# gallilmaimon/DISSC

Measured on AMD Instinct MI355X. Metric: audio-sec/sec (RTF) HiFi-GAN resynth, 10s x32 batch, higher is better.
Workload: dtype f32

## Files before the change

### dissc_amd/_lib.py

```python
import ctypes
import os

import torch

_HERE = os.path.dirname(os.path.abspath(__file__))
_LIB_NAME = "libdissc_hip.so"


def library_path():
    return os.environ.get("DISSC_HIP_LIB") or os.path.join(_HERE, _LIB_NAME)


class DisscError(RuntimeError):
    pass


class DisscTensor(ctypes.Structure):
    _fields_ = [("name", ctypes.c_char_p), ("data", ctypes.c_void_p),
                ("shape", ctypes.c_int64 * 4), ("ndim", ctypes.c_int32)]


MAX_UPS, MAX_RK = 8, 4


class DisscGenConfig(ctypes.Structure):
    _fields_ = [("model_in_dim", ctypes.c_int32), ("upsample_initial_channel", ctypes.c_int32),
                ("num_upsamples", ctypes.c_int32), ("upsample_rates", ctypes.c_int32 * MAX_UPS),
                ("upsample_kernel_sizes", ctypes.c_int32 * MAX_UPS), ("num_kernels", ctypes.c_int32),
                ("resblock_kernel_sizes", ctypes.c_int32 * MAX_RK),
                ("resblock_dilations", (ctypes.c_int32 * 3) * MAX_RK),
                ("num_embeddings", ctypes.c_int32), ("embedding_dim", ctypes.c_int32),
                ("num_speakers", ctypes.c_int32), ("has_f0", ctypes.c_int32), ("has_spkr", ctypes.c_int32)]


class DisscConvLaunch(ctypes.Structure):
    _fields_ = [(n, ctypes.c_int32) for n in ("family", "cfg", "bm", "bn", "rows", "p0", "np", "ntap", "pad_left")]


class DisscBf3Info(ctypes.Structure):
    _fields_ = [(n, ctypes.c_int32) for n in ("bm", "bn", "small_grid", "tile", "cols", "h4", "pad")]


class DisscWino8Plan(ctypes.Structure):
    _fields_ = [(n, ctypes.c_int32) for n in ("mi", "ni", "wps", "r", "ns", "unit", "ot", "cpr", "gx", "gy")]


class DisscWinoPlan(ctypes.Structure):
    _fields_ = [(n, ctypes.c_int32) for n in ("ns", "dilation", "cpr", "rh", "tw", "shv", "unit", "ot", "gx", "gy", "wgs", "lds_bytes")]


def _load():
    path = library_path()
    if not os.path.exists(path):
        raise DisscError(
            f"{path} not found: build the HIP library first "
            "(python -c 'import __graft_entry__ as g; g.build()').  "
            "dissc_amd has no CPU fallback.")
    L = ctypes.CDLL(path)
    vp, i32, i64p = ctypes.c_void_p, ctypes.c_int, ctypes.c_void_p
    L.dissc_last_error.restype = ctypes.c_char_p
    L.dissc_abi_version.restype = i32
    L.dissc_device_count.restype = i32
    L.dissc_device_name.argtypes = [i32, ctypes.c_char_p, ctypes.c_size_t]
    L.dissc_gen_create.argtypes = [ctypes.POINTER(DisscGenConfig), ctypes.POINTER(DisscTensor),
                                   ctypes.c_size_t, ctypes.POINTER(vp)]
    L.dissc_gen_create_ex.argtypes = [ctypes.POINTER(DisscGenConfig), ctypes.POINTER(DisscTensor),
                                      ctypes.c_size_t, i32, ctypes.POINTER(vp)]
    L.dissc_gen_destroy.argtypes = [vp]
    L.dissc_gen_destroy.restype = None
    L.dissc_gen_hop.argtypes = [vp]
    L.dissc_gen_workspace_bytes.argtypes = [vp, i32, i32]
    L.dissc_gen_workspace_bytes.restype = ctypes.c_size_t
    L.dissc_gen_flops.argtypes = [vp, ctypes.c_int64]
    L.dissc_gen_flops.restype = ctypes.c_double
    L.dissc_gen_flops_executed.argtypes = [vp, ctypes.c_int64]
    L.dissc_gen_flops_executed.restype = ctypes.c_double
    L.dissc_gen_forward.argtypes = [vp, i64p, vp, i64p, vp, i32, i32, vp, vp, ctypes.c_size_t, vp]
    L.dissc_conv1d.argtypes = [vp, vp, vp, vp, vp, i32, i32, i32, i32, i32, i32, i32, i32,
                               ctypes.c_float, vp]
    L.dissc_conv_transpose1d.argtypes = [vp, vp, vp, vp, vp, i32, i32, i32, i32, i32, i32, i32, i32,
                                         ctypes.c_float, vp]
    L.dissc_conv1d_prec.argtypes = [vp, vp, vp, vp, vp, i32, i32, i32, i32, i32, i32, i32, i32, ctypes.c_float, i32, vp]
    L.dissc_conv_transpose1d_prec.argtypes = [vp, vp, vp, vp, vp, i32, i32, i32, i32, i32, i32, i32, i32, ctypes.c_float, i32, vp]
    L.dissc_pred_create.argtypes = [i32, ctypes.POINTER(DisscTensor), ctypes.c_size_t, ctypes.POINTER(vp)]
    L.dissc_pred_destroy.argtypes = [vp]
    L.dissc_pred_destroy.restype = None
    L.dissc_pred_workspace_bytes.argtypes = [vp, i32, i32]
    L.dissc_pred_workspace_bytes.restype = ctypes.c_size_t
    L.dissc_len_set_norm.argtypes = [vp, ctypes.c_float, ctypes.c_float]
    L.dissc_len_forward.argtypes = [vp, vp, vp, vp, i32, i32, vp, i32, vp, ctypes.c_size_t, vp]
    L.dissc_pitch_forward.argtypes = [vp, vp, vp, vp, i32, i32, i32, vp, vp, i32, vp, i32, vp,
                                      ctypes.c_size_t, vp]
    L.dissc_dedup.argtypes = [vp, vp, i32, i32, vp, vp, vp, vp]
    L.dissc_len_carryover.argtypes = [vp, vp, i32, i32, vp, vp, vp]
    L.dissc_expand.argtypes = [vp, vp, vp, i32, i32, vp, i32, vp]
    L.dissc_hubert_create.argtypes = [i32, ctypes.POINTER(DisscTensor), ctypes.c_size_t, vp, i32,
                                      ctypes.POINTER(vp)]
    L.dissc_hubert_create_ex.argtypes = [i32, ctypes.POINTER(DisscTensor), ctypes.c_size_t, vp, i32, i32,
                                         ctypes.POINTER(vp)]
    L.dissc_hubert_precision.argtypes = [vp]
    L.dissc_hubert_destroy.argtypes = [vp]
    L.dissc_hubert_destroy.restype = None
    L.dissc_hubert_frames.argtypes = [i32]
    L.dissc_hubert_workspace_bytes.argtypes = [vp, i32, i32]
    L.dissc_hubert_workspace_bytes.restype = ctypes.c_size_t
    L.dissc_hubert_forward.argtypes = [vp, vp, vp, i32, i32, vp, vp, vp, ctypes.c_size_t, vp]
    L.dissc_kmeans_assign.argtypes = [vp, vp, vp, i32, i32, i32, vp, vp]
    L.dissc_mfma_peak.argtypes = [i32, ctypes.POINTER(ctypes.c_float)]
    L.dissc_erf_check.argtypes = [vp, vp, i32, vp]
    L.dissc_attention.argtypes = [vp, vp, i32, i32, i32, i32, vp, vp]
    L.dissc_layernorm_cf.argtypes = [vp, vp, vp, vp, i32, i32, i32, ctypes.c_float, vp, vp]
    L.dissc_set_option.argtypes = [ctypes.c_char_p, i32]
    L.dissc_get_option.argtypes = [ctypes.c_char_p, ctypes.POINTER(ctypes.c_int)]
    L.dissc_conv_bench.argtypes = [i32] * 9 + [ctypes.POINTER(ctypes.c_float)]
    L.dissc_conv1d_s2.argtypes = [vp, vp, vp, vp, vp] + [i32] * 9 + [vp]
    L.dissc_conv1d_s2_prec.argtypes = [vp, vp, vp, vp, vp] + [i32] * 9 + [vp]
    L.dissc_linear_prec.argtypes = [vp, vp, vp, vp, vp, vp] + [i32] * 7 + [vp]
    L.dissc_conv_s2_bench.argtypes = [i32] * 5 + [ctypes.POINTER(ctypes.c_float)]
    L.dissc_pair_bench.argtypes = [i32] * 8 + [ctypes.POINTER(ctypes.c_float)]
    L.dissc_pair_info.argtypes = [i32] * 3 + [ctypes.POINTER(ctypes.c_int)] * 2
    L.dissc_conv_info.argtypes = [i32] * 7 + [ctypes.POINTER(DisscConvLaunch), i32, ctypes.POINTER(ctypes.c_int)]
    L.dissc_wino8_info.argtypes = [i32] * 6 + [ctypes.POINTER(DisscWino8Plan)]
    L.dissc_wino_info.argtypes = [i32] * 5 + [ctypes.POINTER(DisscWinoPlan)]
    L.dissc_resblock1d_bf3.argtypes = [vp, vp, vp, vp, vp, i32, i32, i32, vp, i32, i32, ctypes.c_float, i32, ctypes.c_float, i32, i32, vp]
    L.dissc_bf3_info.argtypes = [i32] * 6 + [vp, i32, i32, ctypes.POINTER(DisscBf3Info)]
    L.dissc_respair1d.argtypes = [vp] * 8 + [i32] * 6 + [ctypes.c_float, i32, ctypes.c_float, i32, vp]
    L.dissc_wav_postprocess.argtypes = [vp, vp, i32, i32, vp]
    L.dissc_pitch_stats.argtypes = [vp, vp, i32, vp, vp, vp, vp]
    i64 = ctypes.c_longlong
    L.dissc_pack_rows.argtypes = [vp, i64, vp, vp, i32, i32, vp, vp]
    L.dissc_comm_unique_id.argtypes = [ctypes.c_char_p]
    L.dissc_comm_create.argtypes = [ctypes.c_char_p, i32, i32, ctypes.POINTER(vp)]
    L.dissc_comm_destroy.argtypes = [vp]
    L.dissc_allgather_waves.argtypes = [vp, vp, ctypes.c_size_t, vp, vp]
    L.dissc_resample.argtypes = [vp, i32, vp, i32, ctypes.c_double, vp, vp, i32, i32, vp]
    return L


lib = _load()

for _kv in filter(None, os.environ.get("DISSC_OPTIONS", "").split(",")):
    _k, _v = _kv.split("=")
    if lib.dissc_set_option(_k.strip().encode(), int(_v)) != 0:
        raise DisscError(f"DISSC_OPTIONS: unknown option {_k}")


def check(rc, what=""):
    if rc != 0:
        msg = lib.dissc_last_error()
        raise DisscError(f"{what} failed ({rc}): {msg.decode() if msg else '?'}")


def current_stream_ptr(device=None):
    return ctypes.c_void_p(torch.cuda.current_stream(device).cuda_stream)


def make_tensor_table(named):
    arr = (DisscTensor * len(named))()
    keep = []
    for i, (k, t) in enumerate(named.items()):
        t = t.detach().to("cpu", torch.float32).contiguous()
        nb = k.encode()
        keep.append((t, nb))
        arr[i].name = nb
        arr[i].data = t.data_ptr()
        arr[i].ndim = t.dim()
        for d in range(t.dim()):
            arr[i].shape[d] = t.shape[d]
    return arr, keep


def conv_info(Cin, Cout, k, dilation=1, up=1, B=1, Lmax_out=1):
    out = (DisscConvLaunch * 16)()
    n = ctypes.c_int(0)
    check(lib.dissc_conv_info(Cin, Cout, k, dilation, up, B, Lmax_out, out, 16, ctypes.byref(n)), "dissc_conv_info")
    assert n.value <= 16
    return [{f: getattr(out[i], f) for f, _ in DisscConvLaunch._fields_} for i in range(n.value)]


def wino8_info(C, k, dilation, R, B, Lmax):
    out = DisscWino8Plan()
    check(lib.dissc_wino8_info(C, k, dilation, R, B, Lmax, ctypes.byref(out)), "dissc_wino8_info")
    return {f: getattr(out, f) for f, _ in DisscWino8Plan._fields_}


def wino_info(C, k, dilation, B, Lmax):
    out = DisscWinoPlan()
    check(lib.dissc_wino_info(C, k, dilation, B, Lmax, ctypes.byref(out)), "dissc_wino_info")
    return {f: getattr(out, f) for f, _ in DisscWinoPlan._fields_}


def bf3_conv_info(Cin, Cout, k, dilation=1, B=1, Lmax=1):
    out = DisscBf3Info()
    check(lib.dissc_bf3_info(Cout, Cin, k, dilation, B, Lmax, None, 0, 0, ctypes.byref(out)), "dissc_bf3_info")
    return {f: getattr(out, f) for f in ("bm", "bn", "small_grid", "tile")}


def bf3_block_info(C, k, dil, m0=0, m1=3):
    out = DisscBf3Info()
    d3 = (ctypes.c_int32 * 3)(*dil)
    check(lib.dissc_bf3_info(C, C, k, 1, 1, 1, d3, m0, m1, ctypes.byref(out)), "dissc_bf3_info")
    return {f: getattr(out, f) for f in ("cols", "pad", "h4", "bn")}


def get_option(key):
    v = ctypes.c_int(0)
    check(lib.dissc_get_option(key.encode(), ctypes.byref(v)), f"dissc_get_option({key})")
    return v.value


def set_option(key, value):
    check(lib.dissc_set_option(key.encode(), int(value)), f"dissc_set_option({key})")
```

### dissc_amd/csrc/common.h

```cpp
#pragma once
#include <hip/hip_runtime.h>
#include <stdint.h>
#include <stdio.h>

#include <atomic>
#include <functional>
#include <mutex>
#include <string>
#include <vector>

#include "../../include/dissc_hip.h"

#ifndef DISSC_EXPERIMENTAL
#define DISSC_EXPERIMENTAL 0
#endif

namespace dissc {

void set_error(const char* fmt, ...);

#define DISSC_OPTION_LIST_DEFAULT(X) \
  X(multistream, 1, "multistream") \
  X(pair_dma, 1, "pair_dma") \
  X(precision, 0, "precision") \
  X(enc_precision, 0, "enc_precision") \
  X(use_mfma32, 1, "mfma32") \
  X(ragged_enum, 1, "ragged_enum") \
  X(lin128, 1, "lin128") \
  X(conv2s128, 1, "conv2s128") \
  X(xcd_order, 11, "xcd_order") \
  X(xcd_mg, 0, "xcd_mg") \
  X(small_grid, 1, "small_grid") \
  X(kernel_dbg, 0, "kernel_dbg") \
  X(wino_sv, 1, "wino_sv") \
  X(wino8_c64_wide, 3, "wino8_c64_wide") \
  X(wino8_mask, 0450770550, "wino8_mask") \
  X(wino8_r4_mask, 0770770010, "wino8_r4_mask") \
  X(wino8_r4, 1, "wino8_r4") \
  X(wino8, 1, "wino8") \
  X(wino, 1, "wino") \
  X(hubert_split, 1, "hubert_split") \
  X(pair_max_c, 32, "pair_max_c") \
  X(pair_f23, 3, "pair_f23") \
  X(pair_tc6, 3, "pair_tc6") \
  X(pair_f23_c64, 1, "pair_f23_c64") \
  X(pair_tc6_c64, 1, "pair_tc6_c64")
#define DISSC_OPTION_LIST_EXPERIMENTAL(X) \
  X(graphs, 0, "graphs") \
  X(graph_frames, 2048, "graph_frames") \
  X(enc_tc, 0, "enc_tc") \
  X(s2tc_xmode, 0, "s2tc_xmode") \
  X(pair_wino, 0, "pair_wino") \
  X(pairw_chv, 2, "pairw_chv")
#if DISSC_EXPERIMENTAL
#define DISSC_OPTION_LIST(X) DISSC_OPTION_LIST_DEFAULT(X) DISSC_OPTION_LIST_EXPERIMENTAL(X)
#else
#define DISSC_OPTION_LIST(X) DISSC_OPTION_LIST_DEFAULT(X)
#endif
struct Options {
#define DISSC_OPT_FIELD(f, d, k) int f = d;
  DISSC_OPTION_LIST(DISSC_OPT_FIELD)
#undef DISSC_OPT_FIELD
#if !DISSC_EXPERIMENTAL
#define DISSC_OPT_CONST(f, d, k) static constexpr int f = d;
  DISSC_OPTION_LIST_EXPERIMENTAL(DISSC_OPT_CONST)
#undef DISSC_OPT_CONST
#endif
  int cfg_for_bm[5] = {6, 5, 7, 1, 0};
  int cfg32_for_bm[4] = {3, 2, 1, 0};
};
extern Options g_defaults;
extern thread_local const Options* t_opts;
inline const Options& opts() { return t_opts ? *t_opts : g_defaults; }
extern int g_graph_hits, g_graph_captures;
struct OptScope {
  const Options* prev;
  explicit OptScope(const Options* o) : prev(t_opts) { t_opts = o; }
  ~OptScope() { t_opts = prev; }
  OptScope(const OptScope&) = delete;
  OptScope& operator=(const OptScope&) = delete;
};

extern thread_local int g_conv_prec;
struct PrecScope {
  const int prev;
  explicit PrecScope(int p) : prev(g_conv_prec) { g_conv_prec = p; }
  ~PrecScope() { g_conv_prec = prev; }
  PrecScope(const PrecScope&) = delete;
  PrecScope& operator=(const PrecScope&) = delete;
};

#define DISSC_HIP_CHECK(expr)                                                       \
  do {                                                                              \
    hipError_t _e = (expr);                                                         \
    if (_e != hipSuccess) {                                                         \
      dissc::set_error("%s failed: %s (%s:%d)", #expr, hipGetErrorString(_e),       \
                       __FILE__, __LINE__);                                         \
      return DISSC_EHIP;                                                            \
    }                                                                               \
  } while (0)

typedef float f32x4 __attribute__((ext_vector_type(4)));

struct DeviceOnce {
  std::mutex mu;
  std::atomic<bool> done[64];
  DeviceOnce() {
    for (auto& d : done) d.store(false, std::memory_order_relaxed);
  }
  hipError_t max_lds(const void* fn, int bytes) {
    int dev = 0;
    hipError_t e = hipGetDevice(&dev);
    if (e != hipSuccess) return e;
    std::atomic<bool>& d = done[dev & 63];
    if (d.load(std::memory_order_acquire)) return hipSuccess;
    std::lock_guard<std::mutex> g(mu);
    if (d.load(std::memory_order_relaxed)) return hipSuccess;
    e = hipFuncSetAttribute(fn, hipFuncAttributeMaxDynamicSharedMemorySize, bytes);
    if (e == hipSuccess) d.store(true, std::memory_order_release);
    return e;
  }
};

#ifdef __HIPCC__
__device__ __forceinline__ float erf_1ulp(float a) {
  const float t = fabsf(a), s = a * a;
  float r = fmaf(-1.72853470e-5f, t, 3.83197126e-4f);
  const float u = fmaf(-3.88396438e-3f, t, 2.42546219e-2f);
  r = fmaf(r, s, u);
  r = fmaf(r, t, -1.06777877e-1f);
  r = fmaf(r, t, -6.34846687e-1f);
  r = fmaf(r, t, -1.28717512e-1f);
  r = fmaf(r, t, -t);
  const float big = copysignf(1.0f - __expf(r), a);
  float q = -5.96761703e-4f;
  q = fmaf(q, s, 4.99119423e-3f);
  q = fmaf(q, s, -2.67681349e-2f);
  q = fmaf(q, s, 1.12819925e-1f);
  q = fmaf(q, s, -3.76125336e-1f);
  q = fmaf(q, s, 1.28379166e-1f);
  const float small = fmaf(q, a, a);
  return t > 0.927734375f ? big : small;
}
#endif

#ifdef __HIPCC__
typedef unsigned dissc_u32x4 __attribute__((ext_vector_type(4)));
__device__ __forceinline__ __amdgpu_buffer_rsrc_t wave_rsrc(const void* base, unsigned bytes) {
  const unsigned long long pa = reinterpret_cast<unsigned long long>(base);
  const unsigned lo = __builtin_amdgcn_readfirstlane((unsigned)pa), hi = __builtin_amdgcn_readfirstlane((unsigned)(pa >> 32));
  return __builtin_amdgcn_make_buffer_rsrc(reinterpret_cast<void*>(((unsigned long long)hi << 32) | lo), 0,
                                           __builtin_amdgcn_readfirstlane(bytes), 0x00020000);
}
__device__ __forceinline__ f32x4 rsrc_load16(__amdgpu_buffer_rsrc_t rs, unsigned lane_bytes, unsigned scalar_bytes) {
  return __builtin_bit_cast(f32x4, __builtin_amdgcn_raw_buffer_load_b128(rs, (int)lane_bytes, (int)scalar_bytes, 0));
}
#endif

constexpr int KC = 16;

enum Epi : int {
  EPI_STORE = 0,
  EPI_RES = 1,
  EPI_MRF_SET = 2,
  EPI_MRF_ADD = 3,
  EPI_MRF_DIV = 4,
  EPI_STORE_ACT = 5,
};
constexpr int ZERO_TAIL = 8;

struct ConvArgs {
  const float* x;
  const float* wpack;
  const float* wpack2 = nullptr;
  const float* bias;
  const float* scale;
  const float* shift;
  const float* res;
  float* out;
  float* acc;
  const int32_t* lengths;
  int len_default;
  int len_mul;
  const int32_t* lengths_out;
  int olen_default;
  int pad_left;
  int groups;
  int mt_per_group;
  int nsub_group;
  int act;
  int xcd;
  int xcd_ntile, xcd_nb;
  int xcd_mg, xcd_span;
  int prec;
  int m32;
  int cfg32;
  int CIN, M, KS, dil, nchunk;
  int XW;
  int ldx, ldo;
  long long x_bstride, o_bstride;
  float slope;
  float mrf_div;
  float out_slope;
  int dma_in;
  int ragged_enum;
  int epi;
  int up;
  int up_np, up_p0;
};

constexpr int MAX_TAP_SPAN = 60;
constexpr int WIDE_TAP_SPAN = 128;

int launch_conv(const ConvArgs& a, int B, int Lmax_out, int stride, hipStream_t stream);
int conv_tile_bn(int M);
int conv_cfg(int M);
int conv_cfg_bm(int cfg);
int conv_cfg_bn(int cfg);
void conv_set_cfg(int bm_class, int cfg);
int conv_xw(int M, int KS, int dil, int stride = 1, int m32 = 0, int bn = 0);
int launch_conv32(const ConvArgs& a, int B, int Lmax_out, int stride, hipStream_t stream);
bool lin128_supported(const ConvArgs& a);
int launch_lin128(const ConvArgs& a, int B, int Lmax_out, hipStream_t stream);
bool conv2s128_shape(int Cout, int Cin, int KS, int stride, int groups);
void pack_s2_weights128(const float* w, int Cout, int Cin, std::vector<float>& packed);
bool conv2s128_supported(const ConvArgs& a);
int launch_conv2s128(const ConvArgs& a, int B, int Lmax_out, hipStream_t stream);
int conv32_tile_bn(int M);
int conv32_cfg(int M);
int conv32_pick_cfg(int M, int B, int Lmax_out);
int conv32_launch_cfg(int cfg32, int M);
int conv32_cfg_bm(int cfg);
int conv32_cfg_bn(int cfg);
void conv32_set_cfg(int bm_class, int cfg);
void pack_conv_weights32(const float* w, int Cout, int Cin, int KS, std::vector<float>& packed,
                         int& Mpad, int& nchunk, int groups);
void pack_conv_weights_bf3(const float* w, int Cout, int Cin, int KS, std::vector<float>& packed,
                           int& Mpad, int& nchunk);
int launch_conv_bf3(const ConvArgs& a, int B, int Lmax_out, hipStream_t stream);
int conv_bf3_tile_bn(int M);
struct ConvBf3Plan { int tile, BM, BN, small; };
int conv_bf3_plan(int M, int KS, int dil, int groups, int B, int Lmax_out, ConvBf3Plan& p);
bool enc_bf3_supported(int Cout, int Cin, int KS, int dil, int groups, int stride, int pad_left);
int launch_enc_bf3(const ConvArgs& a, int B, int Lmax_out, int stride, hipStream_t stream);

void pack_conv_weights(const float* w, int Cout, int Cin, int KS, std::vector<float>& packed,
                       int& Mpad, int& nchunk, int groups = 1);
void convT_phase_weights(const float* w, int Cin, int Cout, int k, int s, int p0, int np, int dlo,
                         int ntap, std::vector<float>& wc);

struct DevConv {
  float* wpack = nullptr;
  float* wpack2 = nullptr;
  float* bias = nullptr;
  float* scale = nullptr;
  float* shift = nullptr;
  int CIN = 0, M = 0, KS = 0, dil = 1, nchunk = 0, up = 1;
  int groups = 1, Mpad = 0, stride = 1, pad_left = -1;
  int up_np = 1, up_p0 = 0;
  int act = 0;
  int m32 = 0;
  int prec = 0;
  double macs_per_t = 0;
  int wino = 0;
  int wr = 3;
};
struct Batch {
  const int32_t* lengths = nullptr;
  int len_default = 0, len_mul = 1, B = 0, Lmax = 0;
  const int32_t* lengths_out = nullptr;
  int olen_default = -1;
};
inline Batch batch_of(const int32_t* lengths, int len_mul, int B, int Lmax) {
  Batch bt;
  bt.lengths = lengths; bt.len_default = bt.Lmax = Lmax; bt.len_mul = len_mul; bt.B = B;
  return bt;
}
struct EpiSpec {
  int epi = EPI_STORE;
  const float* res = nullptr;
  float* acc = nullptr;
  float mrf_div = 1.f, out_slope = 0.f;
};
inline EpiSpec epi_of(int epi, const float* res = nullptr, float* acc = nullptr, float mrf_div = 1.f) {
  EpiSpec ep;
  ep.epi = epi; ep.res = res; ep.acc = acc; ep.mrf_div = mrf_div;
  return ep;
}
int upload(const std::vector<float>& h, float** d);
int pack_thread_count();
int run_pack_tasks(const std::vector<std::function<int()>>& tasks, int nthr, const Options& opt, int prec);
int conv_m32_rule(int Mg, int groups);
void conv_geometry(DevConv& dc, int Cout, int Cin, int KS, int dil, int groups, int stride, int pad_left);
struct ConvTGroup { int p0, np, dlo, ntap; };
void convT_groups(int Cout, int k, int s, std::vector<ConvTGroup>& out);
int conv_launch_cfg32(const DevConv& dc, int B, int Lmax_out);
int conv_launch_info(const DevConv& dc, int B, int Lmax_out, int* family, int* cfg, int* bm, int* bn);
int make_conv(const float* w, const float* bias, int Cout, int Cin, int KS, int dil, DevConv& dc,
              int groups = 1, int stride = 1, int pad_left = -1);
int make_convT(const float* w, const float* bias, int Cin, int Cout, int k, int s,
               std::vector<DevConv>& groups);
int set_affine(DevConv& dc, const float* scale, const float* shift, int n);
void free_conv(DevConv& dc);
int run_conv(const DevConv& dc, const float* x, float* out, const Batch& bt, const EpiSpec& ep, int C_x, int ldx, int ldo,
             float slope, hipStream_t stream, int dma_in = 0);

bool wino_supported(int Cout, int Cin, int KS, int dil);
int make_wino(const float* w, const float* bias, int C, int KS, int dil, DevConv& dc);
double wino_executed_macs_per_t(int C, int KS);
int run_wino(const DevConv& dc, const float* x, float* out, const Batch& bt, const EpiSpec& ep, int ldx, int ldo, float slope,
             hipStream_t stream);
struct WinoPlan { int inst, NS, dil, CPR, RH, TW, SHV, unit, OT, gx, gy, wgs, lds_bytes; };
int wino_plan(int C, int KS, int dil, int B, int Lmax, WinoPlan& p);

bool wino8_supported(int Cout, int Cin, int KS, int dil);
bool wino8_r4_supported(int C, int KS, int dil);
int make_wino8(const float* w, const float* bias, int C, int KS, int dil, DevConv& dc, int R = 3);
double wino8_executed_macs_per_t(int C, int KS, int R);
int run_wino8(const DevConv& dc, const float* x, float* out, const Batch& bt, const EpiSpec& ep, int ldx, int ldo, float slope,
              hipStream_t stream);
struct Wino8Plan { int inst, R, NS, MI, NI, WPS, unit, OT, CPR, gx, gy; };
int wino8_plan(int C, int KS, int dil, int R, int B, int Lmax, Wino8Plan& p);

struct DevPairW {
  float* w1 = nullptr;
  float* w2 = nullptr;
  float* b1 = nullptr;
  float* b2 = nullptr;
  int C = 0, KS = 0, dil = 1;
  int form = 0;
};
bool pair_f23_supported(int C, int KS, int dil);
bool pair_tc6_supported(int C, int KS, int dil);
bool pairw43_built();
int pack_pairw43(const float* w, int C, int KS, float** dev);
int launch_pairw43(const DevPairW& pw, const float* x, float* out, const Batch& bt, const EpiSpec& ep, int ld, float slope,
                   hipStream_t stream);
bool pairw_supported(int C, int KS, int dil);
bool pair_form_supported(int form, int C, int KS, int dil);
int pair_reg_tile(int form, int C, int KS, int dil);
int make_pairw(const float* w1, const float* b1, const float* w2, const float* b2, int C, int KS, int dil, int form, DevPairW& pw);
void free_pairw(DevPairW& pw);
int launch_respair_wino(const DevPairW& pw, const float* x, float* out, const Batch& bt, const EpiSpec& ep, int ld, float slope,
                        hipStream_t stream);

bool respair_supported(int C, int KS, int dil);
int launch_respair(const DevConv& c1, const DevConv& c2, const float* x, float* out, const Batch& bt, const EpiSpec& ep, int ld,
                   float slope, hipStream_t stream);

bool resblock_bf3_supported(int C, int KS, const int* dil);
void pack_resblock_bf3(int C, int KS, const float* const* w6, std::vector<float>& packed);
struct Bf3Block { int C, KS; const int* dil; const float *wpack, *bias; };
int launch_resblock_bf3(const Bf3Block& blk, const float* x, const Batch& bt, const EpiSpec& ep, int ld, float slope, int m0, int m1,
                        hipStream_t stream);
struct ResblockBf3Plan { int NW, NI, COLS, PAD, H4, BN; };
int resblock_bf3_plan(int C, int KS, const int* dil, int m0, int m1, ResblockBf3Plan& p);

struct DevS2tc {
  float* wpack = nullptr;
  float* bias = nullptr;
  int CIN = 0, M = 0, act = 0;
};
bool s2tc_supported(int Cout, int Cin, int KS, int stride);
int make_s2tc(const float* w, const float* bias, int Cout, int Cin, DevS2tc& dc);
void free_s2tc(DevS2tc& dc);
double s2tc_executed_macs_per_out(int Cout, int Cin);
int run_s2tc(const DevS2tc& dc, const float* x, float* out, const Batch& bt, int ldx, int ldo, hipStream_t stream);

struct ZeroSpans {
  float* p[DISSC_MAX_RK];
  int n;
};
void launch_embed_concat(const int64_t* code, const float* f0, const int64_t* spkr,
                         const float* dict_w, const float* spkr_w, const int32_t* lengths, int B,
                         int T, int E, int has_f0, int has_spkr, int n_codes, int n_spk, float* x,
                         int ldx, const ZeroSpans& zs, hipStream_t stream);
void launch_conv_post(const float* x, const float* w, const float* bias, const int32_t* lengths,
                      int len_mul, int B, int C, int KS, int L, int ldx, long long x_bstride,
                      float slope, float* wav, int ldw, hipStream_t stream);
void launch_wav_postprocess(float* wav, const int32_t* n_samples, int B, int ld,
                            hipStream_t stream);

}
```

### dissc_amd/csrc/diag.hip

```cpp
#include <stdlib.h>

#include <algorithm>
#include <vector>

#include "gen_plan.h"

using namespace dissc;

namespace {

struct DiagScope {
  DevConv c1, c2;
  DevPairW pw;
  DevS2tc tc;
  std::vector<float*> bufs;
  hipEvent_t e0 = nullptr, e1 = nullptr;
  hipError_t alloc(float** p, size_t n) {
    const hipError_t e = hipMalloc((void**)p, n * sizeof(float));
    if (e == hipSuccess) bufs.push_back(*p);
    return e;
  }
  hipError_t events() {
    const hipError_t e = hipEventCreate(&e0);
    return e != hipSuccess ? e : hipEventCreate(&e1);
  }
  ~DiagScope() {
    if (e0) (void)hipEventDestroy(e0);
    if (e1) (void)hipEventDestroy(e1);
    for (float* q : bufs) (void)hipFree(q);
    free_conv(c1);
    free_conv(c2);
    free_pairw(pw);
    free_s2tc(tc);
  }
};

struct Lcg {
  uint32_t s = 12345u;
  void fill(std::vector<float>& v, float scale, float centre = 0.5f) {
    for (auto& x : v) {
      s = s * 1664525u + 1013904223u;
      x = ((s >> 8) / 16777216.0f - centre) * scale;
    }
  }
};

template <class Once>
int time_launches(const DiagScope& d, int iters, Once once, float* ms_out) {
  int rc = DISSC_OK;
  for (int it = 0; it < 2 && !rc; ++it) rc = once();
  if (rc) return rc;
  DISSC_HIP_CHECK(hipEventRecord(d.e0, nullptr));
  for (int it = 0; it < iters && !rc; ++it) rc = once();
  DISSC_HIP_CHECK(hipEventRecord(d.e1, nullptr));
  const hipError_t e = hipEventSynchronize(d.e1);
  float ms = 0.f;
  (void)hipEventElapsedTime(&ms, d.e0, d.e1);
  *ms_out = ms / iters;
  if (rc) return rc;
  DISSC_HIP_CHECK(e);
  return DISSC_OK;
}

void dump_timeline(const char* path, const float* dev, size_t bytes) {
  std::vector<char> hb(bytes);
  if (hipMemcpy(hb.data(), dev, hb.size(), hipMemcpyDeviceToHost) == hipSuccess)
    if (FILE* f = fopen(path, "wb")) {
      fwrite(hb.data(), 1, hb.size(), f);
      fclose(f);
    }
}

}

extern "C" {

static int drained(int rc, hipStream_t stream) {
  const hipError_t e = hipStreamSynchronize(stream);
  if (rc) return rc;
  DISSC_HIP_CHECK(e);
  return DISSC_OK;
}

static int conv_once(DevConv& dc, const float* x, float* y, const Batch& bt, int ldx, int ldo, float in_slope, hipStream_t stream) {
  const int rc = drained(run_conv(dc, x, y, bt, EpiSpec(), dc.CIN, ldx, ldo, in_slope, stream), stream);
  free_conv(dc);
  return rc;
}

static int prec_available(const char* who, int prec, int Cout, int Cin, int k, int dilation) {
  if (prec != 1) return DISSC_OK;
  DevConv dc;
  PrecScope prec_scope(1);
  conv_geometry(dc, Cout, Cin, k, dilation, 1, 1, -1);
  if (dc.prec != 1) {
    set_error("%s: no split-bf16 instance for %d rows, k = %d, dilation %d (>= 32 rows, taps spanning <= %d columns, not the big "
              "1x1 layers)", who, dc.M, dc.KS, dc.dil, MAX_TAP_SPAN);
    return DISSC_EINVAL;
  }
  return DISSC_OK;
}

int dissc_conv1d_prec(const float* x, const float* w_host, const float* bias_host, float* y, const int32_t* lengths, int B, int Cin,
                      int Cout, int k, int dilation, int ldx, int ldo, int Lmax, float in_slope, int prec, void* stream) {
  if (!x || !w_host || !y || k % 2 != 1 || dilation < 1 || (prec != 0 && prec != 1)) {
    set_error("dissc_conv1d: bad argument (prec %d: 0 = fp32, 1 = split-bf16)", prec);
    return DISSC_EINVAL;
  }
  int rc = prec_available("dissc_conv1d_prec", prec, Cout, Cin, k, dilation);
  if (rc) return rc;
  DevConv dc;
  {
    PrecScope prec_scope(prec);
    if (!prec && opts().wino8 >= 2 && wino8_supported(Cout, Cin, k, dilation))
      rc = make_wino8(w_host, bias_host, Cout, k, dilation, dc, opts().wino8_r4 >= 2 && wino8_r4_supported(Cout, k, dilation) ? 4 : 3);
    else if (!prec && opts().wino >= 2 && wino_supported(Cout, Cin, k, dilation))
      rc = make_wino(w_host, bias_host, Cout, k, dilation, dc);
    else
      rc = make_conv(w_host, bias_host, Cout, Cin, k, dilation, dc);
  }
  if (rc) return rc;
  return conv_once(dc, x, y, batch_of(lengths, 1, B, Lmax), ldx, ldo, in_slope, (hipStream_t)stream);
}

int dissc_conv1d(const float* x, const float* w_host, const float* bias_host, float* y, const int32_t* lengths, int B, int Cin,
                 int Cout, int k, int dilation, int ldx, int ldo, int Lmax, float in_slope, void* stream) {
  return dissc_conv1d_prec(x, w_host, bias_host, y, lengths, B, Cin, Cout, k, dilation, ldx, ldo, Lmax, in_slope, 0, stream);
}

static int pair_run(int mode, const DiagScope& d, const float* x, float* tmp, float* y, const Batch& bt, const EpiSpec& ep, int C,
                    int ld, float slope, hipStream_t st) {
  int rc;
  switch (mode) {
    case 0: case 2: case 4: case 5:
      if ((rc = run_conv(d.c1, x, tmp, bt, EpiSpec(), C, ld, ld, slope, st))) return rc;
      return run_conv(d.c2, tmp, y, bt, epi_of(ep.epi, x, ep.acc, ep.mrf_div), C, ld, ld, slope, st);
    case 1:
      return launch_respair(d.c1, d.c2, x, y, bt, ep, ld, slope, st);
    case 3:
      return launch_respair_wino(d.pw, x, y, bt, ep, ld, slope, st);
    default:
      set_error("pair mode %d", mode);
      return DISSC_EINVAL;
  }
}

static int pair_make(int mode, const float* w1, const float* b1, const float* w2, const float* b2, int C, int k, int d, DiagScope& ds) {
  DevConv &c1 = ds.c1, &c2 = ds.c2;
  int rc;
  if (mode == 2) {
    if (!wino_supported(C, C, k, d) && !(C == 32 && (k == 3 || k == 7 || k == 11) && (d == 1 || d == 3 || d == 5))) {
      set_error("pair mode 2: no conv_wino instance for C = %d, k = %d, d = %d", C, k, d);
      return DISSC_EINVAL;
    }
    if ((rc = make_wino(w1, b1, C, k, d, c1))) return rc;
    return make_wino(w2, b2, C, k, 1, c2);
  }
  if (mode == 3) return make_pairw(w1, b1, w2, b2, C, k, d, pair_reg_form(C, k, d), ds.pw);
  if (mode == 4) {
    if (!wino_supported(C, C, k, d) || !wino_supported(C, C, k, 1)) {
      set_error("pair mode 4: no transform-domain conv instance for C = %d, k = %d, d = %d", C, k, d);
      return DISSC_EINVAL;
    }
    if ((rc = make_pair_conv(td_conv_form(C, k, d), w1, b1, C, k, d, c1))) return rc;
    return make_pair_conv(td_conv_form(C, k, 1), w2, b2, C, k, 1, c2);
  }
  if (mode == 5 && ((rc = prec_available("pair mode 5", 1, C, C, k, d)) || (rc = prec_available("pair mode 5", 1, C, C, k, 1)))) return rc;
  PrecScope prec_scope(mode == 5 ? 1 : 0);
  if ((rc = make_conv(w1, b1, C, C, k, d, c1))) return rc;
  return make_conv(w2, b2, C, C, k, 1, c2);
}

int dissc_respair1d(const float* x, const float* w1_host, const float* b1_host, const float* w2_host, const float* b2_host,
                    float* y, float* acc, const int32_t* lengths, int B, int C, int k, int dilation, int ld, int Lmax,
                    float slope, int epi, float mrf_div, int mode, void* stream) {
  if (!x || !w1_host || !w2_host || !y || k % 2 != 1 || dilation < 1 || B <= 0 || epi < EPI_RES || epi > EPI_MRF_DIV ||
      (epi != EPI_RES && !acc)) {
    set_error("dissc_respair1d: bad argument");
    return DISSC_EINVAL;
  }
  DiagScope ds;
  float* tmp = nullptr;
  int rc = pair_make(mode, w1_host, b1_host, w2_host, b2_host, C, k, dilation, ds);
  if (!rc && (mode == 0 || mode == 2 || mode == 4 || mode == 5) && ds.alloc(&tmp, (size_t)B * C * ld) != hipSuccess) {
    set_error("dissc_respair1d: hipMalloc");
    rc = DISSC_ENOMEM;
  }
  if (!rc)
    rc = pair_run(mode, ds, x, tmp, y, batch_of(lengths, 1, B, Lmax), epi_of(epi, nullptr, acc, mrf_div), C, ld, slope, (hipStream_t)stream);
  return drained(rc, (hipStream_t)stream);
}

int dissc_resblock1d_bf3(const float* x, const float* const* w6_host, const float* const* b6_host, float* acc, const int32_t* lengths,
                         int B, int C, int k, const int32_t* dil3, int ld, int Lmax, float slope, int epi, float mrf_div, int m0, int m1,
                         void* stream) {
  if (!x || !w6_host || !b6_host || !acc || !dil3 || x == acc) {
    set_error("dissc_resblock1d_bf3: bad argument (null pointer, or acc aliasing x)");
    return DISSC_EINVAL;
  }
  for (int l = 0; l < 6; ++l)
    if (!w6_host[l] || !b6_host[l]) {
      set_error("dissc_resblock1d_bf3: weight or bias %d is null", l);
      return DISSC_EINVAL;
    }
  const int dil[3] = {dil3[0], dil3[1], dil3[2]};
  ResblockBf3Plan plan;
  int rc = resblock_bf3_plan(C, k, dil, m0, m1, plan);
  if (rc) return rc;
  std::vector<float> fw, fb;
  pack_resblock_bf3(C, k, w6_host, fw);
  for (int l = 0; l < 6; ++l) fb.insert(fb.end(), b6_host[l], b6_host[l] + C);
  DiagScope ds;
  float *dw = nullptr, *db = nullptr;
  if (ds.alloc(&dw, fw.size()) != hipSuccess || ds.alloc(&db, fb.size()) != hipSuccess) {
    set_error("dissc_resblock1d_bf3: hipMalloc");
    return DISSC_ENOMEM;
  }
  DISSC_HIP_CHECK(hipMemcpy(dw, fw.data(), fw.size() * sizeof(float), hipMemcpyHostToDevice));
  DISSC_HIP_CHECK(hipMemcpy(db, fb.data(), fb.size() * sizeof(float), hipMemcpyHostToDevice));
  Bf3Block blk;
  blk.C = C; blk.KS = k; blk.dil = dil; blk.wpack = dw; blk.bias = db;
  rc = launch_resblock_bf3(blk, x, batch_of(lengths, 1, B, Lmax), epi_of(epi, nullptr, acc, mrf_div), ld, slope, m0, m1,
                           (hipStream_t)stream);
  return drained(rc, (hipStream_t)stream);
}

int dissc_bf3_info(int Cout, int Cin, int k, int dilation, int B, int Lmax, const int32_t* dil3, int m0, int m1, DisscBf3Info* out) {
  DisscBf3Info o = {};
  if (!dil3) {
    if (Cin < 1 || Cout < 1 || k < 1 || dilation < 1) {
      set_error("dissc_bf3_info: bad argument");
      return DISSC_EINVAL;
    }
    int rc = prec_available("dissc_bf3_info", 1, Cout, Cin, k, dilation);
    ConvBf3Plan p;
    if (!rc) rc = conv_bf3_plan(Cout, k, dilation, 1, B, Lmax, p);
    if (rc) return rc;
    o.bm = p.BM; o.bn = p.BN; o.small_grid = p.small; o.tile = p.tile;
  } else {
    const int dil[3] = {dil3[0], dil3[1], dil3[2]};
    ResblockBf3Plan p;
    const int rc = resblock_bf3_plan(Cout, k, dil, m0, m1, p);
    if (rc) return rc;
    o.bn = p.BN; o.cols = p.COLS; o.h4 = p.H4; o.pad = p.PAD;
  }
  if (out) *out = o;
  return DISSC_OK;
}

int dissc_pair_info(int C, int k, int dilation, int* form_out, int* tile_out) {
  const int form = pair_reg_form(C, k, dilation);
  if (!pair_form_supported(form, C, k, dilation)) {
    set_error("dissc_pair_info: no instance for C = %d, k = %d, dilation %d", C, k, dilation);
    return DISSC_EINVAL;
  }
  if (form_out) *form_out = form;
  if (tile_out) *tile_out = pair_reg_tile(form, C, k, dilation);
  return DISSC_OK;
}

int dissc_conv_info(int Cin, int Cout, int k, int dilation, int up, int B, int Lmax_out, DisscConvLaunch* out, int max_out,
                    int* n_out) {
  if (Cin < 1 || Cout < 1 || k < 1 || dilation < 1 || up < 1 || B < 1 || Lmax_out < 1 || max_out < 0 || (max_out && !out) ||
      (up == 1 && k % 2 != 1) || (up > 1 && ((k - up) % 2 != 0 || k < up || dilation != 1))) {
    set_error("dissc_conv_info: bad argument");
    return DISSC_EINVAL;
  }
  std::vector<ConvTGroup> plan;
  if (up > 1) convT_groups(Cout, k, up, plan);
  else plan.push_back(ConvTGroup{0, 1, 0, k});
  int n = 0;
  for (const ConvTGroup& g : plan) {
    DevConv dc;
    conv_geometry(dc, Cout * g.np, Cin, g.ntap, up > 1 ? 1 : dilation, 1, 1, up > 1 ? -g.dlo : -1);
    int family, cfg, bm, bn;
    const int rc = conv_launch_info(dc, B, Lmax_out, &family, &cfg, &bm, &bn);
    if (rc) return rc;
    if (n < max_out) {
      DisscConvLaunch& o = out[n];
      o.family = family; o.cfg = cfg; o.bm = bm; o.bn = bn; o.rows = dc.M;
      o.p0 = g.p0; o.np = g.np; o.ntap = g.ntap;
      o.pad_left = dc.pad_left >= 0 ? dc.pad_left : ((dc.KS - 1) * dc.dil) / 2;
    }
    ++n;
  }
  if (n_out) *n_out = n;
  return DISSC_OK;
}

int dissc_wino8_info(int C, int k, int dilation, int R, int B, int Lmax, DisscWino8Plan* out) {
  Wino8Plan p;
  const int rc = wino8_plan(C, k, dilation, R, B, Lmax, p);
  if (rc) return rc;
  if (out) {
    out->mi = p.MI; out->ni = p.NI; out->wps = p.WPS; out->r = p.R; out->ns = p.NS;
    out->unit = p.unit; out->ot = p.OT; out->cpr = p.CPR; out->gx = p.gx; out->gy = p.gy;
  }
  return DISSC_OK;
}

int dissc_wino_info(int C, int k, int dilation, int B, int Lmax, DisscWinoPlan* out) {
  WinoPlan p;
  const int rc = wino_plan(C, k, dilation, B, Lmax, p);
  if (rc) return rc;
  if (out) {
    out->ns = p.NS; out->dilation = p.dil; out->cpr = p.CPR; out->rh = p.RH; out->tw = p.TW; out->shv = p.SHV;
    out->unit = p.unit; out->ot = p.OT; out->gx = p.gx; out->gy = p.gy; out->wgs = p.wgs; out->lds_bytes = p.lds_bytes;
  }
  return DISSC_OK;
}

int dissc_pair_bench(int B, int C, int k, int dilation, int L, int epi, int iters, int mode, float* ms_out) {
  if (!ms_out || B <= 0 || L <= 0 || iters <= 0 || epi < EPI_RES || epi > EPI_MRF_DIV) {
    set_error("dissc_pair_bench: bad argument");
    return DISSC_EINVAL;
  }
  std::vector<float> w1((size_t)C * C * k), w2((size_t)C * C * k), bias(C, 0.1f);
  Lcg rnd;
  rnd.fill(w1, 0.05f);
  rnd.fill(w2, 0.05f);
  DiagScope ds;
  int rc = pair_make(mode, w1.data(), bias.data(), w2.data(), bias.data(), C, k, dilation, ds);
  if (rc) return rc;
  const int ld = (L + 3) / 4 * 4;
  const size_t n = (size_t)B * C * ld;
  float *x = nullptr, *y = nullptr, *t = nullptr, *a = nullptr;
  std::vector<float> hx(n);
  rnd.fill(hx, 2.f);
  if (ds.alloc(&x, n) != hipSuccess || ds.alloc(&y, n) != hipSuccess || ds.alloc(&t, n) != hipSuccess ||
      ds.alloc(&a, n) != hipSuccess || hipMemcpy(x, hx.data(), n * 4, hipMemcpyHostToDevice) != hipSuccess ||
      hipMemset(a, 0, n * 4) != hipSuccess || ds.events() != hipSuccess) {
    set_error("dissc_pair_bench: allocation failed");
    return DISSC_ENOMEM;
  }
  const Batch bt = batch_of(nullptr, 1, B, L);
  const EpiSpec ep = epi_of(epi, nullptr, a, 3.f);
  return time_launches(ds, iters, [&]() { return pair_run(mode, ds, x, t, y, bt, ep, C, ld, 0.1f, nullptr); }, ms_out);
}

int dissc_conv_transpose1d_prec(const float* x, const float* w_host, const float* bias_host, float* y, const int32_t* lengths, int B,
                                int Cin, int Cout, int k, int stride, int ldx, int ldo, int Lmax, float in_slope, int prec,
                                void* stream) {
  if (!x || !w_host || !y || stride < 1 || (k - stride) % 2 != 0 || (prec != 0 && prec != 1)) {
    set_error("dissc_conv_transpose1d: bad argument (prec %d: 0 = fp32, 1 = split-bf16)", prec);
    return DISSC_EINVAL;
  }
  std::vector<ConvTGroup> plan;
  convT_groups(Cout, k, stride, plan);
  int rc = DISSC_OK;
  for (const ConvTGroup& g : plan)
    if (!rc) rc = prec_available("dissc_conv_transpose1d_prec", prec, Cout * g.np, Cin, g.ntap, 1);
  if (rc) return rc;
  std::vector<DevConv> grp;
  {
    PrecScope prec_scope(prec);
    rc = make_convT(w_host, bias_host, Cin, Cout, k, stride, grp);
  }
  for (auto& dc : grp) {
    int r2 = rc ? rc : conv_once(dc, x, y, batch_of(lengths, 1, B, Lmax), ldx, ldo, in_slope, (hipStream_t)stream);
    if (rc) free_conv(dc);
    rc = rc ? rc : r2;
  }
  return rc;
}

int dissc_conv_transpose1d(const float* x, const float* w_host, const float* bias_host, float* y, const int32_t* lengths, int B,
                           int Cin, int Cout, int k, int stride, int ldx, int ldo, int Lmax, float in_slope, void* stream) {
  return dissc_conv_transpose1d_prec(x, w_host, bias_host, y, lengths, B, Cin, Cout, k, stride, ldx, ldo, Lmax, in_slope, 0, stream);
}

int dissc_conv_bench(int B, int Cin, int Cout, int k, int dilation, int L, int epi, int iters, int flags, float* ms_out) {
  if (!ms_out || B <= 0 || L <= 0 || iters <= 0) {
    set_error("dissc_conv_bench: bad argument");
    return DISSC_EINVAL;
  }
  std::vector<float> w((size_t)Cout * Cin * k), bias(Cout, 0.1f);
  Lcg rnd;
  rnd.fill(w, 0.05f);
  if (flags & 0x20) std::fill(w.begin(), w.end(), 0.f);
  DiagScope ds;
  DevConv& dc = ds.c1;
  const bool w8 = (flags & 4) && wino8_supported(Cout, Cin, k, dilation);
  const bool wino = w8 || ((flags & 2) && wino_supported(Cout, Cin, k, dilation));
  int rc;
  {
    PrecScope prec_scope(opts().precision);
    rc = w8 ? make_wino8(w.data(), bias.data(), Cout, k, dilation, dc, (flags & 8) && wino8_r4_supported(Cout, k, dilation) ? 4 : 3)
            : wino ? make_wino(w.data(), bias.data(), Cout, k, dilation, dc)
                   : make_conv(w.data(), bias.data(), Cout, Cin, k, dilation, dc);
  }
  if (rc) return rc;
  const int ld = (L + 3) / 4 * 4;
  const size_t nx = (size_t)B * Cin * ld, no = (size_t)B * Cout * ld;
  float *x = nullptr, *y = nullptr, *r = nullptr, *a = nullptr;
  std::vector<float> hx(nx);
  rnd.fill(hx, 2.f);
  if (flags & 0x20) std::fill(hx.begin(), hx.end(), 0.f);
  DISSC_HIP_CHECK(ds.alloc(&x, nx));
  DISSC_HIP_CHECK(ds.alloc(&y, no));
  DISSC_HIP_CHECK(ds.alloc(&r, no));
  DISSC_HIP_CHECK(ds.alloc(&a, no));
  DISSC_HIP_CHECK(hipMemcpy(x, hx.data(), nx * 4, hipMemcpyHostToDevice));
  DISSC_HIP_CHECK(hipMemset(r, 0, no * 4));
  DISSC_HIP_CHECK(hipMemset(a, 0, no * 4));
  DISSC_HIP_CHECK(ds.events());
  const int saved_cls = (flags >> 16) & 0xf;
  if (flags & 0x8000) conv_set_cfg(saved_cls, (flags >> 8) & 0x3f);
  const Batch bt = batch_of(nullptr, 1, B, L);
  const EpiSpec ep = epi_of(epi, r, a, 3.f);
  rc = time_launches(ds, iters, [&]() { return run_conv(dc, x, y, bt, ep, Cin, ld, ld, (flags & 1) ? 1.0f : 0.1f, nullptr); }, ms_out);
  if (const char* tlp = getenv("DISSC_TIMELINE")) dump_timeline(tlp, a, std::min<size_t>(no * 4, (size_t)4096 * 64));
  return rc;
}

int dissc_conv_s2_bench(int B, int C, int L, int form, int iters, float* ms_out) {
  if (!ms_out || B <= 0 || L < 3 || iters <= 0 || (form != 0 && form != 1)) {
    set_error("dissc_conv_s2_bench: bad argument");
    return DISSC_EINVAL;
  }
  std::vector<float> w((size_t)C * C * 3);
  Lcg rnd;
  rnd.fill(w, 0.1f);
  const int Lo = (L - 3) / 2 + 1;
  const int ldx = (L + 3) / 4 * 4, ldo = (Lo + 3) / 4 * 4;
  const size_t nx = (size_t)B * C * ldx, no = (size_t)B * C * ldo;
  std::vector<float> hx(nx);
  rnd.fill(hx, 2.f, 0.3f);
  DiagScope ds;
  float *x = nullptr, *y = nullptr;
  DISSC_HIP_CHECK(ds.alloc(&x, nx));
  DISSC_HIP_CHECK(ds.alloc(&y, no));
  DISSC_HIP_CHECK(hipMemcpy(x, hx.data(), nx * 4, hipMemcpyHostToDevice));
  DevS2tc& tc = ds.tc;
  DevConv& dc = ds.c1;
  int rc = form == 1 ? make_s2tc(w.data(), nullptr, C, C, tc) : make_conv(w.data(), nullptr, C, C, 3, 1, dc, 1, 2, 0);
  if (rc) return rc;
  tc.act = 1;
  dc.act = 1;
  Batch bt;
  bt.len_default = L; bt.olen_default = Lo; bt.B = B; bt.Lmax = Lo;
  float* tlbuf = nullptr;
  const char* tlp = getenv("DISSC_TIMELINE");
  if (tlp) {
    DISSC_HIP_CHECK(ds.alloc(&tlbuf, (size_t)1024 * 64));
    DISSC_HIP_CHECK(hipMemset(tlbuf, 0, (size_t)4096 * 64));
  }
  DISSC_HIP_CHECK(ds.events());
  rc = time_launches(ds, iters, [&]() {
    return form == 1 ? run_s2tc(tc, x, y, bt, ldx, ldo, nullptr)
                     : run_conv(dc, x, y, bt, epi_of(EPI_STORE, nullptr, tlbuf), C, ldx, ldo, 1.0f, nullptr);
  }, ms_out);
  if (tlbuf) dump_timeline(tlp, tlbuf, (size_t)4096 * 64);
  return rc;
}

}
```

### dissc_amd/csrc/gen_plan.h

```cpp
#pragma once
#include "common.h"

namespace dissc {

enum class ChainForm : uint8_t {
  pairs,
  bf3_block,
  bf3_pairs,
};
enum class PairForm : uint8_t {
  direct,
  direct_dma,
  td,
  fused,
  fused_td,
};
enum class ConvForm : uint8_t { direct, f43, f63, f54 };
struct PairPlan {
  PairForm form = PairForm::direct;
  ConvForm conv[2] = {ConvForm::direct, ConvForm::direct};
  uint8_t reg_form = 0;
};
struct ChainPlan {
  ChainForm form = ChainForm::pairs;
  PairPlan pair[3];
};

ConvForm td_conv_form(int C, int KS, int dil);
int pair_reg_form(int C, int KS, int dil);
ChainPlan plan_chain(int C, int KS, const int* dil, int prec);
double pair_macs(const PairPlan& p, int C, int KS, bool executed);
int make_pair_conv(ConvForm f, const float* w, const float* b, int C, int KS, int dil, DevConv& dc);
inline int mrf_epi(int j, int nk) { return j == nk - 1 ? EPI_MRF_DIV : j == 0 ? EPI_MRF_SET : EPI_MRF_ADD; }

}
```

### dissc_amd/csrc/gen_plan.hip

```cpp
#include "gen_plan.h"

namespace dissc {

constexpr int WINO_MIN_C = 64;
constexpr int WINO_C64_KMIN = 3;
static bool wino_wanted(int C, int KS) {
  if (!opts().wino || C < WINO_MIN_C) return false;
  if (C < 128 && KS < WINO_C64_KMIN) return false;
  return wino_supported(C, C, KS, 1);
}

static int w8_shape_bit(int C, int KS, int dil) {
  const int cls = C >= 256 ? 2 : C >= 128 ? 1 : 0;
  return 9 * cls + 3 * (KS == 11 ? 2 : KS == 7 ? 1 : 0) + (dil == 1 ? 0 : dil == 3 ? 1 : 2);
}
ConvForm td_conv_form(int C, int KS, int dil) {
  if (!opts().wino8 || !wino8_supported(C, C, KS, dil) || !((opts().wino8_mask >> w8_shape_bit(C, KS, dil)) & 1))
    return ConvForm::f43;
  const bool r4 = opts().wino8_r4 && wino8_r4_supported(C, KS, dil) && ((opts().wino8_r4_mask >> w8_shape_bit(C, KS, dil)) & 1);
  return r4 ? ConvForm::f54 : ConvForm::f63;
}

int pair_reg_form(int C, int KS, int dil) {
  if (C == 64) {
    if (opts().pair_f23 == 0) return 0;
    if (KS == 3) return opts().pair_f23_c64 && pair_f23_supported(C, KS, dil) ? 1 : 0;
    const int bit = KS == 7 ? 1 : KS == 11 ? 2 : 0;
    return (opts().pair_tc6_c64 & bit) && pair_tc6_supported(C, KS, dil) ? 2 : 0;
  }
  if (C != 16 && C != 32) return 0;
  const int stage = C == 32 ? 1 : 2;
  if (KS == 3) return pair_f23_supported(C, KS, dil) && (opts().pair_f23 & (stage << 2)) ? 1 : 0;
  if (!(opts().pair_f23 & stage)) return 0;
  const int tc6_bit = (C == 32 ? 1 : 4) << (KS == 11 ? 1 : 0);
  if ((KS == 7 || KS == 11) && (opts().pair_tc6 & tc6_bit) && pair_tc6_supported(C, KS, dil)) return 2;
  return pair_f23_supported(C, KS, dil) ? 1 : 0;
}
static bool pairw_wanted(int C, int KS, int dil) {
  if (pair_reg_form(C, KS, dil)) return true;
  if (!opts().pair_wino || !pairw_supported(C, KS, dil)) return false;
  if (opts().pair_wino >= 2) return true;
  if (C == 32) return KS == 11 && dil <= 3;
  return C == 64 && KS == 3 && dil == 1;
}

ChainPlan plan_chain(int C, int KS, const int* dil, int prec) {
  ChainPlan cp;
  if (prec == 1 && resblock_bf3_supported(C, KS, dil)) {
    cp.form = C >= 64 ? ChainForm::bf3_pairs : ChainForm::bf3_block;
    return cp;
  }
  bool fused = prec == 0 && (C < 32 || opts().use_mfma32) && C <= opts().pair_max_c;
  for (int m = 0; m < 3; ++m) fused = fused && respair_supported(C, KS, dil[m]);
  bool all_td = prec == 0 && opts().wino && C > 32 && wino_wanted(C, KS);
  for (int m = 0; m < 3; ++m) all_td = all_td && wino_supported(C, C, KS, dil[m]) && pairw_wanted(C, KS, dil[m]);
  for (int m = 0; m < 3; ++m) {
    PairPlan& p = cp.pair[m];
    const int d = dil[m];
    const bool td = prec == 0 && wino_wanted(C, KS) && wino_supported(C, C, KS, d);
    const bool fuse_td = prec == 0 && opts().wino && pairw_wanted(C, KS, d) && (C > 32 ? td : C <= opts().pair_max_c) &&
                         (fused || all_td || m == 0);
    if (fuse_td) {
      p.form = PairForm::fused_td;
      p.reg_form = (uint8_t)pair_reg_form(C, KS, d);
    } else if (fused) {
      p.form = PairForm::fused;
    } else if (td) {
      p.form = PairForm::td;
      p.conv[0] = td_conv_form(C, KS, d);
      p.conv[1] = td_conv_form(C, KS, 1);
    } else if (opts().pair_dma && prec == 0 && opts().use_mfma32 && C >= 32 && C % KC == 0) {
      p.form = PairForm::direct_dma;
    }
  }
  return cp;
}

double pair_macs(const PairPlan& p, int C, int KS, bool executed) {
  const double direct = (double)C * C * KS;
  auto conv = [&](ConvForm f) {
    return f == ConvForm::f43 ? wino_executed_macs_per_t(C, KS)
         : f == ConvForm::f63 ? wino8_executed_macs_per_t(C, KS, 3)
         : f == ConvForm::f54 ? wino8_executed_macs_per_t(C, KS, 4) : direct;
  };
  if (executed && p.form == PairForm::fused_td) {
    if (p.reg_form == 2) return 2.0 * C * C * 2.0 * ((KS + 3) / 4);
    return p.reg_form == 1 ? 2.0 * C * C * 2.0 * ((KS + 2) / 3) : 2.0 * wino_executed_macs_per_t(C, KS);
  }
  return executed ? conv(p.conv[0]) + conv(p.conv[1]) : direct + direct;
}

int make_pair_conv(ConvForm f, const float* w, const float* b, int C, int KS, int dil, DevConv& dc) {
  switch (f) {
    case ConvForm::f43: return make_wino(w, b, C, KS, dil, dc);
    case ConvForm::f63: return make_wino8(w, b, C, KS, dil, dc, 3);
    case ConvForm::f54: return make_wino8(w, b, C, KS, dil, dc, 4);
    default: return make_conv(w, b, C, C, KS, dil, dc);
  }
}

}
```

### dissc_amd/csrc/generator.hip

```cpp
#include <algorithm>
#include <functional>
#include <map>
#include <mutex>
#include <string>
#include <tuple>
#include <vector>

#include "gen_plan.h"

using namespace dissc;


static hipStream_t shared_aux_stream(int chain, int prio) {
  static std::mutex mu;
  static std::map<std::tuple<int, int, int>, hipStream_t> pool;
  int dev = 0;
  if (hipGetDevice(&dev) != hipSuccess) return nullptr;
  std::lock_guard<std::mutex> lock(mu);
  auto key = std::make_tuple(dev, chain, prio);
  auto it = pool.find(key);
  if (it != pool.end()) return it->second;
  hipStream_t st = nullptr;
  if (hipStreamCreateWithPriority(&st, hipStreamNonBlocking, prio) != hipSuccess) return nullptr;
  pool[key] = st;
  return st;
}

struct dissc_gen {
  Options opt;
  DisscGenConfig cfg;
  int hop = 1;
  DevConv conv_pre;
  std::vector<std::vector<DevConv>> ups;
  std::vector<ChainPlan> plan;
  std::vector<DevConv> rb1, rb2;
  std::vector<DevPairW> pw;
  std::vector<float*> fused_w, fused_b;
  float* post_w = nullptr;
  float* post_b = nullptr;
  int post_C = 0, post_KS = 0;
  float* dict_w = nullptr;
  float* spkr_w = nullptr;
  std::vector<int> stage_C, stage_mul;
  hipStream_t aux[DISSC_MAX_RK] = {nullptr, nullptr, nullptr, nullptr};
  hipEvent_t ev_x = nullptr, ev_fin[DISSC_MAX_RK] = {nullptr, nullptr, nullptr, nullptr};
  struct GraphEntry {
    const void *code, *f0, *spkr, *lengths, *out, *ws;
    int B, T;
    hipGraphExec_t exec;
    unsigned long long stamp;
  };
  std::vector<GraphEntry> graphs;
  hipStream_t cap_stream = nullptr;
  unsigned long long graph_clock = 0;
  int graph_failures = 0;
  ~dissc_gen() {
    for (auto& e : graphs) (void)hipGraphExecDestroy(e.exec);
    if (cap_stream) (void)hipStreamDestroy(cap_stream);
    free_conv(conv_pre);
    for (auto& v : ups) for (auto& c : v) free_conv(c);
    for (auto& c : rb1) free_conv(c);
    for (auto& c : rb2) free_conv(c);
    for (auto& c : pw) free_pairw(c);
    for (float* p : fused_w) if (p) (void)hipFree(p);
    for (float* p : fused_b) if (p) (void)hipFree(p);
    if (post_w) (void)hipFree(post_w);
    if (post_b) (void)hipFree(post_b);
    for (int j = 0; j < DISSC_MAX_RK; ++j)
      if (ev_fin[j]) (void)hipEventDestroy(ev_fin[j]);
    if (ev_x) (void)hipEventDestroy(ev_x);
    if (dict_w) (void)hipFree(dict_w);
    if (spkr_w) (void)hipFree(spkr_w);
  }
};

static inline size_t round_up(size_t x, size_t m) { return (x + m - 1) / m * m; }

extern "C" {

int dissc_gen_create(const DisscGenConfig* cfg, const DisscTensor* weights, size_t n_weights,
                     dissc_gen_t* out) {
  return dissc_gen_create_ex(cfg, weights, n_weights, -1, out);
}

int dissc_gen_create_ex(const DisscGenConfig* cfg, const DisscTensor* weights, size_t n_weights, int precision,
                        dissc_gen_t* out) {
  if (precision < -1 || precision > 1) {
    set_error("dissc_gen_create_ex: precision %d (use -1 = process option, 0 = fp32, 1 = split-bf16)", precision);
    return DISSC_EINVAL;
  }
  const int prec = precision < 0 ? g_defaults.precision : precision;
  if (!cfg || !weights || !out) {
    set_error("dissc_gen_create: null argument");
    return DISSC_EINVAL;
  }
  if (cfg->num_upsamples < 1 || cfg->num_upsamples > DISSC_MAX_UPS || cfg->num_kernels < 1 ||
      cfg->num_kernels > DISSC_MAX_RK) {
    set_error("dissc_gen_create: unsupported num_upsamples=%d / num_kernels=%d", cfg->num_upsamples,
              cfg->num_kernels);
    return DISSC_EINVAL;
  }
  std::map<std::string, const DisscTensor*> byname;
  for (size_t i = 0; i < n_weights; ++i) byname[weights[i].name] = &weights[i];
  auto get = [&](const std::string& name, std::initializer_list<int64_t> shape,
                 const float** p) -> int {
    auto it = byname.find(name);
    if (it == byname.end()) {
      set_error("dissc_gen_create: missing tensor '%s'", name.c_str());
      return DISSC_ENOTFOUND;
    }
    const DisscTensor* t = it->second;
    size_t d = 0;
    bool ok = (size_t)t->ndim == shape.size();
    for (int64_t s : shape) {
      if (ok && t->shape[d] != s) ok = false;
      ++d;
    }
    if (!ok) {
      set_error("dissc_gen_create: tensor '%s' has the wrong shape", name.c_str());
      return DISSC_EINVAL;
    }
    *p = t->data;
    return DISSC_OK;
  };

  dissc_gen* g = new dissc_gen();
  g->opt = g_defaults;
  g->opt.precision = prec;
  OptScope opt_scope(&g->opt);
  g->cfg = *cfg;
  PrecScope prec_scope(prec);
  int rc = DISSC_OK;
  const float *w = nullptr, *b = nullptr;
  const int c0 = cfg->upsample_initial_channel;
  const int in_dim = cfg->model_in_dim;
  const int E = cfg->embedding_dim;
  auto fail = [&](int code) {
    delete g;
    return code;
  };
  std::vector<std::function<int()>> tasks;
  if (in_dim != E + (cfg->has_f0 ? 1 : 0) + (cfg->has_spkr ? E : 0)) {
    set_error("dissc_gen_create: model_in_dim %d != embedding_dim %d (+1 f0) (+%d spkr)", in_dim, E, E);
    return fail(DISSC_EINVAL);
  }
  if ((rc = get("conv_pre.weight", {c0, in_dim, 7}, &w))) return fail(rc);
  if ((rc = get("conv_pre.bias", {c0}, &b))) return fail(rc);
  tasks.push_back([=]() { return make_conv(w, b, c0, in_dim, 7, 1, g->conv_pre); });

  int ch = c0, mul = 1;
  g->ups.resize(cfg->num_upsamples);
  const int nk = cfg->num_kernels;
  g->plan.resize((size_t)cfg->num_upsamples * nk);
  g->rb1.resize((size_t)cfg->num_upsamples * nk * 3);
  g->rb2.resize((size_t)cfg->num_upsamples * nk * 3);
  g->pw.resize((size_t)cfg->num_upsamples * nk * 3);
  g->fused_w.assign((size_t)cfg->num_upsamples * nk, nullptr);
  g->fused_b.assign((size_t)cfg->num_upsamples * nk, nullptr);
  for (int i = 0; i < cfg->num_upsamples; ++i) {
    const int s = cfg->upsample_rates[i], k = cfg->upsample_kernel_sizes[i];
    if (s < 1 || k < s || (k - s) % 2 != 0) {
      set_error("dissc_gen_create: upsample k=%d s=%d unsupported", k, s);
      return fail(DISSC_EINVAL);
    }
    const int cout = ch / 2;
    char name[96];
    snprintf(name, sizeof(name), "ups.%d.weight", i);
    if ((rc = get(name, {ch, cout, k}, &w))) return fail(rc);
    snprintf(name, sizeof(name), "ups.%d.bias", i);
    if ((rc = get(name, {cout}, &b))) return fail(rc);
    tasks.push_back([=]() { return make_convT(w, b, ch, cout, k, s, g->ups[i]); });
    ch = cout;
    mul *= s;
    g->stage_C.push_back(ch);
    g->stage_mul.push_back(mul);
    for (int j = 0; j < nk; ++j) {
      const int rk = cfg->resblock_kernel_sizes[j];
      if (rk % 2 != 1) {
        set_error("dissc_gen_create: even resblock kernel size %d unsupported", rk);
        return fail(DISSC_EINVAL);
      }
      const int* dl = cfg->resblock_dilations[j];
      const size_t cj = (size_t)i * nk + j;
      const ChainPlan& cp = g->plan[cj] = plan_chain(ch, rk, dl, prec);
      const float* w6[6];
      const float* b6[6];
      for (int l = 0; l < 6; ++l) {
        snprintf(name, sizeof(name), "resblocks.%d.convs%d.%d.weight", (int)cj, 1 + l % 2, l / 2);
        if ((rc = get(name, {ch, ch, rk}, &w6[l]))) return fail(rc);
        snprintf(name, sizeof(name), "resblocks.%d.convs%d.%d.bias", (int)cj, 1 + l % 2, l / 2);
        if ((rc = get(name, {ch}, &b6[l]))) return fail(rc);
      }
      if (cp.form != ChainForm::pairs) {
        std::vector<float> fw, fb;
        pack_resblock_bf3(ch, rk, w6, fw);
        for (const float* bl : b6) fb.insert(fb.end(), bl, bl + ch);
        if ((rc = upload(fw, &g->fused_w[cj]))) return fail(rc);
        if ((rc = upload(fb, &g->fused_b[cj]))) return fail(rc);
        continue;
      }
      for (int m = 0; m < 3; ++m) {
        const PairPlan p = cp.pair[m];
        const size_t idx = cj * 3 + m;
        const int d = dl[m];
        const float *w1 = w6[2 * m], *b1 = b6[2 * m], *w2 = w6[2 * m + 1], *b2 = b6[2 * m + 1];
        if (p.form == PairForm::fused_td) {
          tasks.push_back([=]() { return make_pairw(w1, b1, w2, b2, ch, rk, d, p.reg_form, g->pw[idx]); });
        } else {
          tasks.push_back([=]() { return make_pair_conv(p.conv[0], w1, b1, ch, rk, d, g->rb1[idx]); });
          tasks.push_back([=]() { return make_pair_conv(p.conv[1], w2, b2, ch, rk, 1, g->rb2[idx]); });
        }
      }
    }
  }
  g->hop = mul;
  if ((rc = get("conv_post.weight", {1, ch, 7}, &w))) return fail(rc);
  if ((rc = get("conv_post.bias", {1}, &b))) return fail(rc);
  g->post_C = ch;
  g->post_KS = 7;
  if ((rc = upload(std::vector<float>(w, w + ch * 7), &g->post_w))) return fail(rc);
  if ((rc = upload(std::vector<float>(b, b + 1), &g->post_b))) return fail(rc);
  if ((rc = get("dict.weight", {cfg->num_embeddings, E}, &w))) return fail(rc);
  if ((rc = upload(std::vector<float>(w, w + (size_t)cfg->num_embeddings * E), &g->dict_w)))
    return fail(rc);
  if (cfg->has_spkr) {
    if ((rc = get("spkr.weight", {cfg->num_speakers, E}, &w))) return fail(rc);
    if ((rc = upload(std::vector<float>(w, w + (size_t)cfg->num_speakers * E), &g->spkr_w)))
      return fail(rc);
  }
  if ((rc = run_pack_tasks(tasks, pack_thread_count(), g->opt, prec))) return fail(rc);
  if (opts().multistream && nk > 1) {
    if (hipEventCreateWithFlags(&g->ev_x, hipEventDisableTiming) != hipSuccess) return fail(DISSC_EHIP);
    for (int j = 0; j < nk; ++j) {
      if (hipEventCreateWithFlags(&g->ev_fin[j], hipEventDisableTiming) != hipSuccess) return fail(DISSC_EHIP);
      int lo = 0, hi = 0;
      (void)hipDeviceGetStreamPriorityRange(&lo, &hi);
      const int prio = lo + (hi - lo) * j / (nk - 1);
      if (j > 0 && !(g->aux[j] = shared_aux_stream(j, prio))) return fail(DISSC_EHIP);
    }
  }
  *out = g;
  return DISSC_OK;
}

void dissc_gen_destroy(dissc_gen_t g) { delete g; }

int dissc_gen_hop(dissc_gen_t g) { return g ? g->hop : 0; }

constexpr size_t BUF_GUARD = 64;
static size_t gen_buf_floats(const dissc_gen* g, int B, int Tmax) {
  size_t per = (size_t)g->cfg.upsample_initial_channel * round_up(Tmax + ZERO_TAIL, 4);
  per = std::max(per, (size_t)g->cfg.model_in_dim * round_up(Tmax + ZERO_TAIL, 4));
  for (size_t i = 0; i < g->stage_C.size(); ++i)
    per = std::max(per, (size_t)g->stage_C[i] * round_up((size_t)Tmax * g->stage_mul[i] + ZERO_TAIL, 4));
  return round_up(per * B + BUF_GUARD + 512, 64);
}

size_t dissc_gen_workspace_bytes(dissc_gen_t g, int B, int Tmax) {
  if (!g || B <= 0 || Tmax <= 0) return 0;
  OptScope opt_scope(&g->opt);
  return (size_t)(2 + 2 * g->cfg.num_kernels) * gen_buf_floats(g, B, Tmax) * sizeof(float) + 256;
}

static double gen_macs(const dissc_gen* g, bool executed) {
  double macs = g->conv_pre.macs_per_t;
  int mul = 1;
  const int nk = g->cfg.num_kernels;
  for (int i = 0; i < g->cfg.num_upsamples; ++i) {
    for (auto& c : g->ups[i]) macs += c.macs_per_t * mul;
    mul = g->stage_mul[i];
    for (int j = 0; j < nk; ++j)
      for (const PairPlan& p : g->plan[(size_t)i * nk + j].pair)
        macs += pair_macs(p, g->stage_C[i], g->cfg.resblock_kernel_sizes[j], executed) * mul;
  }
  macs += (double)g->post_C * g->post_KS * mul;
  return macs;
}

double dissc_gen_flops(dissc_gen_t g, int64_t frames) { return g ? 2.0 * gen_macs(g, false) * (double)frames : 0; }

double dissc_gen_flops_executed(dissc_gen_t g, int64_t frames) { return g ? 2.0 * gen_macs(g, true) * (double)frames : 0; }

static int gen_forward_body(dissc_gen_t g, const int64_t* code, const float* f0, const int64_t* spkr,
                            const int32_t* lengths, int B, int Tmax, float* wav_out, void* workspace,
                            hipStream_t stream);

int dissc_gen_forward(dissc_gen_t g, const int64_t* code, const float* f0, const int64_t* spkr,
                      const int32_t* lengths, int B, int Tmax, float* wav_out, void* workspace,
                      size_t workspace_bytes, void* stream_) {
  if (!g || !code || !wav_out || !workspace || (g->cfg.has_f0 && !f0) ||
      (g->cfg.has_spkr && !spkr)) {
    set_error("dissc_gen_forward: null argument");
    return DISSC_EINVAL;
  }
  OptScope opt_scope(&g->opt);
  if (B <= 0 || Tmax <= 0) {
    set_error("dissc_gen_forward: B=%d Tmax=%d", B, Tmax);
    return DISSC_EINVAL;
  }
  if ((long long)Tmax * g->hop > 2000000000LL) {
    set_error("dissc_gen_forward: Tmax=%d too long", Tmax);
    return DISSC_EINVAL;
  }
  if (workspace_bytes < dissc_gen_workspace_bytes(g, B, Tmax)) {
    set_error("dissc_gen_forward: workspace %zu < %zu bytes", workspace_bytes,
              dissc_gen_workspace_bytes(g, B, Tmax));
    return DISSC_ENOMEM;
  }
  hipStream_t stream = (hipStream_t)stream_;
#if !DISSC_EXPERIMENTAL
  return gen_forward_body(g, code, f0, spkr, lengths, B, Tmax, wav_out, workspace, stream);
#else
  if (!opts().graphs || g->graph_failures >= 2 || (long long)B * Tmax > opts().graph_frames)
    return gen_forward_body(g, code, f0, spkr, lengths, B, Tmax, wav_out, workspace, stream);
  for (auto& e : g->graphs)
    if (e.code == code && e.f0 == f0 && e.spkr == spkr && e.lengths == lengths && e.out == wav_out && e.ws == workspace &&
        e.B == B && e.T == Tmax) {
      e.stamp = ++g->graph_clock;
      ++g_graph_hits;
      DISSC_HIP_CHECK(hipGraphLaunch(e.exec, stream));
      return DISSC_OK;
    }
  if (!g->cap_stream && hipStreamCreateWithFlags(&g->cap_stream, hipStreamNonBlocking) != hipSuccess) {
    (void)hipGetLastError();
    return gen_forward_body(g, code, f0, spkr, lengths, B, Tmax, wav_out, workspace, stream);
  }
  hipGraph_t graph = nullptr;
  hipGraphExec_t exec = nullptr;
  int rc = DISSC_EHIP;
  if (hipStreamBeginCapture(g->cap_stream, hipStreamCaptureModeThreadLocal) == hipSuccess) {
    rc = gen_forward_body(g, code, f0, spkr, lengths, B, Tmax, wav_out, workspace, g->cap_stream);
    const hipError_t e = hipStreamEndCapture(g->cap_stream, &graph);
    if (rc == DISSC_OK && (e != hipSuccess || !graph)) rc = DISSC_EHIP;
    if (rc == DISSC_OK && hipGraphInstantiate(&exec, graph, nullptr, nullptr, 0) != hipSuccess) rc = DISSC_EHIP;
    if (graph) (void)hipGraphDestroy(graph);
  }
  if (rc != DISSC_OK) {
    (void)hipGetLastError();
    ++g->graph_failures;
    return gen_forward_body(g, code, f0, spkr, lengths, B, Tmax, wav_out, workspace, stream);
  }
  if (g->graphs.size() >= 8) {
    size_t old = 0;
    for (size_t i = 1; i < g->graphs.size(); ++i)
      if (g->graphs[i].stamp < g->graphs[old].stamp) old = i;
    (void)hipGraphExecDestroy(g->graphs[old].exec);
    g->graphs.erase(g->graphs.begin() + old);
  }
  ++g_graph_captures;
  g->graphs.push_back({code, f0, spkr, lengths, wav_out, workspace, B, Tmax, exec, ++g->graph_clock});
  DISSC_HIP_CHECK(hipGraphLaunch(exec, stream));
  return DISSC_OK;
#endif
}

static int gen_forward_body(dissc_gen_t g, const int64_t* code, const float* f0, const int64_t* spkr,
                            const int32_t* lengths, int B, int Tmax, float* wav_out, void* workspace,
                            hipStream_t stream) {
  const size_t nbuf = gen_buf_floats(g, B, Tmax);
  float* base = (float*)round_up((size_t)workspace, 256);
  float* X = base;
  float* ACC = base + nbuf;
  float* TMPj[DISSC_MAX_RK];
  float* XKj[DISSC_MAX_RK];
  ZeroSpans zs;
  for (int j = 0; j < g->cfg.num_kernels; ++j) {
    TMPj[j] = base + (size_t)(2 + 2 * j) * nbuf + BUF_GUARD;
    XKj[j] = base + (size_t)(3 + 2 * j) * nbuf;
    zs.p[j] = TMPj[j] - ZERO_TAIL;
  }
  zs.n = g->cfg.num_kernels;
  float* TMP = TMPj[0];
  const bool multi = g->ev_x != nullptr;
  const DisscGenConfig& c = g->cfg;
  int rc;

  const int ld0 = (int)round_up(Tmax, 4);
  launch_embed_concat(code, f0, spkr, g->dict_w, g->spkr_w, lengths, B, Tmax, c.embedding_dim,
                      c.has_f0, c.has_spkr, c.num_embeddings, c.num_speakers, TMP, ld0, zs, stream);
  Batch bt = batch_of(lengths, 1, B, Tmax);
  if ((rc = run_conv(g->conv_pre, TMP, ACC, bt, EpiSpec(), c.model_in_dim, ld0, ld0, 1.0f, stream))) return rc;
  int ch = c.upsample_initial_channel, mul = 1, ld = ld0;
  const int nk = c.num_kernels;
  for (int i = 0; i < c.num_upsamples; ++i) {
    const int s = c.upsample_rates[i];
    const int ch_out = ch / 2, mul_out = mul * s;
    const int ld_out = (int)round_up((size_t)Tmax * mul_out, 4);
    const int ngrp = (int)g->ups[i].size();
    const bool par_ups = multi && ngrp > 1 && ngrp <= nk;
    if (par_ups) DISSC_HIP_CHECK(hipEventRecord(g->ev_x, stream));
    for (int gi = 0; gi < ngrp; ++gi) {
      hipStream_t sg = (par_ups && gi > 0) ? g->aux[gi] : stream;
      if (par_ups && gi > 0) DISSC_HIP_CHECK(hipStreamWaitEvent(sg, g->ev_x, 0));
      if ((rc = run_conv(g->ups[i][gi], ACC, X, bt, EpiSpec(), ch, ld, ld_out, 0.1f, sg))) return rc;
      if (par_ups && gi > 0) {
        DISSC_HIP_CHECK(hipEventRecord(g->ev_fin[gi], sg));
        DISSC_HIP_CHECK(hipStreamWaitEvent(stream, g->ev_fin[gi], 0));
      }
    }
    ch = ch_out; mul = mul_out; ld = ld_out;
    bt = batch_of(lengths, mul, B, Tmax * mul);
    if (multi) DISSC_HIP_CHECK(hipEventRecord(g->ev_x, stream));
    for (int j = 0; j < nk; ++j) {
      hipStream_t sj = (multi && j > 0) ? g->aux[j] : stream;
      if (multi && j > 0) DISSC_HIP_CHECK(hipStreamWaitEvent(sj, g->ev_x, 0));
      const size_t cj = (size_t)i * nk + j;
      const ChainPlan& cp = g->plan[cj];
      const int rk = c.resblock_kernel_sizes[j];
      const int* dl = c.resblock_dilations[j];
      Bf3Block bf3;
      bf3.C = ch; bf3.KS = rk; bf3.dil = dl; bf3.wpack = g->fused_w[cj]; bf3.bias = g->fused_b[cj];
      float* TMPc = multi ? TMPj[j] : TMPj[0];
      float* XKc = multi ? XKj[j] : XKj[0];
      const EpiSpec mrf = epi_of(mrf_epi(j, nk), nullptr, ACC, (float)nk);
      auto acc_turn = [&]() -> int {
        if (multi && j > 0) DISSC_HIP_CHECK(hipStreamWaitEvent(sj, g->ev_fin[j - 1], 0));
        return DISSC_OK;
      };
      if (cp.form == ChainForm::bf3_block) {
        if ((rc = acc_turn()) || (rc = launch_resblock_bf3(bf3, X, bt, mrf, ld, 0.1f, 0, 3, sj))) return rc;
        if (multi) DISSC_HIP_CHECK(hipEventRecord(g->ev_fin[j], sj));
        continue;
      }
      const float* x = X;
      for (int m = 0; m < 3; ++m) {
        const size_t idx = cj * 3 + m;
        const bool last = m == 2;
        float* nxt = x == XKc ? TMPc : XKc;
        const PairForm pf = cp.pair[m].form;
        if (cp.form == ChainForm::bf3_pairs) {
          if (last && (rc = acc_turn())) return rc;
          rc = launch_resblock_bf3(bf3, x, bt, last ? mrf : epi_of(EPI_STORE, nullptr, nxt), ld, 0.1f, m, m + 1, sj);
          x = nxt;
        } else if (pf == PairForm::fused || pf == PairForm::fused_td) {
          if (last && (rc = acc_turn())) return rc;
          float* out = last ? nullptr : nxt;
          const EpiSpec ep = last ? mrf : epi_of(EPI_RES, nullptr, ACC, (float)nk);
          rc = pf == PairForm::fused_td ? launch_respair_wino(g->pw[idx], x, out, bt, ep, ld, 0.1f, sj)
                                        : launch_respair(g->rb1[idx], g->rb2[idx], x, out, bt, ep, ld, 0.1f, sj);
          x = nxt;
        } else {
          const bool dma = pf == PairForm::direct_dma;
          const int ldt = dma ? (int)round_up((size_t)bt.Lmax + ZERO_TAIL, 4) : ld;
          EpiSpec ep_t = epi_of(dma ? EPI_STORE_ACT : EPI_STORE);
          ep_t.out_slope = 0.1f;
          if ((rc = run_conv(g->rb1[idx], x, TMPc, bt, ep_t, ch, ld, ldt, 0.1f, sj))) return rc;
          if (last && (rc = acc_turn())) return rc;
          rc = run_conv(g->rb2[idx], TMPc, XKc, bt, epi_of(last ? mrf.epi : EPI_RES, x, ACC, (float)nk), ch, ldt, ld, dma ? 1.0f : 0.1f,
                        sj, dma ? 1 : 0);
          x = XKc;
        }
        if (rc) return rc;
      }
      if (multi) DISSC_HIP_CHECK(hipEventRecord(g->ev_fin[j], sj));
    }
    if (multi) DISSC_HIP_CHECK(hipStreamWaitEvent(stream, g->ev_fin[nk - 1], 0));
  }
  launch_conv_post(ACC, g->post_w, g->post_b, lengths, mul, B, ch, g->post_KS, Tmax * mul, ld,
                   (long long)ch * ld, 0.01f, wav_out, Tmax * mul, stream);
  DISSC_HIP_CHECK(hipGetLastError());
  return DISSC_OK;
}

int dissc_wav_postprocess(float* wav, const int32_t* n_samples, int B, int ld, void* stream) {
  if (!wav || !n_samples || B <= 0) {
    set_error("dissc_wav_postprocess: bad argument");
    return DISSC_EINVAL;
  }
  launch_wav_postprocess(wav, n_samples, B, ld, (hipStream_t)stream);
  DISSC_HIP_CHECK(hipGetLastError());
  return DISSC_OK;
}

}
```

### dissc_amd/csrc/pair_host.hip

```cpp
#include <string.h>

#include <algorithm>
#include <vector>

#include "common.h"
#include "respair_f23.h"

namespace dissc {

bool pair_f23_supported(int C, int KS, int dil) {
  if (!(dil == 1 || dil == 3 || dil == 5)) return false;
  if (C == 64) return KS == 3;
  return (C == 16 || C == 32) && (KS == 11 || (KS == 3 && DISSC_EXPERIMENTAL));
}
bool pair_tc6_supported(int C, int KS, int dil) { return (C == 32 || C == 64) && (KS == 7 || KS == 11) && (dil == 1 || dil == 3 || dil == 5); }
bool pairw_supported(int C, int KS, int dil) {
  if (!pairw43_built()) return false;
  if (!(dil == 1 || dil == 3 || dil == 5)) return false;
  if (C == 32) return KS == 7 || KS == 11;
  if (C == 64) return KS == 3;
  return false;
}
bool pair_form_supported(int form, int C, int KS, int dil) {
  return form == 2 ? pair_tc6_supported(C, KS, dil) : form == 1 ? pair_f23_supported(C, KS, dil) : pairw_supported(C, KS, dil);
}

static const double kF23G[4][3] = {{1.0, 0.0, 0.0}, {0.5, 0.5, 0.5}, {0.5, -0.5, 0.5}, {0.0, 0.0, 1.0}};
static const double kTc6G[6][4] = {{1.0 / 4, 0.0, 0.0, 0.0},
                                   {-1.0 / 6, -1.0 / 6, -1.0 / 6, -1.0 / 6},
                                   {-1.0 / 6, 1.0 / 6, -1.0 / 6, 1.0 / 6},
                                   {1.0 / 24, 2.0 / 24, 4.0 / 24, 8.0 / 24},
                                   {1.0 / 24, -2.0 / 24, 4.0 / 24, -8.0 / 24},
                                   {0.0, 0.0, 0.0, 1.0}};

static std::vector<float> transform_taps(const float* w, int C, int KS, const double* G, int points, int taps) {
  const int NS = (KS + taps - 1) / taps;
  std::vector<float> U((size_t)points * C * C * NS);
  size_t o = 0;
  for (int p = 0; p < points; ++p)
    for (int cc = 0; cc < C * C; ++cc)
      for (int j = 0; j < NS; ++j) {
        double u = 0.0;
        for (int i = 0; i < taps; ++i)
          if (j + NS * i < KS) u += G[p * taps + i] * (double)w[(size_t)cc * KS + j + NS * i];
        U[o++] = (float)u;
      }
  return U;
}

static int pack_pair_reg(const float* w, float** dev, int C, int KS, int form) {
  if ((form != 1 && form != 2) || (C != 16 && C != 32 && C != 64) || (form == 2 && C == 16) || (form == 1 && C == 64 && KS != 3)) {
    set_error("pack_pair_reg: no layout for form %d, C = %d", form, C);
    return DISSC_EINVAL;
  }
  const int points = form == 2 ? 6 : 4, taps = form == 2 ? 4 : 3, NS = (KS + taps - 1) / taps;
  const std::vector<float> U = transform_taps(w, C, KS, form == 2 ? &kTc6G[0][0] : &kF23G[0][0], points, taps);
  auto u = [&](int p, int co, int ci, int j) { return U[(((size_t)p * C + co) * C + ci) * NS + j]; };
  std::vector<float> packed(U.size());
  size_t o = 0;
  if (C == 16) {
    for (int j = 0; j < NS; ++j)
      for (int p = 0; p < 4; ++p)
        for (int lane = 0; lane < 64; ++lane)
          for (int cq = 0; cq < 4; ++cq) packed[o++] = u(p, lane & 15, 4 * cq + (lane >> 4), j);
  } else if (C == 64 && form == 2) {
    for (int mi = 0; mi < 2; ++mi)
      for (int c = 0; c < 4; ++c)
        for (int j = 0; j < NS; ++j)
          for (int hf = 0; hf < 2; ++hf)
            for (int p = 0; p < 6; ++p)
              for (int lane = 0; lane < 64; ++lane)
                for (int e = 0; e < 4; ++e) packed[o++] = u(p, 32 * mi + (lane & 31), 16 * c + 2 * (4 * hf + e) + (lane >> 5), j);
  } else if (C == 64) {
    for (int st = 0; st < 8; ++st)
      for (int p = 0; p < 4; ++p)
        for (int mi = 0; mi < 2; ++mi)
          for (int lane = 0; lane < 64; ++lane)
            for (int e = 0; e < 4; ++e) packed[o++] = u(p, 32 * mi + (lane & 31), 8 * st + 2 * e + (lane >> 5), 0);
  } else if (form == 1) {
    for (int c = 0; c < 2; ++c)
      for (int j = 0; j < NS; ++j)
        for (int p = 0; p < 4; ++p)
          for (int hf = 0; hf < 2; ++hf)
            for (int lane = 0; lane < 64; ++lane)
              for (int e = 0; e < 4; ++e) packed[o++] = u(p, lane & 31, 16 * c + 2 * (4 * hf + e) + (lane >> 5), j);
  } else {
    for (int c = 0; c < 2; ++c)
      for (int j = 0; j < NS; ++j)
        for (int hf = 0; hf < 2; ++hf)
          for (int p = 0; p < 6; ++p)
            for (int lane = 0; lane < 64; ++lane)
              for (int e = 0; e < 4; ++e) packed[o++] = u(p, lane & 31, 16 * c + 2 * (4 * hf + e) + (lane >> 5), j);
  }
  return upload(packed, dev);
}

int make_pairw(const float* w1, const float* b1, const float* w2, const float* b2, int C, int KS, int dil, int form, DevPairW& pw) {
  pw.form = form;
  if (!pair_form_supported(form, C, KS, dil)) {
    set_error("make_pairw: no instance for C = %d, k = %d, dilation %d", C, KS, dil);
    return DISSC_EINVAL;
  }
  pw.C = C; pw.KS = KS; pw.dil = dil;
  auto pack = [&](const float* w, float** dev) {
    return form ? pack_pair_reg(w, dev, C, KS, form) : pack_pairw43(w, C, KS, dev);
  };
  int rc = pack(w1, &pw.w1);
  if (!rc) rc = pack(w2, &pw.w2);
  std::vector<float> bb(C, 0.f);
  if (b1) memcpy(bb.data(), b1, C * sizeof(float));
  if (!rc) rc = upload(bb, &pw.b1);
  std::fill(bb.begin(), bb.end(), 0.f);
  if (b2) memcpy(bb.data(), b2, C * sizeof(float));
  if (!rc) rc = upload(bb, &pw.b2);
  return rc;
}

void free_pairw(DevPairW& pw) {
  for (float** q : {&pw.w1, &pw.w2, &pw.b1, &pw.b2}) {
    if (*q) (void)hipFree(*q);
    *q = nullptr;
  }
}

template <auto Kernel, class Geo>
static int launch_pair_reg(const PairArgs& a, int B, int Lmax, hipStream_t stream, bool want_max_lds) {
  static DeviceOnce attr_once;
  if (want_max_lds) DISSC_HIP_CHECK(attr_once.max_lds(reinterpret_cast<const void*>(Kernel), 160 * 1024));
  dim3 grid((Lmax + Geo::WOUT - 1) / Geo::WOUT, B);
  hipLaunchKernelGGL(Kernel, grid, dim3(256), sizeof(float) * Geo::C * Geo::XW, stream, a);
  DISSC_HIP_CHECK(hipGetLastError());
  return DISSC_OK;
}

#define DISSC_TC6(K_, D_) DISSC_CASE(2, 32, respair32_tc6_kernel, Tc6Geo, true, K_, D_)
#define DISSC_TC6_64(K_, D_) DISSC_CASE(2, 64, respair64_tc6_kernel, Tc6Geo64, false, K_, D_)
#define DISSC_F23_32(K_, D_) DISSC_CASE(1, 32, respair32_f23_kernel, F23Geo32, true, K_, D_)
#define DISSC_F23_16(K_, D_) DISSC_CASE(1, 16, respair16_f23_kernel, F23Geo16, false, K_, D_)
#define DISSC_F23_64(K_, D_) DISSC_CASE(1, 64, respair64_f23_kernel, F23Geo64, true, K_, D_)
#define DISSC_PAIR_REG_INSTANCES                                                                          \
  DISSC_PAIR_TC6_SHAPES(DISSC_TC6) DISSC_PAIR_F23_SHAPES(DISSC_F23_32) DISSC_PAIR_F23_SHAPES(DISSC_F23_16) \
  DISSC_PAIR_F23_C64_SHAPES(DISSC_F23_64) DISSC_PAIR_TC6_SHAPES(DISSC_TC6_64)

int pair_reg_tile(int form, int C, int KS, int dil) {
#define DISSC_CASE(FORM_, C_, KERNEL_, GEO_, MAX_LDS_, K_, D_) \
  if (form == FORM_ && C == C_ && KS == K_ && dil == D_) return GEO_<K_, D_>::WOUT;
  DISSC_PAIR_REG_INSTANCES
#undef DISSC_CASE
  return 0;
}

int launch_respair_wino(const DevPairW& pw, const float* x, float* out, const Batch& bt, const EpiSpec& ep, int ld, float slope,
                        hipStream_t stream) {
  const int B = bt.B, Lmax = bt.Lmax;
  if (!pw.w1 || ep.epi == EPI_STORE || x == out || ld < 4 || ld % 4 || misaligned16(x) || misaligned16(out) || misaligned16(ep.acc) ||
      B <= 0 || Lmax <= 0) {
    set_error("launch_respair_wino: bad argument (C=%d k=%d d=%d ld=%d epi=%d)", pw.C, pw.KS, pw.dil, ld, ep.epi);
    return DISSC_EINVAL;
  }
  if (!pw.form) {
    if (pairw43_built()) return launch_pairw43(pw, x, out, bt, ep, ld, slope, stream);
    set_error("launch_respair_wino: no instance (the F(4,3) pair kernel is only in DISSC_EXPERIMENTAL=1 builds)");
    return DISSC_EINVAL;
  }
  PairArgs a;
  a.x = x; a.out = out; a.acc = ep.acc; a.w1 = pw.w1; a.w2 = pw.w2; a.b1 = pw.b1; a.b2 = pw.b2;
  a.lengths = bt.lengths; a.len_default = bt.len_default; a.len_mul = bt.len_mul; a.ld = ld;
  a.bstride = (long long)pw.C * ld; a.slope = slope; a.mrf_div = ep.mrf_div; a.epi = ep.epi; a.dbg = opts().kernel_dbg;
#define DISSC_CASE(FORM_, C_, KERNEL_, GEO_, MAX_LDS_, K_, D_)       \
  if (pw.form == FORM_ && pw.C == C_ && pw.KS == K_ && pw.dil == D_) \
    return launch_pair_reg<KERNEL_<K_, D_>, GEO_<K_, D_>>(a, B, Lmax, stream, MAX_LDS_);
  DISSC_PAIR_REG_INSTANCES
#undef DISSC_CASE
  set_error("launch_pair_f23: no instance of form %d for C = %d, k = %d, dilation %d", pw.form, pw.C, pw.KS, pw.dil);
  return DISSC_EINVAL;
}

}
```

### dissc_amd/csrc/respair16_f23.hip

```cpp
#include "common.h"
#include "respair_f23.h"

namespace dissc {

template <int KS_, int DIL>
__global__ void __launch_bounds__(256, 3) respair16_f23_kernel(const PairArgs a) {
  using G = F23Geo16<KS_, DIL>;
  constexpr int C = G::C, NW = G::NW, NT = 64 * NW, NS = G::NS, P2 = G::P2, P1 = G::P1, D1 = G::D1, D2 = G::D2, XW = G::XW,
                W1 = G::W1, NC1 = G::NC1, NC2 = G::NC2, WOUT = G::WOUT, PW = G::PW, NI = 4;
  extern __shared__ __attribute__((aligned(16))) float xs[];

  int b, len, o0;
  if (!pair_tile<WOUT>(a, gridDim.y, b, len, o0)) return;
  const int tid = threadIdx.x, lane = tid & 63, wave = tid >> 6;
  const int l15 = lane & 15, g = lane >> 4;
  const int tin0 = o0 - P2 - P1;
  const int tb = tin0 & ~3, sh = tin0 - tb;
  const float slope = a.slope;
  const float* xb = a.x + (size_t)b * a.bstride;

  pair_stage_window<C, XW, NT>(a, xb, xs, tb, len, tid);

  int base1[NI], base2[NI];
#pragma unroll
  for (int ni = 0; ni < NI; ++ni) {
    const int c = wave * 64 + ni * 16 + l15;
    const int c1 = c < NC1 ? c : NC1 - 1, c2 = c < NC2 ? c : NC2 - 1;
    base1[ni] = 2 * D1 * (c1 / D1) + (c1 % D1);
    base2[ni] = 2 * D2 * (c2 / D2) + (c2 % D2);
  }
  f32x4 acc[4][NI];
  auto clear = [&]() __attribute__((always_inline)) {
#pragma unroll
    for (int p = 0; p < 4; ++p)
#pragma unroll
      for (int ni = 0; ni < NI; ++ni)
#pragma unroll
        for (int e = 0; e < 4; ++e) acc[p][ni][e] = 0.f;
  };
  auto taps = [&](const float* wq, const float* src, const int (&base)[NI], int off0, int dstep, int dunit) __attribute__((always_inline)) {
    const __amdgpu_buffer_rsrc_t wr = wave_rsrc(wq, 0x7ffffff0u);
    f32x4 u[NS][4];
#pragma unroll
    for (int j = 0; j < NS; ++j)
#pragma unroll
      for (int p = 0; p < 4; ++p) u[j][p] = rsrc_load16(wr, lane * 16u, (j * 4 + p) * 1024u);
#pragma unroll
    for (int j = 0; j < NS; ++j) {
#pragma unroll
      for (int cq = 0; cq < 4; ++cq) {
        const int row = 4 * cq + g;
        float bq[4][NI];
#pragma unroll
        for (int ni = 0; ni < NI; ++ni) {
          const float* q = src + row * XW + off0 + base[ni] + j * dstep;
          const float x0 = q[0], x1 = q[dunit], x2 = q[2 * dunit], x3 = q[3 * dunit];
          bq[0][ni] = x0 - x2;
          bq[1][ni] = x1 + x2;
          bq[2][ni] = x2 - x1;
          bq[3][ni] = x1 - x3;
        }
#pragma unroll
        for (int p = 0; p < 4; ++p)
#pragma unroll
          for (int ni = 0; ni < NI; ++ni)
            acc[p][ni] = __builtin_amdgcn_mfma_f32_16x16x4f32(u[j][p][cq], bq[p][ni], acc[p][ni], 0, 0, 0);
      }
      __builtin_amdgcn_sched_barrier(0);
    }
  };

  __syncthreads();
  clear();
  if (!(a.dbg & 1)) taps(a.w1, xs, base1, sh, DIL, D1);

  __syncthreads();
  pair_zero_beyond_t<C, XW, W1, NT>(xs, tid);
#pragma unroll
  for (int ni = 0; ni < NI; ++ni) {
    const int c = wave * 64 + ni * 16 + l15;
    if (c < NC1 && !(a.dbg & 2)) {
      const int pe = 2 * D1 * (c / D1) + (c % D1), po = pe + D1;
      const int te = o0 - P2 + pe, to = te + D1;
      const bool ine = te >= 0 && te < len, ino = to >= 0 && to < len;
#pragma unroll
      for (int r = 0; r < 4; ++r) {
        const int row = 4 * g + r;
        const float bz = a.b1[row];
        const float y0 = acc[0][ni][r], y1 = acc[1][ni][r], y2 = acc[2][ni][r], y3 = acc[3][ni][r];
        float ve = (y0 + y1) + y2 + bz, vo = (y1 - y2) - y3 + bz;
        ve = ve > 0.f ? ve : ve * slope;
        vo = vo > 0.f ? vo : vo * slope;
        xs[row * XW + pe] = ine ? ve : 0.f;
        xs[row * XW + po] = ino ? vo : 0.f;
      }
    }
  }
  __syncthreads();
  clear();
  if (!(a.dbg & 1)) taps(a.w2, xs, base2, 0, 1, D2);

  __syncthreads();
  float* ep = xs + wave * (16 * PW);
  const int prow = lane >> 5, pc4 = lane & 31;
  const int ncol = wave * 128 + 4 * pc4;
  const int tcol = o0 + ncol;
  const size_t ob = (size_t)b * a.bstride;
  const bool live = ncol < WOUT && tcol < len;
  const int epi = a.epi;
  const bool rmw = epi != EPI_RES && epi != EPI_MRF_SET;
  if (a.dbg & 4) {
    if (acc[0][0][0] == 123.f) a.out[0] = 1.f;
    return;
  }
  f32x4 rv[8], pa[8];
#pragma unroll
  for (int p = 0; p < 8; ++p) {
    const int row = 2 * p + prow;
    const int tc = tcol > a.ld - 4 ? a.ld - 4 : tcol;
    rv[p] = *reinterpret_cast<const f32x4*>(a.x + ob + (size_t)row * a.ld + tc);
    if (rmw && live && tcol + 4 <= len) pa[p] = *reinterpret_cast<const f32x4*>(a.acc + ob + (size_t)row * a.ld + tcol);
  }
#pragma unroll
  for (int ni = 0; ni < NI; ++ni) {
    const int cl = ni * 16 + l15;
    const int pe = 2 * D2 * (cl / D2) + (cl % D2);
#pragma unroll
    for (int r = 0; r < 4; ++r) {
      const float y0 = acc[0][ni][r], y1 = acc[1][ni][r], y2 = acc[2][ni][r], y3 = acc[3][ni][r];
      ep[(4 * g + r) * PW + pe] = (y0 + y1) + y2;
      ep[(4 * g + r) * PW + pe + D2] = (y1 - y2) - y3;
    }
  }
  __builtin_amdgcn_wave_barrier();
#pragma unroll
  for (int p = 0; p < 8; ++p) {
    const int row = 2 * p + prow;
    f32x4 v = *reinterpret_cast<const f32x4*>(ep + row * PW + 4 * pc4);
    if (!live) continue;
    const float bz = a.b2[row];
    const size_t idx = ob + (size_t)row * a.ld + tcol;
    pair_store_tail(a, epi, idx, v, bz, rv[p], [&] { return pa[p]; }, 0, len - tcol < 4 ? len - tcol : 4);
  }
}

#define DISSC_INSTANCE(K_, D_) template __global__ void respair16_f23_kernel<K_, D_>(const PairArgs);
DISSC_PAIR_F23_SHAPES(DISSC_INSTANCE)
#undef DISSC_INSTANCE

}
```

### dissc_amd/csrc/respair_f23.h

```cpp
#pragma once
#include "common.h"
#include "ragged_epi.h"

namespace dissc {

struct PairArgs {
  const float* x;
  float* out;
  float* acc;
  const float* w1;
  const float* w2;
  const float* b1;
  const float* b2;
  const int32_t* lengths;
  int len_default, len_mul;
  int ld;
  long long bstride;
  float slope, mrf_div;
  int epi;
  int dbg;
};

template <int WOUT>
__device__ __forceinline__ bool pair_tile(const PairArgs& a, int B, int& b, int& len, int& o0) {
  if (a.lengths == nullptr) {
    b = blockIdx.y;
    len = a.len_default;
    o0 = blockIdx.x * WOUT;
    return o0 < len;
  }
  int tile;
  if (!ragged_tile<WOUT>(blockIdx.y * gridDim.x + blockIdx.x, B, [&](int i) { return a.lengths[i] * a.len_mul; }, b, tile, len))
    return false;
  o0 = tile * WOUT;
  return true;
}

template <int C, int XW, int NT, int NBATCH = 1>
__device__ __forceinline__ void pair_stage_window(const PairArgs& a, const float* xb, float* xs, int tb, int len, int tid) {
  constexpr int NV = XW / 4, NIT = ((C * NV + NT - 1) / NT + NBATCH - 1) / NBATCH;
  const float slope = a.slope;
#pragma unroll
  for (int nb = 0; nb < NBATCH; ++nb) {
    f32x4 sv[NIT];
#pragma unroll
    for (int it = 0; it < NIT; ++it) {
      const int i = tid + (nb * NIT + it) * NT;
      const int r = i / NV < C ? i / NV : C - 1, v = i - (i / NV) * NV;
      const int t = tb + 4 * v;
      const int tc = t < 0 ? 0 : (t > a.ld - 4 ? a.ld - 4 : t);
      sv[it] = *reinterpret_cast<const f32x4*>(xb + (size_t)r * a.ld + tc);
    }
#pragma unroll
    for (int it = 0; it < NIT; ++it) {
      const int i = tid + (nb * NIT + it) * NT;
      if (i >= C * NV) continue;
      const int r = i / NV, v = i - r * NV;
      const int t = tb + 4 * v;
      f32x4 val = sv[it];
#pragma unroll
      for (int e = 0; e < 4; ++e) val[e] = ((t + e) >= 0 && (t + e) < len) ? (val[e] > 0.f ? val[e] : val[e] * slope) : 0.f;
      *reinterpret_cast<f32x4*>(xs + r * XW + 4 * v) = val;
    }
  }
}

template <int C, int XW, int W1, int NT>
__device__ __forceinline__ void pair_zero_beyond_t(float* xs, int tid) {
  for (int i = tid; i < C * (XW - W1); i += NT) {
    const int r = i / (XW - W1), v = i - r * (XW - W1);
    xs[r * XW + W1 + v] = 0.f;
  }
}

template <class AccOld>
__device__ __forceinline__ void pair_store_tail(const PairArgs& a, int epi, size_t idx, f32x4 v, float bz, const f32x4& rv,
                                                AccOld acc_old, int elo, int ehi) {
  if (elo == 0 && ehi == 4) {
#pragma unroll
    for (int e = 0; e < 4; ++e) v[e] = (v[e] + bz) + rv[e];
    epi_store_res(epi, quad_at(a.out + idx), quad_at(a.acc + idx), v, acc_old, a.mrf_div);
  } else {
    for (int e = elo; e < ehi; ++e)
      epi_store_res(epi, a.out + idx + e, a.acc + idx + e, (v[e] + bz) + a.x[idx + e], [&] { return a.acc[idx + e]; }, a.mrf_div);
  }
}

template <int C_, int PROWS, int KS_, int DIL, int WCOLS = 64>
struct F23Geo {
  static constexpr int KS = KS_, NS = (KS_ + 2) / 3, C = C_, NW = 4;
  static constexpr int P2 = (KS - 1) / 2, P1 = P2 * DIL;
  static constexpr int D1 = DIL * NS, D2 = NS;
  static constexpr int NCOLS = WCOLS * NW;
  static constexpr int NU1 = NCOLS / D1, NC1 = NU1 * D1, W1 = 2 * NC1;
  static constexpr int NU2 = NCOLS / D2, NC2 = NU2 * D2, W2 = 2 * NC2;
  static constexpr int WOUT = ((W1 - 2 * P2) < W2 ? (W1 - 2 * P2) : W2) & ~3;
  static constexpr int REACH1 = (3 * NS - 1) * DIL, REACH2 = 3 * NS - 1;
  static constexpr int XW1 = round32_16(3 + W1 + REACH1);
  static constexpr int XW2 = round32_16(W2 + REACH2 + 1);
  static constexpr int XW = XW1 > XW2 ? XW1 : XW2;
  static constexpr int PW = 2 * WCOLS + 4;
  static_assert(NW * PROWS * PW <= C * XW, "the epilogue patches fit the buffer");
  static_assert(W1 <= XW && W2 + REACH2 < XW, "T fits the buffer");
};
template <int KS, int DIL> using F23Geo32 = F23Geo<32, 8, KS, DIL>;
template <int KS, int DIL> using F23Geo16 = F23Geo<16, 16, KS, DIL>;
template <int KS, int DIL> using F23Geo64 = F23Geo<64, 8, KS, DIL, 32>;

template <int C_, int KS_, int DIL_>
struct Tc6GeoC {
  static constexpr int KS = KS_, DIL = DIL_, NS = (KS_ + 3) / 4, C = C_, NW = 4, RB = C_ / 32, NCT = NW / RB;
  static constexpr int P2 = (KS - 1) / 2, P1 = P2 * DIL;
  static constexpr int D1 = DIL * NS, D2 = NS;
  static constexpr int NCOLS = 32 * NCT;
  static constexpr int NU1 = NCOLS / D1, NC1 = NU1 * D1, W1 = 3 * NC1;
  static constexpr int NCW2 = 32 / D2 * D2, OW = 3 * NCW2, W2 = NCT * OW;
  static constexpr int WOUT = ((W1 - 2 * P2) < W2 ? (W1 - 2 * P2) : W2) & ~3;
  static constexpr int REACH1 = (4 * NS - 1) * DIL, REACH2 = 4 * NS - 1;
  static constexpr int XW1 = (3 + W1 + REACH1 + 3) & ~3;
  static constexpr int XW2 = (W2 + REACH2 + 3) & ~3;
  static constexpr int XW = XW1 > XW2 ? XW1 : XW2;
  static constexpr int PW = 96 + 4;
  static constexpr int OCC = 3 * 4 * C * XW <= 160 * 1024 ? 3 : 2;
  static_assert(C == 32 || C == 64, "one or two 32-row blocks");
  static_assert(3 + OW <= PW - 1 && NW * 8 * PW <= C * XW, "the epilogue patches fit the buffer");
  static_assert(W1 <= XW && WOUT + 2 * P2 <= W1 && WOUT <= W2, "T fits the buffer and covers what the owned outputs read");
};
template <int KS, int DIL> using Tc6Geo = Tc6GeoC<32, KS, DIL>;
template <int KS, int DIL> using Tc6Geo64 = Tc6GeoC<64, KS, DIL>;

template <int KS, int DIL> __global__ void respair32_f23_kernel(const PairArgs a);
template <int KS, int DIL> __global__ void respair32_tc6_kernel(const PairArgs a);
template <int KS, int DIL> __global__ void respair16_f23_kernel(const PairArgs a);
template <int KS, int DIL> __global__ void respair64_f23_kernel(const PairArgs a);
template <int KS, int DIL> __global__ void respair64_tc6_kernel(const PairArgs a);
#if DISSC_EXPERIMENTAL
#define DISSC_PAIR_F23_SHAPES(X) X(11, 1) X(11, 3) X(11, 5) X(3, 1) X(3, 3) X(3, 5)
#else
#define DISSC_PAIR_F23_SHAPES(X) X(11, 1) X(11, 3) X(11, 5)
#endif
#define DISSC_PAIR_F23_C64_SHAPES(X) X(3, 1) X(3, 3) X(3, 5)
#define DISSC_PAIR_TC6_SHAPES(X) X(7, 1) X(7, 3) X(7, 5) X(11, 1) X(11, 3) X(11, 5)

}
```

### dissc_amd/csrc/respair_f23.hip

```cpp
#include "common.h"
#include "respair_f23.h"

namespace dissc {

template <int KS_, int DIL>
__global__ void __launch_bounds__(256, 2) respair32_f23_kernel(const PairArgs a) {
  using G = F23Geo32<KS_, DIL>;
  constexpr int C = G::C, NW = G::NW, NT = 64 * NW, NS = G::NS, P2 = G::P2, P1 = G::P1, D1 = G::D1, D2 = G::D2, XW = G::XW,
                W1 = G::W1, NC1 = G::NC1, NC2 = G::NC2, WOUT = G::WOUT, PW = G::PW;
  extern __shared__ __attribute__((aligned(16))) float xs[];

  int b, len, o0;
  if (!pair_tile<WOUT>(a, gridDim.y, b, len, o0)) return;
  const int tid = threadIdx.x, lane = tid & 63, wave = tid >> 6;
  const int l31 = lane & 31, h = lane >> 5;
  const int tin0 = o0 - P2 - P1;
  const int tb = tin0 & ~3, sh = tin0 - tb;
  const float slope = a.slope;
  const float* xb = a.x + (size_t)b * a.bstride;

  pair_stage_window<C, XW, NT>(a, xb, xs, tb, len, tid);

  int base1[2], base2[2];
#pragma unroll
  for (int ni = 0; ni < 2; ++ni) {
    int c = wave * 64 + ni * 32 + l31;
    const int c1 = c < NC1 ? c : NC1 - 1, c2 = c < NC2 ? c : NC2 - 1;
    base1[ni] = 2 * D1 * (c1 / D1) + (c1 % D1);
    base2[ni] = 2 * D2 * (c2 / D2) + (c2 % D2);
  }
  typedef float f32x16f __attribute__((ext_vector_type(16)));
  f32x16f acc[4][2];
  auto clear = [&]() __attribute__((always_inline)) {
#pragma unroll
    for (int p = 0; p < 4; ++p)
#pragma unroll
      for (int ni = 0; ni < 2; ++ni)
#pragma unroll
        for (int e = 0; e < 16; ++e) acc[p][ni][e] = 0.f;
  };
  auto taps = [&](const float* wq, const float* src, const int (&base)[2], int off0, int dstep, int dunit) __attribute__((always_inline)) {
    const __amdgpu_buffer_rsrc_t wr = wave_rsrc(wq, 0x7ffffff0u);
    const unsigned lane16 = lane * 16u;
    f32x4 av[4][2], avn[4][2];
#pragma unroll
    for (int p = 0; p < 4; ++p) {
      av[p][0] = rsrc_load16(wr, lane16, (p * 2 + 0) * 1024u);
      av[p][1] = rsrc_load16(wr, lane16, (p * 2 + 1) * 1024u);
    }
#pragma unroll
    for (int s = 0; s < 2 * NS; ++s) {
      const int sn = s + 1 < 2 * NS ? s + 1 : s;
#pragma unroll
      for (int p = 0; p < 4; ++p) {
        avn[p][0] = rsrc_load16(wr, lane16, ((sn * 4 + p) * 2 + 0) * 1024u);
        avn[p][1] = rsrc_load16(wr, lane16, ((sn * 4 + p) * 2 + 1) * 1024u);
      }
      __builtin_amdgcn_sched_barrier(0);
      const int chunk = s / NS, j = s % NS;
#pragma unroll
      for (int hf = 0; hf < 2; ++hf)
#pragma unroll
        for (int e = 0; e < 4; ++e) {
          const int row = 16 * chunk + 2 * (4 * hf + e) + h;
          float bq[4][2];
#pragma unroll
          for (int ni = 0; ni < 2; ++ni) {
            const float* q = src + row * XW + off0 + base[ni] + j * dstep;
            const float x0 = q[0], x1 = q[dunit], x2 = q[2 * dunit], x3 = q[3 * dunit];
            bq[0][ni] = x0 - x2;
            bq[1][ni] = x1 + x2;
            bq[2][ni] = x2 - x1;
            bq[3][ni] = x1 - x3;
          }
#pragma unroll
          for (int p = 0; p < 4; ++p)
#pragma unroll
            for (int ni = 0; ni < 2; ++ni)
              acc[p][ni] = __builtin_amdgcn_mfma_f32_32x32x2f32(av[p][hf][e], bq[p][ni], acc[p][ni], 0, 0, 0);
        }
      __builtin_amdgcn_sched_barrier(0);
#pragma unroll
      for (int p = 0; p < 4; ++p) {
        av[p][0] = avn[p][0];
        av[p][1] = avn[p][1];
      }
    }
  };

  __syncthreads();
  clear();
  if (!(a.dbg & 1)) taps(a.w1, xs, base1, sh, DIL, D1);

  __syncthreads();
  pair_zero_beyond_t<C, XW, W1, NT>(xs, tid);
#pragma unroll
  for (int ni = 0; ni < 2; ++ni) {
    const int c = wave * 64 + ni * 32 + l31;
    if (c < NC1 && !(a.dbg & 2)) {
      const int pe = 2 * D1 * (c / D1) + (c % D1), po = pe + D1;
      const int te = o0 - P2 + pe, to = te + D1;
      const bool ine = te >= 0 && te < len, ino = to >= 0 && to < len;
#pragma unroll
      for (int r = 0; r < 16; ++r) {
        const int row = (r & 3) + 8 * (r >> 2) + 4 * h;
        const float bz = a.b1[row];
        const float y0 = acc[0][ni][r], y1 = acc[1][ni][r], y2 = acc[2][ni][r], y3 = acc[3][ni][r];
        float ve = (y0 + y1) + y2 + bz, vo = (y1 - y2) - y3 + bz;
        ve = ve > 0.f ? ve : ve * slope;
        vo = vo > 0.f ? vo : vo * slope;
        xs[row * XW + pe] = ine ? ve : 0.f;
        xs[row * XW + po] = ino ? vo : 0.f;
      }
    }
  }
  __syncthreads();
  clear();
  if (!(a.dbg & 1)) taps(a.w2, xs, base2, 0, 1, D2);

  __syncthreads();
  float* ep = xs + wave * (8 * PW);
  const int prow = lane >> 5, pc4 = lane & 31;
  const int ncol = wave * 128 + 4 * pc4;
  const int tcol = o0 + ncol;
  const size_t ob = (size_t)b * a.bstride;
  const bool live = ncol < WOUT && tcol < len;
  const int epi = a.epi;
  const bool rmw = epi != EPI_RES && epi != EPI_MRF_SET;
  if (a.dbg & 4) {
    if (acc[0][0][0] == 123.f) a.out[0] = 1.f;
    return;
  }
#pragma unroll
  for (int qd = 0; qd < 4; ++qd) {
    f32x4 rv[4], pa[4];
#pragma unroll
    for (int p = 0; p < 4; ++p) {
      const int row = 8 * qd + 2 * p + prow;
      const int tc = tcol > a.ld - 4 ? a.ld - 4 : tcol;
      rv[p] = *reinterpret_cast<const f32x4*>(a.x + ob + (size_t)row * a.ld + tc);
      if (rmw && live && tcol + 4 <= len) pa[p] = *reinterpret_cast<const f32x4*>(a.acc + ob + (size_t)row * a.ld + tcol);
    }
    __builtin_amdgcn_wave_barrier();
#pragma unroll
    for (int ni = 0; ni < 2; ++ni) {
      const int cl = ni * 32 + l31;
      const int pe = 2 * D2 * (cl / D2) + (cl % D2);
#pragma unroll
      for (int r = 0; r < 4; ++r) {
        const int rr = 4 * qd + r;
        const float y0 = acc[0][ni][rr], y1 = acc[1][ni][rr], y2 = acc[2][ni][rr], y3 = acc[3][ni][rr];
        ep[(r + 4 * h) * PW + pe] = (y0 + y1) + y2;
        ep[(r + 4 * h) * PW + pe + D2] = (y1 - y2) - y3;
      }
    }
    __builtin_amdgcn_wave_barrier();
#pragma unroll
    for (int p = 0; p < 4; ++p) {
      const int prw = 2 * p + prow;
      f32x4 v = *reinterpret_cast<const f32x4*>(ep + prw * PW + 4 * pc4);
      if (!live) continue;
      const int row = 8 * qd + prw;
      const float bz = a.b2[row];
      const size_t idx = ob + (size_t)row * a.ld + tcol;
      pair_store_tail(a, epi, idx, v, bz, rv[p], [&] { return pa[p]; }, 0, len - tcol < 4 ? len - tcol : 4);
    }
  }
}

template <class G>
__device__ __forceinline__ void pair_tc6_body(const PairArgs a) {
  constexpr int C = G::C, NW = G::NW, NT = 64 * NW, NS = G::NS, P2 = G::P2, P1 = G::P1, D1 = G::D1, D2 = G::D2, XW = G::XW,
                W1 = G::W1, NC1 = G::NC1, NCW2 = G::NCW2, OW = G::OW, WOUT = G::WOUT, PW = G::PW, RB = G::RB, DIL = G::DIL;
  extern __shared__ __attribute__((aligned(16))) float xs[];

  int b, len, o0;
  if (!pair_tile<WOUT>(a, gridDim.y, b, len, o0)) return;
  const int tid = threadIdx.x, lane = tid & 63, wave = tid >> 6;
  const int l31 = lane & 31, h = lane >> 5;
  const int ct = wave / RB, mrow = 32 * (wave % RB);
  const int tin0 = o0 - P2 - P1;
  const int tb = tin0 & ~3, sh = tin0 - tb;
  const float slope = a.slope;
  const float* xb = a.x + (size_t)b * a.bstride;

  pair_stage_window<C, XW, NT, RB>(a, xb, xs, tb, len, tid);

  int base1, base2;
  {
    const int c = ct * 32 + l31;
    const int c1 = c < NC1 ? c : NC1 - 1, c2 = l31 < NCW2 ? l31 : NCW2 - 1;
    base1 = 3 * D1 * (c1 / D1) + (c1 % D1);
    base2 = ct * OW + 3 * D2 * (c2 / D2) + (c2 % D2);
  }
  typedef float f32x16f __attribute__((ext_vector_type(16)));
  f32x16f acc[6];
  auto clear = [&]() __attribute__((always_inline)) {
#pragma unroll
    for (int p = 0; p < 6; ++p)
#pragma unroll
      for (int e = 0; e < 16; ++e) acc[p][e] = 0.f;
  };
  auto taps = [&](const float* wq, const float* src, int base, int dstep, int dunit) __attribute__((always_inline)) {
    const __amdgpu_buffer_rsrc_t wr = wave_rsrc(wq, 0x7ffffff0u);
    const unsigned lane16 = lane * 16u;
    constexpr int NST = C / 16 * NS * 2;
    const unsigned wstep = (a.dbg & 8) ? 0u : 6 * 1024u;
    f32x4 av[6], avn[6];
#pragma unroll
    for (int p = 0; p < 6; ++p) av[p] = rsrc_load16(wr, lane16, p * 1024u);
#pragma unroll
    for (int st = 0; st < NST; ++st) {
      const int sn = st + 1 < NST ? st + 1 : st;
#pragma unroll
      for (int p = 0; p < 6; ++p) avn[p] = rsrc_load16(wr, lane16, sn * wstep + p * 1024u);
      __builtin_amdgcn_sched_barrier(0);
      const int chunk = (st >> 1) / NS, j = (st >> 1) % NS, hf = st & 1;
#pragma unroll
      for (int e = 0; e < 4; ++e) {
        const int row = 16 * chunk + 2 * (4 * hf + e) + h;
        const float* q = src + row * XW + base + j * dstep;
        const float x0 = q[0], x1 = q[dunit], x2 = q[2 * dunit], x3 = q[3 * dunit], x4 = q[4 * dunit], x5 = q[5 * dunit];
        const float pe = __builtin_fmaf(-4.f, x2, x4), po = __builtin_fmaf(-4.f, x1, x3), re = x4 - x2, ro = x3 - x1;
        float bq[6];
        bq[0] = __builtin_fmaf(4.f, x0, __builtin_fmaf(-5.f, x2, x4));
        bq[1] = pe + po;
        bq[2] = pe - po;
        bq[3] = __builtin_fmaf(2.f, ro, re);
        bq[4] = __builtin_fmaf(-2.f, ro, re);
        bq[5] = __builtin_fmaf(4.f, x1, __builtin_fmaf(-5.f, x3, x5));
#pragma unroll
        for (int p = 0; p < 6; ++p) acc[p] = __builtin_amdgcn_mfma_f32_32x32x2f32(av[p][e], bq[p], acc[p], 0, 0, 0);
      }
      __builtin_amdgcn_sched_barrier(0);
#pragma unroll
      for (int p = 0; p < 6; ++p) av[p] = avn[p];
    }
  };
  auto outs = [&](int r, float& y0, float& y1, float& y2) __attribute__((always_inline)) {
    const float s12 = acc[1][r] + acc[2][r], d12 = acc[1][r] - acc[2][r];
    const float s34 = acc[3][r] + acc[4][r], d34 = acc[3][r] - acc[4][r];
    y0 = (acc[0][r] + s12) + s34;
    y1 = __builtin_fmaf(2.f, d34, d12);
    y2 = __builtin_fmaf(4.f, s34, s12) + acc[5][r];
  };

  const int wslab = (wave % RB) * (C / 16 * NS * 2 * 6 * 256);
  __syncthreads();
  clear();
  if (!(a.dbg & 1)) taps(a.w1 + wslab, xs + sh, base1, DIL, D1);

  __syncthreads();
  pair_zero_beyond_t<C, XW, W1, NT>(xs, tid);
  {
    const int c = ct * 32 + l31;
    if (c < NC1 && !(a.dbg & 2)) {
      const int p0 = 3 * D1 * (c / D1) + (c % D1);
      const int t0 = o0 - P2 + p0;
      const bool in0 = t0 >= 0 && t0 < len, in1 = t0 + D1 >= 0 && t0 + D1 < len, in2 = t0 + 2 * D1 >= 0 && t0 + 2 * D1 < len;
#pragma unroll
      for (int r = 0; r < 16; ++r) {
        const int row = mrow + (r & 3) + 8 * (r >> 2) + 4 * h;
        const float bz = a.b1[row];
        float v0, v1, v2;
        outs(r, v0, v1, v2);
        v0 += bz; v1 += bz; v2 += bz;
        v0 = v0 > 0.f ? v0 : v0 * slope;
        v1 = v1 > 0.f ? v1 : v1 * slope;
        v2 = v2 > 0.f ? v2 : v2 * slope;
        xs[row * XW + p0] = in0 ? v0 : 0.f;
        xs[row * XW + p0 + D1] = in1 ? v1 : 0.f;
        xs[row * XW + p0 + 2 * D1] = in2 ? v2 : 0.f;
      }
    }
  }
  __syncthreads();
  clear();
  if (!(a.dbg & 1)) taps(a.w2 + wslab, xs, base2, 1, D2);

  __syncthreads();
  float* ep = xs + wave * (8 * PW);
  const int prow = lane >> 5, pc4 = lane & 31;
  const int ws = ct * OW, woff = ws & 3;
  const int ncol = ws - woff + 4 * pc4;
  const int tcol = o0 + ncol;
  const size_t ob = (size_t)b * a.bstride;
  const int wend = ws + OW < WOUT ? ws + OW : WOUT;
  const int elo = ncol < ws ? ws - ncol : 0;
  const int ehi = (wend - ncol < len - tcol ? wend - ncol : len - tcol) < 4 ? (wend - ncol < len - tcol ? wend - ncol : len - tcol) : 4;
  const bool live = ehi > elo;
  const int epi = a.epi;
  const bool rmw = epi != EPI_RES && epi != EPI_MRF_SET;
  if (a.dbg & 4) {
    if (acc[0][0] == 123.f) a.out[0] = 1.f;
    return;
  }
  const int cl = l31 < NCW2 ? l31 : NCW2 - 1;
  const int pcol = woff + 3 * D2 * (cl / D2) + (cl % D2);
#pragma unroll
  for (int qd = 0; qd < 4; ++qd) {
    __builtin_amdgcn_sched_barrier(0);
    f32x4 rv[4], pa[4];
    const int tc = tcol > a.ld - 4 ? a.ld - 4 : tcol;
#pragma unroll
    for (int p = 0; p < 4; ++p) rv[p] = *reinterpret_cast<const f32x4*>(a.x + ob + (size_t)(mrow + 8 * qd + 2 * p + prow) * a.ld + tc);
    if (rmw) {
#pragma unroll
      for (int p = 0; p < 4; ++p) pa[p] = *reinterpret_cast<const f32x4*>(a.acc + ob + (size_t)(mrow + 8 * qd + 2 * p + prow) * a.ld + tc);
    }
    __builtin_amdgcn_wave_barrier();
#pragma unroll
    for (int r = 0; r < 4; ++r) {
      float y0, y1, y2;
      outs(4 * qd + r, y0, y1, y2);
      ep[(r + 4 * h) * PW + pcol] = y0;
      ep[(r + 4 * h) * PW + pcol + D2] = y1;
      ep[(r + 4 * h) * PW + pcol + 2 * D2] = y2;
    }
    __builtin_amdgcn_wave_barrier();
#pragma unroll
    for (int p = 0; p < 4; ++p) {
      const int prw = 2 * p + prow;
      f32x4 v = *reinterpret_cast<const f32x4*>(ep + prw * PW + (4 * pc4 < PW - 4 ? 4 * pc4 : PW - 4));
      if (!live) continue;
      const int row = mrow + 8 * qd + prw;
      const float bz = a.b2[row];
      const size_t idx = ob + (size_t)row * a.ld + tcol;
      pair_store_tail(a, epi, idx, v, bz, rv[p], [&] { return pa[p]; }, elo, ehi);
    }
  }
}

template <int KS_, int DIL>
__global__ void __launch_bounds__(256, (Tc6Geo<KS_, DIL>::OCC)) respair32_tc6_kernel(const PairArgs a) {
  pair_tc6_body<Tc6Geo<KS_, DIL>>(a);
}
template <int KS_, int DIL>
__global__ void __launch_bounds__(256, (Tc6Geo64<KS_, DIL>::OCC)) respair64_tc6_kernel(const PairArgs a) {
  pair_tc6_body<Tc6Geo64<KS_, DIL>>(a);
}

template <int KS_, int DIL>
__global__ void __launch_bounds__(256, 2) respair64_f23_kernel(const PairArgs a) {
  using G = F23Geo64<KS_, DIL>;
  constexpr int C = G::C, NW = G::NW, NT = 64 * NW, P2 = G::P2, P1 = G::P1, D1 = G::D1, D2 = G::D2, XW = G::XW, W1 = G::W1,
                NC1 = G::NC1, NC2 = G::NC2, WOUT = G::WOUT, PW = G::PW;
  static_assert(G::NS == 1 && D2 == 1 && XW % 2 == 0, "one sub-filter; conv_1's samples pair up into 8-byte reads");
  extern __shared__ __attribute__((aligned(16))) float xs[];

  int b, len, o0;
  if (!pair_tile<WOUT>(a, gridDim.y, b, len, o0)) return;
  const int tid = threadIdx.x, lane = tid & 63, wave = tid >> 6;
  const int l31 = lane & 31, h = lane >> 5;
  const int tin0 = o0 - P2 - P1;
  const int tb = tin0 & ~3, sh = tin0 - tb;
  const float slope = a.slope;
  const float* xb = a.x + (size_t)b * a.bstride;

  pair_stage_window<C, XW, NT, 2>(a, xb, xs, tb, len, tid);

  const int col = wave * 32 + l31;
  const int c1 = col < NC1 ? col : NC1 - 1, c2 = col < NC2 ? col : NC2 - 1;
  const int base1 = 2 * D1 * (c1 / D1) + (c1 % D1), base2 = 2 * D2 * (c2 / D2) + (c2 % D2);
  typedef float f32x16f __attribute__((ext_vector_type(16)));
  typedef float f32x2f __attribute__((ext_vector_type(2)));
  f32x16f acc[4][2];
  auto clear = [&]() __attribute__((always_inline)) {
#pragma unroll
    for (int p = 0; p < 4; ++p)
#pragma unroll
      for (int mi = 0; mi < 2; ++mi)
#pragma unroll
        for (int e = 0; e < 16; ++e) acc[p][mi][e] = 0.f;
  };
  auto taps = [&](const float* wq, const float* src, int dunit) __attribute__((always_inline)) {
    const __amdgpu_buffer_rsrc_t wr = wave_rsrc(wq, 0x7ffffff0u);
    const unsigned lane16 = lane * 16u;
    constexpr int NST = C / 8;
    f32x4 av[4][2], avn[4][2];
#pragma unroll
    for (int p = 0; p < 4; ++p)
#pragma unroll
      for (int mi = 0; mi < 2; ++mi) av[p][mi] = rsrc_load16(wr, lane16, (p * 2 + mi) * 1024u);
#pragma unroll
    for (int st = 0; st < NST; ++st) {
      const int sn = st + 1 < NST ? st + 1 : st;
#pragma unroll
      for (int p = 0; p < 4; ++p)
#pragma unroll
        for (int mi = 0; mi < 2; ++mi) avn[p][mi] = rsrc_load16(wr, lane16, ((sn * 4 + p) * 2 + mi) * 1024u);
      __builtin_amdgcn_sched_barrier(0);
#pragma unroll
      for (int e = 0; e < 4; ++e) {
        const float* q = src + (8 * st + 2 * e + h) * XW;
        float x0, x1, x2, x3;
        if (dunit == 1) {
          const f32x2f lo = *reinterpret_cast<const f32x2f*>(q), hi = *reinterpret_cast<const f32x2f*>(q + 2);
          x0 = lo[0]; x1 = lo[1]; x2 = hi[0]; x3 = hi[1];
        } else {
          x0 = q[0]; x1 = q[dunit]; x2 = q[2 * dunit]; x3 = q[3 * dunit];
        }
        float bq[4];
        bq[0] = x0 - x2;
        bq[1] = x1 + x2;
        bq[2] = x2 - x1;
        bq[3] = x1 - x3;
#pragma unroll
        for (int p = 0; p < 4; ++p)
#pragma unroll
          for (int mi = 0; mi < 2; ++mi)
            acc[p][mi] = __builtin_amdgcn_mfma_f32_32x32x2f32(av[p][mi][e], bq[p], acc[p][mi], 0, 0, 0);
      }
      __builtin_amdgcn_sched_barrier(0);
#pragma unroll
      for (int p = 0; p < 4; ++p)
#pragma unroll
        for (int mi = 0; mi < 2; ++mi) av[p][mi] = avn[p][mi];
    }
  };

  __syncthreads();
  clear();
  if (!(a.dbg & 1)) taps(a.w1, xs + sh + base1, D1);

  __syncthreads();
  pair_zero_beyond_t<C, XW, W1, NT>(xs, tid);
  if (col < NC1 && !(a.dbg & 2)) {
    const int pe = base1, po = pe + D1;
    const int te = o0 - P2 + pe, to = te + D1;
    const bool ine = te >= 0 && te < len, ino = to >= 0 && to < len;
#pragma unroll
    for (int mi = 0; mi < 2; ++mi)
#pragma unroll
      for (int r = 0; r < 16; ++r) {
        const int row = 32 * mi + (r & 3) + 8 * (r >> 2) + 4 * h;
        const float bz = a.b1[row];
        const float y0 = acc[0][mi][r], y1 = acc[1][mi][r], y2 = acc[2][mi][r], y3 = acc[3][mi][r];
        float ve = (y0 + y1) + y2 + bz, vo = (y1 - y2) - y3 + bz;
        ve = ve > 0.f ? ve : ve * slope;
        vo = vo > 0.f ? vo : vo * slope;
        xs[row * XW + pe] = ine ? ve : 0.f;
        xs[row * XW + po] = ino ? vo : 0.f;
      }
  }
  __syncthreads();
  clear();
  if (!(a.dbg & 1)) taps(a.w2, xs + base2, D2);

  __syncthreads();
  float* ep = xs + wave * (8 * PW);
  const int prow = lane >> 4, pc4 = lane & 15;
  const int ncol = wave * 64 + 4 * pc4;
  const int tcol = o0 + ncol;
  const size_t ob = (size_t)b * a.bstride;
  const bool live = ncol < WOUT && tcol < len;
  const int epi = a.epi;
  const bool rmw = epi != EPI_RES && epi != EPI_MRF_SET;
  if (a.dbg & 4) {
    if (acc[0][0][0] == 123.f) a.out[0] = 1.f;
    return;
  }
  const int pcol = 2 * l31;
#pragma unroll
  for (int mq = 0; mq < 8; ++mq) {
    const int mi = mq >> 2, qd = mq & 3;
    __builtin_amdgcn_sched_barrier(0);
    f32x4 rv[2], pa[2];
    const int tc = tcol > a.ld - 4 ? a.ld - 4 : tcol;
#pragma unroll
    for (int p = 0; p < 2; ++p) {
      const int row = 8 * mq + 4 * p + prow;
      rv[p] = *reinterpret_cast<const f32x4*>(a.x + ob + (size_t)row * a.ld + tc);
      if (rmw && live && tcol + 4 <= len) pa[p] = *reinterpret_cast<const f32x4*>(a.acc + ob + (size_t)row * a.ld + tcol);
    }
    __builtin_amdgcn_wave_barrier();
#pragma unroll
    for (int r = 0; r < 4; ++r) {
      const int rr = 4 * qd + r;
      const float y0 = acc[0][mi][rr], y1 = acc[1][mi][rr], y2 = acc[2][mi][rr], y3 = acc[3][mi][rr];
      f32x2f v;
      v[0] = (y0 + y1) + y2;
      v[1] = (y1 - y2) - y3;
      *reinterpret_cast<f32x2f*>(ep + (r + 4 * h) * PW + pcol) = v;
    }
    __builtin_amdgcn_wave_barrier();
#pragma unroll
    for (int p = 0; p < 2; ++p) {
      const int prw = 4 * p + prow;
      f32x4 v = *reinterpret_cast<const f32x4*>(ep + prw * PW + 4 * pc4);
      if (!live) continue;
      const int row = 8 * mq + prw;
      const float bz = a.b2[row];
      const size_t idx = ob + (size_t)row * a.ld + tcol;
      pair_store_tail(a, epi, idx, v, bz, rv[p], [&] { return pa[p]; }, 0, len - tcol < 4 ? len - tcol : 4);
    }
  }
}

#define DISSC_INSTANCE(K_, D_) template __global__ void respair32_f23_kernel<K_, D_>(const PairArgs);
DISSC_PAIR_F23_SHAPES(DISSC_INSTANCE)
#undef DISSC_INSTANCE
#define DISSC_INSTANCE(K_, D_) template __global__ void respair32_tc6_kernel<K_, D_>(const PairArgs);
DISSC_PAIR_TC6_SHAPES(DISSC_INSTANCE)
#undef DISSC_INSTANCE
#define DISSC_INSTANCE(K_, D_) template __global__ void respair64_f23_kernel<K_, D_>(const PairArgs);
DISSC_PAIR_F23_C64_SHAPES(DISSC_INSTANCE)
#undef DISSC_INSTANCE
#define DISSC_INSTANCE(K_, D_) template __global__ void respair64_tc6_kernel<K_, D_>(const PairArgs);
DISSC_PAIR_TC6_SHAPES(DISSC_INSTANCE)
#undef DISSC_INSTANCE

}
```

### include/dissc_hip.h

```cpp
#ifndef DISSC_HIP_H
#define DISSC_HIP_H

#include <stddef.h>
#include <stdint.h>

#ifdef __cplusplus
extern "C" {
#endif

#define DISSC_OK 0
#define DISSC_EINVAL (-1)
#define DISSC_ENOMEM (-2)
#define DISSC_EHIP (-3)
#define DISSC_ENOTFOUND (-4)
#define DISSC_ENOTSUP (-5)
#define DISSC_ECOMM (-6)

typedef struct {
  const char* name;
  const float* data;
  int64_t shape[4];
  int32_t ndim;
} DisscTensor;

const char* dissc_last_error(void);
int dissc_abi_version(void);
int dissc_device_count(void);
int dissc_device_name(int dev, char* buf, size_t buflen);

#define DISSC_MAX_UPS 8
#define DISSC_MAX_RK 4

typedef struct {
  int32_t model_in_dim;
  int32_t upsample_initial_channel;
  int32_t num_upsamples;
  int32_t upsample_rates[DISSC_MAX_UPS];
  int32_t upsample_kernel_sizes[DISSC_MAX_UPS];
  int32_t num_kernels;
  int32_t resblock_kernel_sizes[DISSC_MAX_RK];
  int32_t resblock_dilations[DISSC_MAX_RK][3];
  int32_t num_embeddings;
  int32_t embedding_dim;
  int32_t num_speakers;
  int32_t has_f0;
  int32_t has_spkr;
} DisscGenConfig;

typedef struct dissc_gen* dissc_gen_t;

int dissc_gen_create(const DisscGenConfig* cfg, const DisscTensor* weights, size_t n_weights,
                     dissc_gen_t* out);
int dissc_gen_create_ex(const DisscGenConfig* cfg, const DisscTensor* weights, size_t n_weights, int precision,
                        dissc_gen_t* out);
void dissc_gen_destroy(dissc_gen_t g);
int dissc_gen_hop(dissc_gen_t g);
size_t dissc_gen_workspace_bytes(dissc_gen_t g, int B, int Tmax);
double dissc_gen_flops(dissc_gen_t g, int64_t frames);
double dissc_gen_flops_executed(dissc_gen_t g, int64_t frames);
int dissc_gen_forward(dissc_gen_t g, const int64_t* code, const float* f0, const int64_t* spkr,
                      const int32_t* lengths, int B, int Tmax, float* wav_out, void* workspace,
                      size_t workspace_bytes, void* stream);
int dissc_conv1d(const float* x, const float* w_host, const float* bias_host, float* y,
                 const int32_t* lengths, int B, int Cin, int Cout, int k, int dilation, int ldx,
                 int ldo, int Lmax, float in_slope, void* stream);
int dissc_conv_transpose1d(const float* x, const float* w_host, const float* bias_host, float* y,
                           const int32_t* lengths, int B, int Cin, int Cout, int k, int stride,
                           int ldx, int ldo, int Lmax, float in_slope, void* stream);
int dissc_conv1d_prec(const float* x, const float* w_host, const float* bias_host, float* y,
                      const int32_t* lengths, int B, int Cin, int Cout, int k, int dilation, int ldx,
                      int ldo, int Lmax, float in_slope, int prec, void* stream);
int dissc_conv_transpose1d_prec(const float* x, const float* w_host, const float* bias_host, float* y,
                                const int32_t* lengths, int B, int Cin, int Cout, int k, int stride,
                                int ldx, int ldo, int Lmax, float in_slope, int prec, void* stream);

int dissc_conv1d_s2(const float* x, const float* w_host, const float* bias_host, float* y, const int32_t* lengths_in, int B,
                    int Cin, int Cout, int k, int ldx, int ldo, int Lmax_in, int act, int form, void* stream);
int dissc_conv1d_s2_prec(const float* x, const float* w_host, const float* bias_host, float* y, const int32_t* lengths_in, int B,
                         int Cin, int Cout, int k, int ldx, int ldo, int Lmax_in, int act, int prec, void* stream);
int dissc_linear_prec(const float* x, const float* w_host, const float* bias_host, const float* res, float* y,
                      const int32_t* lengths, int B, int Cin, int Cout, int ld, int Tmax, int act, int prec, void* stream);
int dissc_conv_s2_bench(int B, int C, int L, int form, int iters, float* ms_out);

int dissc_set_option(const char* key, int value);
int dissc_get_option(const char* key, int* value);

int dissc_conv_bench(int B, int Cin, int Cout, int k, int dilation, int L, int epi, int iters,
                     int flags, float* ms_out);

int dissc_respair1d(const float* x, const float* w1_host, const float* b1_host, const float* w2_host, const float* b2_host,
                    float* y, float* acc, const int32_t* lengths, int B, int C, int k, int dilation, int ld, int Lmax,
                    float slope, int epi, float mrf_div, int mode, void* stream);
int dissc_pair_bench(int B, int C, int k, int dilation, int L, int epi, int iters, int mode, float* ms_out);
int dissc_pair_info(int C, int k, int dilation, int* form_out, int* tile_out);
typedef struct {
  int32_t family, cfg, bm, bn, rows;
  int32_t p0, np, ntap, pad_left;
} DisscConvLaunch;
int dissc_conv_info(int Cin, int Cout, int k, int dilation, int up, int B, int Lmax_out, DisscConvLaunch* out, int max_out,
                    int* n_out);

typedef struct {
  int32_t mi, ni, wps, r, ns;
  int32_t unit, ot, cpr, gx, gy;
} DisscWino8Plan;
int dissc_wino8_info(int C, int k, int dilation, int R, int B, int Lmax, DisscWino8Plan* out);

typedef struct {
  int32_t ns, dilation, cpr, rh, tw, shv;
  int32_t unit, ot, gx, gy, wgs, lds_bytes;
} DisscWinoPlan;
int dissc_wino_info(int C, int k, int dilation, int B, int Lmax, DisscWinoPlan* out);

int dissc_resblock1d_bf3(const float* x, const float* const* w6_host, const float* const* b6_host, float* acc,
                         const int32_t* lengths, int B, int C, int k, const int32_t* dil3, int ld, int Lmax, float slope,
                         int epi, float mrf_div, int m0, int m1, void* stream);
typedef struct {
  int32_t bm, bn, small_grid, tile;
  int32_t cols, h4, pad;
} DisscBf3Info;
int dissc_bf3_info(int Cout, int Cin, int k, int dilation, int B, int Lmax, const int32_t* dil3, int m0, int m1,
                   DisscBf3Info* out);

typedef struct dissc_pred* dissc_pred_t;
int dissc_pred_create(int kind, const DisscTensor* weights, size_t n_weights, dissc_pred_t* out);
void dissc_pred_destroy(dissc_pred_t p);
size_t dissc_pred_workspace_bytes(dissc_pred_t p, int B, int Lmax);
int dissc_len_set_norm(dissc_pred_t p, float mean, float std);
int dissc_len_forward(dissc_pred_t p, const int64_t* seq, const int64_t* spk, const int32_t* lengths,
                      int B, int Lmax, float* out, int ldo, void* workspace, size_t workspace_bytes,
                      void* stream);
int dissc_pitch_forward(dissc_pred_t p, const int64_t* seq, const int64_t* spk,
                        const int32_t* lengths, int B, int Tmax, int norm, const float* id2mean,
                        const float* id2std, int n_stats, float* out, int ldo, void* workspace,
                        size_t workspace_bytes, void* stream);
int dissc_pitch_stats(const double* f0, const int64_t* offsets, int n_speakers, double* mean_out,
                      double* std_out, int64_t* count_out, void* stream);
int dissc_dedup(const int64_t* units, const int32_t* lengths, int B, int Tmax, int64_t* vals,
                int32_t* counts, int32_t* n_out, void* stream);
int dissc_len_carryover(const float* lens, const int32_t* n, int B, int ld, int32_t* lens_int,
                        int32_t* totals, void* stream);
int dissc_expand(const int64_t* vals, const int32_t* lens_int, const int32_t* n, int B, int ld_in,
                 int64_t* out, int ld_out, void* stream);

typedef struct dissc_hubert* dissc_hubert_t;
int dissc_hubert_create(int n_layers, const DisscTensor* weights, size_t n_weights,
                        const float* centers, int n_centers, dissc_hubert_t* out);
int dissc_hubert_create_ex(int n_layers, const DisscTensor* weights, size_t n_weights, const float* centers, int n_centers,
                           int precision, dissc_hubert_t* out);
int dissc_hubert_precision(dissc_hubert_t m);
void dissc_hubert_destroy(dissc_hubert_t m);
int dissc_hubert_frames(int n_samples);
size_t dissc_hubert_workspace_bytes(dissc_hubert_t m, int B, int Nmax);
int dissc_hubert_forward(dissc_hubert_t m, const float* wav, const int32_t* n_samples, int B, int Nmax,
                         float* dense_out, int64_t* units_out, void* workspace,
                         size_t workspace_bytes, void* stream);
int dissc_kmeans_assign(const float* dense, const float* centers, const float* cnorm, int T, int K, int D, int64_t* units,
                        void* stream);

int dissc_mfma_peak(int iters, float* tflops);
int dissc_erf_check(const float* x, float* y, int n, void* stream);
int dissc_attention(const float* qkv, const int32_t* lens, int B, int Tmax, int D, int ld, float* out, void* stream);
int dissc_layernorm_cf(const float* x, const float* gamma, const float* beta, const int32_t* lens, int B, int C, int ld, float eps,
                       float* y, void* stream);
int dissc_pipe_overlap(int mfma_iters, int valu_iters, float* ms);

int dissc_wav_postprocess(float* wav, const int32_t* n_samples, int B, int ld, void* stream);

int dissc_pack_rows(const float* wav, long long ld_wav, const int32_t* n_samples, const long long* offsets,
                    int B, int n_max, float* data, void* stream);

#define DISSC_COMM_ID_BYTES 128
int dissc_comm_unique_id(void* id_out);
int dissc_comm_create(const void* id, int nranks, int rank, void** comm_out);
int dissc_comm_destroy(void* comm);
int dissc_allgather_waves(void* nccl_comm, const float* send, size_t n_floats, float* recv, void* stream);

typedef struct {
  int32_t fs;
  int32_t frame_len;
  int32_t frame_hop;
  int32_t tda_len;
  int32_t nfft;
  float f0_min, f0_max;
  int32_t shc_numharms;
  float shc_window_hz, shc_pwidth_hz, shc_thresh1, shc_thresh2, f0_double, f0_half;
  float nccf_thresh1, nccf_thresh2;
  int32_t nccf_pwidth;
} DisscYaaptConfig;
typedef struct dissc_yaapt* dissc_yaapt_t;
int dissc_yaapt_create(const float* fir, int n_taps, const DisscYaaptConfig* cfg, dissc_yaapt_t* out);
void dissc_yaapt_destroy(dissc_yaapt_t y);
int dissc_yaapt_frames(dissc_yaapt_t y, int n_samples);
int dissc_yaapt_tda_frames(dissc_yaapt_t y, int n_samples);
int dissc_yaapt_shc_bins(dissc_yaapt_t y);
size_t dissc_yaapt_workspace_bytes(dissc_yaapt_t y, int B, int Nmax);
int dissc_yaapt_spectral(dissc_yaapt_t y, const float* wav, const int32_t* n_samples, int B, int Nmax, float* filt,
                         float* nlfilt, float* energy, float* cand_pitch, float* cand_merit, float* shc_out,
                         void* workspace, size_t workspace_bytes, void* stream);
int dissc_yaapt_nccf(dissc_yaapt_t y, const float* sig, const int32_t* n_samples, const int32_t* lag_min,
                     const int32_t* lag_max, int B, int Nmax, int F, float* pitch, float* merit, float* phi_out,
                     void* workspace, size_t workspace_bytes, void* stream);

typedef struct {
  double nlfer_thresh1, nlfer_thresh2;
  double dp5_k1;
  double merit_boost, merit_pivot, merit_extra;
  double dp_w1, dp_w2, dp_w3, dp_w4;
  double spec_pitch_min_std;
  double f0_min, f0_max;
  int32_t median_value;
  int32_t nccf_pwidth;
  int32_t fs;
  int32_t reserved;
} DisscYaaptTrackConfig;
size_t dissc_yaapt_track_workspace_bytes(int B, int F);
int dissc_yaapt_spec_track(const DisscYaaptTrackConfig* cfg, const float* energy, const float* cand_pitch,
                           const float* cand_merit, const int32_t* n_frames, const int32_t* n_tda, int B, int F,
                           double* en_norm, uint8_t* vuv, double* spec, double* spec_std, int32_t* lag_min,
                           int32_t* lag_max, void* workspace, size_t workspace_bytes, void* stream);
int dissc_yaapt_final_track(const DisscYaaptTrackConfig* cfg, const float* tp1, const float* tm1, const float* tp2,
                            const float* tm2, const double* en_norm, const uint8_t* vuv, const double* spec,
                            const double* spec_std, const int32_t* n_tda, int B, int F, float* f0, void* workspace,
                            size_t workspace_bytes, void* stream);

#define DISSC_EMD_MAX_PAIR_FRAMES 40000
#define DISSC_FFE_EMPTY_SYN 1
#define DISSC_FFE_BAD_ENTRY 2
size_t dissc_track_emd_workspace_bytes(int n_pairs, int max_pair_frames);
int dissc_track_emd(const float* tracks, int n_rows, int ld, const int32_t* pairs, int n_pairs, int max_pair_frames,
                    double* emd_out, void* workspace, size_t workspace_bytes, void* stream);
size_t dissc_track_ffe_workspace_bytes(int n_intervals);
int dissc_track_ffe(const float* tracks, int n_rows, int ld, const int32_t* intervals, int n_intervals,
                    double* ffe_out, int32_t* status_out, void* workspace, size_t workspace_bytes, void* stream);

int dissc_resample(const double* x, int n_orig, double* y, int n_out, double ratio, const double* win,
                   const double* delta, int nwin, int num_table, void* stream);

typedef struct dissc_trainer* dissc_trainer_t;
int dissc_train_create(int kind, const DisscTensor* tensors, size_t n, dissc_trainer_t* out);
void dissc_train_destroy(dissc_trainer_t t);
int dissc_train_set_len_norm(dissc_trainer_t t, float mean, float std);
int dissc_train_set_pitch_stats(dissc_trainer_t t, const float* id2mean, const float* id2std, int n);
size_t dissc_train_workspace_bytes(dissc_trainer_t t, int B, int L);
int dissc_train_step(dissc_trainer_t t, const int64_t* seq, const int64_t* spk, const float* target, const float* keep,
                     const float* pe_mult, int B, int L, float pad_value, float lr, float* loss_out, void* workspace,
                     size_t workspace_bytes, void* stream);
int dissc_train_num_tensors(dissc_trainer_t t);
const char* dissc_train_tensor_name(dissc_trainer_t t, int i);
long long dissc_train_tensor_numel(dissc_trainer_t t, int i);
long long dissc_train_steps(dissc_trainer_t t);
int dissc_train_read(dissc_trainer_t t, int i, int which, float* host_out, void* stream);
int dissc_train_debug_read(dissc_trainer_t t, int layer, int which, float* host_out, size_t n, void* stream);

#define DISSC_MEL_TILE_FRAMES 64
#define DISSC_MEL_GRAD_TILE_FRAMES 64
#define DISSC_MEL_LINEAR 1
typedef struct dissc_mel* dissc_mel_t;
int dissc_mel_filterbank(int sr, int n_fft, int num_mels, double fmin, double fmax, double* out);
int dissc_mel_create(int sr, int n_fft, int num_mels, int hop, int win, double fmin, double fmax, dissc_mel_t* out);
void dissc_mel_destroy(dissc_mel_t h);
int dissc_mel_frames(dissc_mel_t h, int n_samples);
size_t dissc_mel_workspace_bytes(dissc_mel_t h, int B, int Nmax);
int dissc_mel_forward(dissc_mel_t h, const float* wav, int ld, const int32_t* n_samples_dev, int B, float* mel_out, int ldF,
                      int flags, void* workspace, size_t workspace_bytes, void* stream);
int dissc_mel_l1(dissc_mel_t h, const float* a, int lda, const float* b, int ldb, const int32_t* n_samples_dev, int B,
                 double* sum_out, void* workspace, size_t workspace_bytes, void* stream);
size_t dissc_mel_grad_workspace_bytes(dissc_mel_t h, int B, int Nmax);
int dissc_mel_backward(dissc_mel_t h, const float* wav, int ld, const int32_t* n_samples_dev, int B, const float* g_mel, int ldF,
                       int flags, float* grad_wav, int ldg, void* workspace, size_t workspace_bytes, void* stream);
int dissc_mel_l1_grad(dissc_mel_t h, const float* a, int lda, const float* b, int ldb, const int32_t* n_samples_dev, int B,
                      const double* scale_dev, double* sum_out, float* grad_b, int ldg, void* workspace, size_t workspace_bytes,
                      void* stream);

#define DISSC_CONVGRAD_CHUNK 64
typedef struct dissc_convgrad* dissc_convgrad_t;
int dissc_convgrad_create(int Cin, int Cout, int k, int dilation, dissc_convgrad_t* out);
void dissc_convgrad_destroy(dissc_convgrad_t h);
int dissc_convgrad_set_weights(dissc_convgrad_t h, const float* w_dev, const float* bias_dev, void* stream);
int dissc_convgrad_forward(dissc_convgrad_t h, const float* x, const float* add, float* y, const int32_t* lengths, int B,
                           int ldx, int ldo, int Lmax, float in_slope, void* stream);
int dissc_convgrad_partials(dissc_convgrad_t h, int B, int Lmax, int* P, int* pairs_per_partial);
size_t dissc_convgrad_workspace_bytes(dissc_convgrad_t h, int B, int Lmax);
int dissc_convgrad_backward(dissc_convgrad_t h, const float* x, const float* gy, const int32_t* lengths, int B, int ldx,
                            int ldo, int Lmax, float in_slope, float* gx, float* gw, float* gb, void* workspace,
                            size_t workspace_bytes, void* stream);

typedef struct dissc_convtgrad* dissc_convtgrad_t;
int dissc_convtgrad_create(int Cin, int Cout, int k, int stride, dissc_convtgrad_t* out);
void dissc_convtgrad_destroy(dissc_convtgrad_t h);
int dissc_convtgrad_set_weights(dissc_convtgrad_t h, const float* w_dev, const float* bias_dev, void* stream);
int dissc_convtgrad_forward(dissc_convtgrad_t h, const float* x, float* y, const int32_t* lengths, int B, int ldx, int ldo,
                            int Lmax_in, float in_slope, void* stream);
int dissc_convtgrad_partials(dissc_convtgrad_t h, int B, int Lmax_in, int* P, int* pairs_per_partial);
size_t dissc_convtgrad_workspace_bytes(dissc_convtgrad_t h, int B, int Lmax_in);
int dissc_convtgrad_backward(dissc_convtgrad_t h, const float* x, const float* gy, const int32_t* lengths, int B, int ldx,
                             int ldo, int Lmax_in, float in_slope, float* gx, float* gw, float* gb, void* workspace,
                             size_t workspace_bytes, void* stream);

typedef struct dissc_convsgrad* dissc_convsgrad_t;
int dissc_convsgrad_create(int Cin, int Cout, int k, int stride, dissc_convsgrad_t* out);
void dissc_convsgrad_destroy(dissc_convsgrad_t h);
int dissc_convsgrad_set_weights(dissc_convsgrad_t h, const float* w_dev, const float* bias_dev, void* stream);
long long dissc_convsgrad_packed(dissc_convsgrad_t h, int which, float* dst_dev, void* stream);
int dissc_convsgrad_forward(dissc_convsgrad_t h, const float* x, float* y, const int32_t* lengths, int B, int ldx, int ldo,
                            int Lmax_in, float in_slope, void* stream);
int dissc_convsgrad_partials(dissc_convsgrad_t h, int B, int Lmax_in, int* P, int* pairs_per_partial);
size_t dissc_convsgrad_workspace_bytes(dissc_convsgrad_t h, int B, int Lmax_in);
int dissc_convsgrad_backward(dissc_convsgrad_t h, const float* x, const float* gy, const int32_t* lengths, int B, int ldx,
                             int ldo, int Lmax_in, float in_slope, float* gx, float* gw, float* gb, void* workspace,
                             size_t workspace_bytes, void* stream);
int dissc_period_fold_fwd(const float* wav, const int32_t* lengths, int B, int T, int period, int ldw, int ldh, float* x0,
                          void* stream);
int dissc_period_fold_bwd(const float* gx0, const int32_t* lengths, int B, int T, int period, int ldw, int ldh, float* gwav,
                          void* stream);

typedef struct dissc_convggrad* dissc_convggrad_t;
int dissc_convggrad_create(int Cin, int Cout, int k, int stride, int groups, dissc_convggrad_t* out);
void dissc_convggrad_destroy(dissc_convggrad_t h);
int dissc_convggrad_set_weights(dissc_convggrad_t h, const float* w_dev, const float* bias_dev, void* stream);
long long dissc_convggrad_packed(dissc_convggrad_t h, int which, float* dst_dev, void* stream);
int dissc_convggrad_forward(dissc_convggrad_t h, const float* x, float* y, const int32_t* lengths, int B, int ldx, int ldo,
                            int Lmax_in, float in_slope, void* stream);
int dissc_convggrad_partials(dissc_convggrad_t h, int B, int Lmax_in, int* P, int* pairs_per_partial);
size_t dissc_convggrad_workspace_bytes(dissc_convggrad_t h, int B, int Lmax_in);
int dissc_convggrad_backward(dissc_convggrad_t h, const float* x, const float* gy, const int32_t* lengths, int B, int ldx,
                             int ldo, int Lmax_in, float in_slope, float* gx, float* gw, float* gb, void* workspace,
                             size_t workspace_bytes, void* stream);
int dissc_mean_pool_fwd(const float* x, float* out, const int32_t* lengths, int B, int C, int T, int ldx, int ldo, void* stream);
int dissc_mean_pool_bwd(const float* gy, float* gx, const int32_t* lengths, int B, int C, int T, int ldx, int ldo, void* stream);

typedef struct dissc_wnorm* dissc_wnorm_t;
int dissc_wnorm_create(int n, const int* rows, const int* cols, dissc_wnorm_t* out);
void dissc_wnorm_destroy(dissc_wnorm_t h);
int dissc_wnorm_offsets(dissc_wnorm_t h, long long* off, long long* row_off, long long* total_floats, long long* total_rows);
int dissc_wnorm_wave_cols(void);
int dissc_wnorm_forward(dissc_wnorm_t h, const float* v_flat, const float* g_flat, float* w_flat, float* inv_norm,
                        const float* bias_flat, float* bias_out, int nbias, void* stream);
int dissc_wnorm_backward(dissc_wnorm_t h, const float* v_flat, const float* g_flat, const float* const* gw_ptrs, float* gv_flat, float* gg_flat, const float* const* gb_ptrs,
                         const int* bias_n, float* gb_flat, void* stream);
int dissc_embed_concat_fwd(const int64_t* code, const float* f0, const int64_t* spkr, const float* dict_w, const float* spkr_w,
                           const int32_t* lengths, int B, int T, int E, int n_codes, int n_spk, float* x, int ldx, void* stream);
int dissc_embed_concat_bwd(const float* gx, const int64_t* code, int has_f0, const int64_t* spkr, const int32_t* lengths, int B,
                           int T, int E, int n_codes, int n_spk, int ldx, float* g_dict, float* g_spkr, void* stream);
int dissc_mrf_mean_fwd(const float* const* r, int nk, float* y, const int32_t* lengths, int B, int C, int ld, int Lmax, void* stream);
int dissc_mrf_mean_bwd(const float* g, int nk, float* gx, const int32_t* lengths, int B, int C, int ld, int Lmax, void* stream);
int dissc_tanh_fwd(const float* x, float* y, const int32_t* lengths, int B, int C, int ldx, int ldy, int Lmax, void* stream);
int dissc_tanh_bwd(const float* y, const float* gy, float* gx, const int32_t* lengths, int B, int C, int ldx, int ldy, int Lmax,
                   void* stream);

#define DISSC_GANLOSS_MAX_MAPS 64
#define DISSC_GANLOSS_FM 0
#define DISSC_GANLOSS_DISC 1
#define DISSC_GANLOSS_GEN 2
size_t dissc_ganloss_workspace_bytes(int n, const int* R, const int* C, const int* ld);
int dissc_ganloss_forward(int n, const float* const* maps, const int32_t* const* lengths, const int* R, const int* C,
                          const int* ld, const int* ops, const float* slopes, float* out, void* workspace, size_t workspace_bytes,
                          void* stream);
int dissc_ganloss_backward(int n, const float* const* maps, const int32_t* const* lengths, const int* R, const int* C,
                           const int* ld, const int* ops, const float* slopes, const float* g_total, const float* g_vals,
                           float* const* gmaps, void* stream);

#ifdef __cplusplus
}
#endif
#endif
```

Before: 10270.

## Fuse whole k=3 resblock chain into one Winograd F(2,3) MFMA kernel

Adds a kernel that runs all three conv pairs of a k=3, dilation (1,3,5) resblock for C=16 and C=32 in a single launch. It stages a haloed input window in LDS and keeps intermediates in LDS and registers between pairs, using Winograd F(2,3) on MFMA. This removes two of three launches and the global-memory round trips of intermediate activations. The cost is redundant halo computation, larger LDS use and register pressure, which may lower occupancy. It is enabled by default through a new chain_f23 option.

After: 10450, median of 6. +1.8%, better.

```diff
diff --git a/dissc_amd/_lib.py b/dissc_amd/_lib.py
--- a/dissc_amd/_lib.py
+++ b/dissc_amd/_lib.py
@@ -39,6 +39,10 @@
 
 class DisscBf3Info(ctypes.Structure):
     _fields_ = [(n, ctypes.c_int32) for n in ("bm", "bn", "small_grid", "tile", "cols", "h4", "pad")]
+
+
+class DisscChainInfo(ctypes.Structure):
+    _fields_ = [(n, ctypes.c_int32) for n in ("wout", "span", "halo", "lds_bytes", "tiles_per_wave")]
 
 
 class DisscWino8Plan(ctypes.Structure):
@@ -124,6 +128,10 @@
     L.dissc_wino_info.argtypes = [i32] * 5 + [ctypes.POINTER(DisscWinoPlan)]
     L.dissc_resblock1d_bf3.argtypes = [vp, vp, vp, vp, vp, i32, i32, i32, vp, i32, i32, ctypes.c_float, i32, ctypes.c_float, i32, i32, vp]
     L.dissc_bf3_info.argtypes = [i32] * 6 + [vp, i32, i32, ctypes.POINTER(DisscBf3Info)]
+    if hasattr(L, "dissc_reschain1d"):
+        L.dissc_reschain1d.argtypes = [vp] * 6 + [i32] * 3 + [vp, i32, i32, ctypes.c_float, i32, ctypes.c_float, i32, vp]
+        L.dissc_chain_info.argtypes = [i32, i32, vp, ctypes.POINTER(DisscChainInfo)]
+        L.dissc_chain_bench.argtypes = [i32] * 6 + [ctypes.POINTER(ctypes.c_float)]
     L.dissc_respair1d.argtypes = [vp] * 8 + [i32] * 6 + [ctypes.c_float, i32, ctypes.c_float, i32, vp]
     L.dissc_wav_postprocess.argtypes = [vp, vp, i32, i32, vp]
     L.dissc_pitch_stats.argtypes = [vp, vp, i32, vp, vp, vp, vp]
diff --git a/dissc_amd/csrc/common.h b/dissc_amd/csrc/common.h
--- a/dissc_amd/csrc/common.h
+++ b/dissc_amd/csrc/common.h
@@ -44,7 +44,8 @@
   X(pair_f23, 3, "pair_f23") \
   X(pair_tc6, 3, "pair_tc6") \
   X(pair_f23_c64, 1, "pair_f23_c64") \
-  X(pair_tc6_c64, 1, "pair_tc6_c64")
+  X(pair_tc6_c64, 1, "pair_tc6_c64") \
+  X(chain_f23, 3, "chain_f23")
 #define DISSC_OPTION_LIST_EXPERIMENTAL(X) \
   X(graphs, 0, "graphs") \
   X(graph_frames, 2048, "graph_frames") \
@@ -344,6 +345,13 @@
 int launch_respair_wino(const DevPairW& pw, const float* x, float* out, const Batch& bt, const EpiSpec& ep, int ld, float slope,
                         hipStream_t stream);
 
+struct ChainInfo { int wout, span, halo, lds_bytes, tiles_per_wave; };
+bool chain_f23_supported(int C, int KS, const int* dil);
+bool chain_f23_info(int C, int KS, const int* dil, ChainInfo& ci);
+int make_chain_f23(const float* const* w6, const float* const* b6, int C, float** dev_w, float** dev_b);
+int launch_reschain_f23(const float* w, const float* bias, int C, const float* x, float* out, const Batch& bt, const EpiSpec& ep, int ld,
+                        float slope, hipStream_t stream);
+
 bool respair_supported(int C, int KS, int dil);
 int launch_respair(const DevConv& c1, const DevConv& c2, const float* x, float* out, const Batch& bt, const EpiSpec& ep, int ld,
                    float slope, hipStream_t stream);
diff --git a/dissc_amd/csrc/diag.hip b/dissc_amd/csrc/diag.hip
--- a/dissc_amd/csrc/diag.hip
+++ b/dissc_amd/csrc/diag.hip
@@ -189,6 +189,120 @@
   if (!rc)
     rc = pair_run(mode, ds, x, tmp, y, batch_of(lengths, 1, B, Lmax), epi_of(epi, nullptr, acc, mrf_div), C, ld, slope, (hipStream_t)stream);
   return drained(rc, (hipStream_t)stream);
+}
+
+struct ChainDiag {
+  DiagScope pair[3];
+  int pmode[3] = {0, 0, 0};
+  float *w = nullptr, *b = nullptr, *s1 = nullptr, *s2 = nullptr;
+  ~ChainDiag() {
+    for (float* q : {w, b, s1, s2})
+      if (q) (void)hipFree(q);
+  }
+};
+static int chain_make(int mode, const float* const* w6, const float* const* b6, int C, int k, const int* dil, size_t scratch_floats,
+                      ChainDiag& cd) {
+  if (mode == 1) {
+    if (!chain_f23_supported(C, k, dil)) {
+      set_error("chain mode 1: no instance for C = %d, k = %d, dilations (%d, %d, %d)", C, k, dil[0], dil[1], dil[2]);
+      return DISSC_EINVAL;
+    }
+    return make_chain_f23(w6, b6, C, &cd.w, &cd.b);
+  }
+  if (mode != 0) {
+    set_error("chain mode %d", mode);
+    return DISSC_EINVAL;
+  }
+  for (int m = 0; m < 3; ++m) {
+    cd.pmode[m] = pair_reg_form(C, k, dil[m]) ? 3 : 1;
+    if (cd.pmode[m] == 1 && !respair_supported(C, k, dil[m])) {
+      set_error("chain mode 0: no one-launch pair for C = %d, k = %d, dilation %d", C, k, dil[m]);
+      return DISSC_EINVAL;
+    }
+    const int rc = pair_make(cd.pmode[m], w6[2 * m], b6[2 * m], w6[2 * m + 1], b6[2 * m + 1], C, k, dil[m], cd.pair[m]);
+    if (rc) return rc;
+  }
+  if (hipMalloc(&cd.s1, scratch_floats * sizeof(float)) != hipSuccess || hipMalloc(&cd.s2, scratch_floats * sizeof(float)) != hipSuccess) {
+    set_error("chain mode 0: hipMalloc");
+    return DISSC_ENOMEM;
+  }
+  return DISSC_OK;
+}
+static int chain_run(int mode, const ChainDiag& cd, const float* x, float* y, const Batch& bt, const EpiSpec& ep, int C, int ld, float slope,
+                     hipStream_t st) {
+  if (mode == 1) return launch_reschain_f23(cd.w, cd.b, C, x, y, bt, ep, ld, slope, st);
+  int rc = pair_run(cd.pmode[0], cd.pair[0], x, nullptr, cd.s1, bt, epi_of(EPI_RES), C, ld, slope, st);
+  if (!rc) rc = pair_run(cd.pmode[1], cd.pair[1], cd.s1, nullptr, cd.s2, bt, epi_of(EPI_RES), C, ld, slope, st);
+  if (!rc) rc = pair_run(cd.pmode[2], cd.pair[2], cd.s2, nullptr, y, bt, ep, C, ld, slope, st);
+  return rc;
+}
+
+int dissc_reschain1d(const float* x, const float* const* w6_host, const float* const* b6_host, float* y, float* acc, const int32_t* lengths,
+                     int B, int C, int k, const int32_t* dil3, int ld, int Lmax, float slope, int epi, float mrf_div, int mode,
+                     void* stream) {
+  if (!x || !w6_host || !b6_host || !dil3 || B <= 0 || Lmax <= 0 || ld < Lmax || epi < EPI_RES || epi > EPI_MRF_DIV ||
+      (epi == EPI_RES ? !y || y == x : !acc || acc == x)) {
+    set_error("dissc_reschain1d: bad argument");
+    return DISSC_EINVAL;
+  }
+  for (int l = 0; l < 6; ++l)
+    if (!w6_host[l] || !b6_host[l]) {
+      set_error("dissc_reschain1d: weight or bias %d is null", l);
+      return DISSC_EINVAL;
+    }
+  const int dil[3] = {dil3[0], dil3[1], dil3[2]};
+  ChainDiag cd;
+  int rc = chain_make(mode, w6_host, b6_host, C, k, dil, (size_t)B * C * ld, cd);
+  if (!rc) rc = chain_run(mode, cd, x, y, batch_of(lengths, 1, B, Lmax), epi_of(epi, nullptr, acc, mrf_div), C, ld, slope, (hipStream_t)stream);
+  return drained(rc, (hipStream_t)stream);
+}
+
+int dissc_chain_info(int C, int k, const int32_t* dil3, DisscChainInfo* out) {
+  ChainInfo ci;
+  const int dil[3] = {dil3 ? dil3[0] : 0, dil3 ? dil3[1] : 0, dil3 ? dil3[2] : 0};
+  if (!chain_f23_info(C, k, dil, ci)) {
+    set_error("dissc_chain_info: no instance for C = %d, k = %d, dilations (%d, %d, %d)", C, k, dil[0], dil[1], dil[2]);
+    return DISSC_EINVAL;
+  }
+  if (out) {
+    out->wout = ci.wout; out->span = ci.span; out->halo = ci.halo; out->lds_bytes = ci.lds_bytes; out->tiles_per_wave = ci.tiles_per_wave;
+  }
+  return DISSC_OK;
+}
+
+int dissc_chain_bench(int B, int C, int L, int epi, int iters, int mode, float* ms_out) {
+  if (!ms_out || B <= 0 || L <= 0 || iters <= 0 || epi < EPI_RES || epi > EPI_MRF_DIV) {
+    set_error("dissc_chain_bench: bad argument");
+    return DISSC_EINVAL;
+  }
+  const int k = 3, dil[3] = {1, 3, 5};
+  std::vector<float> w[6], bias(C, 0.1f);
+  const float *w6[6], *b6[6];
+  Lcg rnd;
+  for (int l = 0; l < 6; ++l) {
+    w[l].resize((size_t)C * C * k);
+    rnd.fill(w[l], 0.05f);
+    w6[l] = w[l].data();
+    b6[l] = bias.data();
+  }
+  const int ld = (L + 3) / 4 * 4;
+  const size_t n = (size_t)B * C * ld;
+  ChainDiag cd;
+  int rc = chain_make(mode, w6, b6, C, k, dil, n, cd);
+  if (rc) return rc;
+  DiagScope ds;
+  float *x = nullptr, *y = nullptr, *a = nullptr;
+  std::vector<float> hx(n);
+  rnd.fill(hx, 2.f);
+  if (ds.alloc(&x, n) != hipSuccess || ds.alloc(&y, n) != hipSuccess || ds.alloc(&a, n) != hipSuccess ||
+      hipMemcpy(x, hx.data(), n * 4, hipMemcpyHostToDevice) != hipSuccess || hipMemset(a, 0, n * 4) != hipSuccess ||
+      ds.events() != hipSuccess) {
+    set_error("dissc_chain_bench: allocation failed");
+    return DISSC_ENOMEM;
+  }
+  const Batch bt = batch_of(nullptr, 1, B, L);
+  const EpiSpec ep = epi_of(epi, nullptr, a, 3.f);
+  return time_launches(ds, iters, [&]() { return chain_run(mode, cd, x, y, bt, ep, C, ld, 0.1f, nullptr); }, ms_out);
 }
 
 int dissc_resblock1d_bf3(const float* x, const float* const* w6_host, const float* const* b6_host, float* acc, const int32_t* lengths,
diff --git a/dissc_amd/csrc/gen_plan.h b/dissc_amd/csrc/gen_plan.h
--- a/dissc_amd/csrc/gen_plan.h
+++ b/dissc_amd/csrc/gen_plan.h
@@ -7,6 +7,7 @@
   pairs,
   bf3_block,
   bf3_pairs,
+  f23_chain,
 };
 enum class PairForm : uint8_t {
   direct,
@@ -30,6 +31,7 @@
 int pair_reg_form(int C, int KS, int dil);
 ChainPlan plan_chain(int C, int KS, const int* dil, int prec);
 double pair_macs(const PairPlan& p, int C, int KS, bool executed);
+double chain_macs(const ChainPlan& cp, int C, int KS, bool executed);
 int make_pair_conv(ConvForm f, const float* w, const float* b, int C, int KS, int dil, DevConv& dc);
 inline int mrf_epi(int j, int nk) { return j == nk - 1 ? EPI_MRF_DIV : j == 0 ? EPI_MRF_SET : EPI_MRF_ADD; }
 
diff --git a/dissc_amd/csrc/gen_plan.hip b/dissc_amd/csrc/gen_plan.hip
--- a/dissc_amd/csrc/gen_plan.hip
+++ b/dissc_amd/csrc/gen_plan.hip
@@ -19,6 +19,11 @@
     return ConvForm::f43;
   const bool r4 = opts().wino8_r4 && wino8_r4_supported(C, KS, dil) && ((opts().wino8_r4_mask >> w8_shape_bit(C, KS, dil)) & 1);
   return r4 ? ConvForm::f54 : ConvForm::f63;
+}
+
+static bool chain_f23_wanted(int C, int KS, const int* dil, int prec) {
+  const int bit = C == 32 ? 1 : C == 16 ? 2 : 0;
+  return prec == 0 && opts().wino && opts().pair_f23 && C <= opts().pair_max_c && (opts().chain_f23 & bit) && chain_f23_supported(C, KS, dil);
 }
 
 int pair_reg_form(int C, int KS, int dil) {
@@ -73,7 +78,15 @@
       p.form = PairForm::direct_dma;
     }
   }
+  if (chain_f23_wanted(C, KS, dil, prec)) cp.form = ChainForm::f23_chain;
   return cp;
+}
+
+double chain_macs(const ChainPlan& cp, int C, int KS, bool executed) {
+  if (executed && cp.form == ChainForm::f23_chain) return 3 * 2 * 2.0 * C * C;
+  double macs = 0;
+  for (const PairPlan& p : cp.pair) macs += pair_macs(p, C, KS, executed);
+  return macs;
 }
 
 double pair_macs(const PairPlan& p, int C, int KS, bool executed) {
diff --git a/dissc_amd/csrc/generator.hip b/dissc_amd/csrc/generator.hip
--- a/dissc_amd/csrc/generator.hip
+++ b/dissc_amd/csrc/generator.hip
@@ -191,6 +191,11 @@
         snprintf(name, sizeof(name), "resblocks.%d.convs%d.%d.bias", (int)cj, 1 + l % 2, l / 2);
         if ((rc = get(name, {ch}, &b6[l]))) return fail(rc);
       }
+      if (cp.form == ChainForm::f23_chain) {
+        const std::vector<const float*> wv(w6, w6 + 6), bv(b6, b6 + 6);
+        tasks.push_back([=]() { return make_chain_f23(wv.data(), bv.data(), ch, &g->fused_w[cj], &g->fused_b[cj]); });
+        continue;
+      }
       if (cp.form != ChainForm::pairs) {
         std::vector<float> fw, fb;
         pack_resblock_bf3(ch, rk, w6, fw);
@@ -270,8 +275,7 @@
     for (auto& c : g->ups[i]) macs += c.macs_per_t * mul;
     mul = g->stage_mul[i];
     for (int j = 0; j < nk; ++j)
-      for (const PairPlan& p : g->plan[(size_t)i * nk + j].pair)
-        macs += pair_macs(p, g->stage_C[i], g->cfg.resblock_kernel_sizes[j], executed) * mul;
+      macs += chain_macs(g->plan[(size_t)i * nk + j], g->stage_C[i], g->cfg.resblock_kernel_sizes[j], executed) * mul;
   }
   macs += (double)g->post_C * g->post_KS * mul;
   return macs;
@@ -419,6 +423,11 @@
       };
       if (cp.form == ChainForm::bf3_block) {
         if ((rc = acc_turn()) || (rc = launch_resblock_bf3(bf3, X, bt, mrf, ld, 0.1f, 0, 3, sj))) return rc;
+        if (multi) DISSC_HIP_CHECK(hipEventRecord(g->ev_fin[j], sj));
+        continue;
+      }
+      if (cp.form == ChainForm::f23_chain) {
+        if ((rc = acc_turn()) || (rc = launch_reschain_f23(g->fused_w[cj], g->fused_b[cj], ch, X, nullptr, bt, mrf, ld, 0.1f, sj))) return rc;
         if (multi) DISSC_HIP_CHECK(hipEventRecord(g->ev_fin[j], sj));
         continue;
       }
diff --git a/dissc_amd/csrc/pair_host.hip b/dissc_amd/csrc/pair_host.hip
--- a/dissc_amd/csrc/pair_host.hip
+++ b/dissc_amd/csrc/pair_host.hip
@@ -95,6 +95,48 @@
   return upload(packed, dev);
 }
 
+bool chain_f23_supported(int C, int KS, const int* dil) {
+  return (C == 16 || C == 32) && KS == 3 && dil && dil[0] == 1 && dil[1] == 3 && dil[2] == 5;
+}
+
+bool chain_f23_info(int C, int KS, const int* dil, ChainInfo& ci) {
+  if (!chain_f23_supported(C, KS, dil)) return false;
+  auto fill = [&](auto geo) {
+    using G = decltype(geo);
+    ci.wout = G::WOUT; ci.span = G::NP; ci.halo = G::HALO; ci.lds_bytes = (int)sizeof(float) * G::C * G::XW; ci.tiles_per_wave = G::NI;
+  };
+  if (C == 32) fill(F23ChainGeo32());
+  else fill(F23ChainGeo16());
+  return true;
+}
+
+int make_chain_f23(const float* const* w6, const float* const* b6, int C, float** dev_w, float** dev_b) {
+  if (C != 16 && C != 32) {
+    set_error("make_chain_f23: no instance for C = %d", C);
+    return DISSC_EINVAL;
+  }
+  std::vector<float> packed, bias((size_t)6 * C, 0.f);
+  packed.reserve((size_t)6 * 4 * C * C);
+  for (int l = 0; l < 6; ++l) {
+    const std::vector<float> U = transform_taps(w6[l], C, 3, &kF23G[0][0], 4, 3);
+    auto u = [&](int p, int co, int ci) { return U[((size_t)p * C + co) * C + ci]; };
+    if (C == 16) {
+      for (int p = 0; p < 4; ++p)
+        for (int lane = 0; lane < 64; ++lane)
+          for (int cq = 0; cq < 4; ++cq) packed.push_back(u(p, lane & 15, 4 * cq + (lane >> 4)));
+    } else {
+      for (int st = 0; st < 4; ++st)
+        for (int p = 0; p < 4; ++p)
+          for (int lane = 0; lane < 64; ++lane)
+            for (int e = 0; e < 4; ++e) packed.push_back(u(p, lane & 31, 8 * st + 2 * e + (lane >> 5)));
+    }
+    if (b6 && b6[l]) memcpy(bias.data() + (size_t)l * C, b6[l], C * sizeof(float));
+  }
+  int rc = upload(packed, dev_w);
+  if (!rc) rc = upload(bias, dev_b);
+  return rc;
+}
+
 int make_pairw(const float* w1, const float* b1, const float* w2, const float* b2, int C, int KS, int dil, int form, DevPairW& pw) {
   pw.form = form;
   if (!pair_form_supported(form, C, KS, dil)) {
@@ -176,4 +218,28 @@
   return DISSC_EINVAL;
 }
 
-}
+template <class Geo, auto Kernel, auto KernelDbg>
+static int launch_chain(const PairArgs& a, int B, int Lmax, hipStream_t stream) {
+  dim3 grid((Lmax + Geo::WOUT - 1) / Geo::WOUT, B);
+  hipLaunchKernelGGL(a.dbg ? KernelDbg : Kernel, grid, dim3(256), sizeof(float) * Geo::C * Geo::XW, stream, a);
+  DISSC_HIP_CHECK(hipGetLastError());
+  return DISSC_OK;
+}
+
+int launch_reschain_f23(const float* w, const float* bias, int C, const float* x, float* out, const Batch& bt, const EpiSpec& ep, int ld,
+                        float slope, hipStream_t stream) {
+  const int B = bt.B, Lmax = bt.Lmax;
+  if (!w || !bias || !x || (C != 16 && C != 32) || ep.epi == EPI_STORE || (ep.epi == EPI_RES ? !out || x == out : !ep.acc || x == ep.acc) ||
+      ld < 4 || ld % 4 || misaligned16(x) || misaligned16(out) || misaligned16(ep.acc) || B <= 0 || Lmax <= 0) {
+    set_error("launch_reschain_f23: bad argument (C=%d ld=%d epi=%d)", C, ld, ep.epi);
+    return DISSC_EINVAL;
+  }
+  PairArgs a;
+  a.x = x; a.out = out; a.acc = ep.acc; a.w1 = w; a.w2 = nullptr; a.b1 = bias; a.b2 = nullptr;
+  a.lengths = bt.lengths; a.len_default = bt.len_default; a.len_mul = bt.len_mul; a.ld = ld;
+  a.bstride = (long long)C * ld; a.slope = slope; a.mrf_div = ep.mrf_div; a.epi = ep.epi; a.dbg = opts().kernel_dbg;
+  if (C == 32) return launch_chain<F23ChainGeo32, reschain32_f23_kernel<false>, reschain32_f23_kernel<true>>(a, B, Lmax, stream);
+  return launch_chain<F23ChainGeo16, reschain16_f23_kernel<false>, reschain16_f23_kernel<true>>(a, B, Lmax, stream);
+}
+
+}
diff --git a/dissc_amd/csrc/respair16_f23.hip b/dissc_amd/csrc/respair16_f23.hip
--- a/dissc_amd/csrc/respair16_f23.hip
+++ b/dissc_amd/csrc/respair16_f23.hip
@@ -144,6 +144,182 @@
   }
 }
 
+template <bool DBG>
+__global__ void __launch_bounds__(256, 3) reschain16_f23_kernel(const PairArgs a) {
+  using G = F23ChainGeo16;
+  constexpr int C = G::C, NW = G::NW, NT = 64 * NW, XW = G::XW, PADL = G::PADL, HALO = G::HALO, WOUT = G::WOUT, PW = G::PW, NI = G::NI;
+  static_assert(NI == 4, "four column tiles per wave");
+  extern __shared__ __attribute__((aligned(16))) float xs[];
+
+  int b, len, o0;
+  if (!pair_tile<WOUT>(a, gridDim.y, b, len, o0)) return;
+  const int tid = threadIdx.x, lane = tid & 63, wave = tid >> 6;
+  const int l15 = lane & 15, g = lane >> 4;
+  const int t00 = o0 - HALO;
+  const float slope = a.slope;
+  const int dbg = DBG ? a.dbg : 0;
+  const size_t ob = (size_t)b * a.bstride;
+  const float* xb = a.x + ob;
+  typedef float f32x2f __attribute__((ext_vector_type(2)));
+
+  const __amdgpu_buffer_rsrc_t wr = wave_rsrc(a.w1, 0x7ffffff0u);
+  f32x4 u[4];
+  auto load_w = [&](int ci) __attribute__((always_inline)) {
+#pragma unroll
+    for (int p = 0; p < 4; ++p) u[p] = rsrc_load16(wr, lane * 16u, (unsigned)((ci * 4 + p) * 1024));
+  };
+  load_w(0);
+  pair_stage_window<C, XW, NT>(a, xb, xs, t00 - PADL, len, tid);
+  __builtin_amdgcn_sched_barrier(0);
+
+  const int col0 = wave * 64 + l15;
+  f32x2f res[NI][4];
+#pragma unroll
+  for (int ni = 0; ni < NI; ++ni) {
+    const int tc0 = t00 + 2 * (col0 + 16 * ni);
+    const int tcl = tc0 < 0 ? 0 : (tc0 > a.ld - 2 ? a.ld - 2 : tc0);
+#pragma unroll
+    for (int r = 0; r < 4; ++r) res[ni][r] = *reinterpret_cast<const f32x2f*>(xb + (size_t)(4 * g + r) * a.ld + tcl);
+  }
+  f32x2f y[NI][4];
+  auto taps = [&](const float* src, const int (&off)[NI], int dunit) __attribute__((always_inline)) {
+#pragma unroll
+    for (int ni = 0; ni < NI; ++ni) {
+      f32x4 acc[4];
+#pragma unroll
+      for (int p = 0; p < 4; ++p)
+#pragma unroll
+        for (int e = 0; e < 4; ++e) acc[p][e] = 0.f;
+#pragma unroll
+      for (int cq = 0; cq < 4; ++cq) {
+        const float* q = src + (4 * cq + g) * XW + off[ni];
+        float x0, x1, x2, x3;
+        if (dunit == 1) {
+          const f32x2f lo = *reinterpret_cast<const f32x2f*>(q), hi = *reinterpret_cast<const f32x2f*>(q + 2);
+          x0 = lo[0]; x1 = lo[1]; x2 = hi[0]; x3 = hi[1];
+        } else {
+          x0 = q[0]; x1 = q[dunit]; x2 = q[2 * dunit]; x3 = q[3 * dunit];
+        }
+        float bq[4];
+        bq[0] = x0 - x2;
+        bq[1] = x1 + x2;
+        bq[2] = x2 - x1;
+        bq[3] = x1 - x3;
+#pragma unroll
+        for (int p = 0; p < 4; ++p) acc[p] = __builtin_amdgcn_mfma_f32_16x16x4f32(u[p][cq], bq[p], acc[p], 0, 0, 0);
+      }
+#pragma unroll
+      for (int r = 0; r < 4; ++r) {
+        y[ni][r][0] = (acc[0][r] + acc[1][r]) + acc[2][r];
+        y[ni][r][1] = (acc[1][r] - acc[2][r]) - acc[3][r];
+      }
+    }
+  };
+  auto clear = [&]() __attribute__((always_inline)) {
+#pragma unroll
+    for (int ni = 0; ni < NI; ++ni)
+#pragma unroll
+      for (int r = 0; r < 4; ++r) y[ni][r][0] = y[ni][r][1] = 0.f;
+  };
+  int pc[NI];
+#pragma unroll
+  for (int ni = 0; ni < NI; ++ni) pc[ni] = 2 * (col0 + 16 * ni);
+
+#pragma unroll
+  for (int m = 0; m < 3; ++m) {
+    const int d = G::dil(m), T0 = G::t0(m), NC1 = G::nc1(m);
+    int pe[NI], offd[NI];
+#pragma unroll
+    for (int ni = 0; ni < NI; ++ni) {
+      const int c = col0 + 16 * ni, c1 = c < NC1 ? c : NC1 - 1;
+      pe[ni] = T0 + 2 * d * (c1 / d) + (c1 % d);
+      offd[ni] = pe[ni] - d;
+    }
+    __syncthreads();
+    __builtin_amdgcn_sched_barrier(0);
+    if (dbg & 1) clear();
+    else taps(xs + PADL, offd, d);
+    __builtin_amdgcn_sched_barrier(0);
+    load_w(2 * m + 1);
+
+    __syncthreads();
+    __builtin_amdgcn_sched_barrier(0);
+#pragma unroll
+    for (int ni = 0; ni < NI; ++ni) {
+      if (col0 + 16 * ni < NC1 && !(dbg & 2)) {
+        const int te = t00 + pe[ni], to = te + d;
+        const bool ine = te >= 0 && te < len, ino = to >= 0 && to < len;
+#pragma unroll
+        for (int r = 0; r < 4; ++r) {
+          const int row = 4 * g + r;
+          const float bz = a.b1[(2 * m) * C + row];
+          float ve = y[ni][r][0] + bz, vo = y[ni][r][1] + bz;
+          ve = ve > 0.f ? ve : ve * slope;
+          vo = vo > 0.f ? vo : vo * slope;
+          xs[row * XW + PADL + 1 + pe[ni]] = ine ? ve : 0.f;
+          xs[row * XW + PADL + 1 + pe[ni] + d] = ino ? vo : 0.f;
+        }
+      }
+    }
+    __syncthreads();
+    __builtin_amdgcn_sched_barrier(0);
+    if (dbg & 1) clear();
+    else taps(xs + PADL, pc, 1);
+    __builtin_amdgcn_sched_barrier(0);
+    if (m < 2) load_w(2 * m + 2);
+
+#pragma unroll
+    for (int ni = 0; ni < NI; ++ni)
+#pragma unroll
+      for (int r = 0; r < 4; ++r) {
+        const float bz = a.b1[(2 * m + 1) * C + 4 * g + r];
+        res[ni][r][0] = (y[ni][r][0] + bz) + res[ni][r][0];
+        res[ni][r][1] = (y[ni][r][1] + bz) + res[ni][r][1];
+      }
+    __syncthreads();
+    __builtin_amdgcn_sched_barrier(0);
+    if (m < 2 && !(dbg & 2)) {
+#pragma unroll
+      for (int ni = 0; ni < NI; ++ni) {
+        const int tc0 = t00 + pc[ni];
+        const bool in_e = tc0 >= 0 && tc0 < len, in_o = tc0 + 1 >= 0 && tc0 + 1 < len;
+#pragma unroll
+        for (int r = 0; r < 4; ++r) {
+          f32x2f v;
+          v[0] = in_e ? (res[ni][r][0] > 0.f ? res[ni][r][0] : res[ni][r][0] * slope) : 0.f;
+          v[1] = in_o ? (res[ni][r][1] > 0.f ? res[ni][r][1] : res[ni][r][1] * slope) : 0.f;
+          *reinterpret_cast<f32x2f*>(xs + (4 * g + r) * XW + PADL + pc[ni]) = v;
+        }
+      }
+    }
+  }
+
+  if (dbg & 4) {
+    if (res[0][0][0] == 123.f && a.acc) a.acc[0] = 1.f;
+    return;
+  }
+  float* ep = xs + wave * (16 * PW);
+  const int prow = lane >> 5, pc4 = lane & 31;
+  const int pq = wave * 128 + 4 * pc4;
+  const int tq = t00 + pq;
+  const bool live = pq >= HALO && pq < HALO + WOUT && tq < len;
+  const int epi = a.epi;
+#pragma unroll
+  for (int ni = 0; ni < NI; ++ni)
+#pragma unroll
+    for (int r = 0; r < 4; ++r) *reinterpret_cast<f32x2f*>(ep + (4 * g + r) * PW + 2 * (16 * ni + l15)) = res[ni][r];
+  __builtin_amdgcn_wave_barrier();
+#pragma unroll
+  for (int p = 0; p < 8; ++p) {
+    const int row = 2 * p + prow;
+    const f32x4 v = *reinterpret_cast<const f32x4*>(ep + row * PW + 4 * pc4);
+    if (!live) continue;
+    chain_store_tail(a, epi, ob + (size_t)row * a.ld + tq, v, len - tq);
+  }
+}
+
+template __global__ void reschain16_f23_kernel<false>(const PairArgs);
+template __global__ void reschain16_f23_kernel<true>(const PairArgs);
 #define DISSC_INSTANCE(K_, D_) template __global__ void respair16_f23_kernel<K_, D_>(const PairArgs);
 DISSC_PAIR_F23_SHAPES(DISSC_INSTANCE)
 #undef DISSC_INSTANCE
diff --git a/dissc_amd/csrc/respair_f23.h b/dissc_amd/csrc/respair_f23.h
--- a/dissc_amd/csrc/respair_f23.h
+++ b/dissc_amd/csrc/respair_f23.h
@@ -107,6 +107,46 @@
 template <int KS, int DIL> using F23Geo16 = F23Geo<16, 16, KS, DIL>;
 template <int KS, int DIL> using F23Geo64 = F23Geo<64, 8, KS, DIL, 32>;
 
+template <int C_, int PROWS, int WCOLS>
+struct F23ChainGeo {
+  static constexpr int C = C_, NW = 4, KS = 3, NI = WCOLS / (C_ == 16 ? 16 : 32);
+  static constexpr int NCOLS = WCOLS * NW, NP = 2 * NCOLS;
+  static constexpr int HALO = 12, PADL = 4;
+  static constexpr int WOUT = NP - 2 * HALO;
+  static constexpr int XW = round32_16(PADL + NP + 8);
+  static constexpr int PW = 2 * WCOLS + 4;
+  static constexpr int dil(int m) { return 2 * m + 1; }
+  static constexpr int t0(int m) { return m == 0 ? 1 : m == 1 ? 3 : 4; }
+  static constexpr int nc1(int m) { return NCOLS / dil(m) * dil(m); }
+  static constexpr int w1(int m) { return 2 * nc1(m); }
+  static constexpr bool covers() {
+    int a = -PADL, b = XW - PADL;
+    for (int m = 0; m < 3; ++m) {
+      const int d = dil(m), lo = t0(m), hi = t0(m) + w1(m);
+      if (lo - d < -PADL || hi + d > XW - PADL || hi + 1 > XW - PADL) return false;
+      const int tlo = lo > a + d ? lo : a + d, thi = hi < b - d ? hi : b - d;
+      a = tlo + 1 > 0 ? tlo + 1 : 0;
+      b = thi - 1 < NP ? thi - 1 : NP;
+    }
+    return a <= HALO && b >= HALO + WOUT;
+  }
+  static_assert(WOUT % 4 == 0 && HALO % 4 == 0 && PADL % 4 == 0, "owned quads are whole");
+  static_assert(PADL + NP + 3 <= XW, "conv_1's reads of T stay in the row");
+  static_assert(NW * PROWS * PW <= C * XW, "the epilogue patches fit the buffer");
+};
+using F23ChainGeo32 = F23ChainGeo<32, 8, 32>;
+using F23ChainGeo16 = F23ChainGeo<16, 16, 64>;
+static_assert(F23ChainGeo32::covers() && F23ChainGeo16::covers(), "each pair's valid range covers what the next pair reads");
+
+__device__ __forceinline__ void chain_store_tail(const PairArgs& a, int epi, size_t idx, const f32x4& x, int n) {
+  if (n >= 4) {
+    epi_store_res(epi, quad_at(a.out + idx), quad_at(a.acc + idx), x, [&] { return load_quad(a.acc + idx); }, a.mrf_div);
+  } else {
+    for (int e = 0; e < n; ++e)
+      epi_store_res(epi, a.out + idx + e, a.acc + idx + e, x[e], [&] { return a.acc[idx + e]; }, a.mrf_div);
+  }
+}
+
 template <int C_, int KS_, int DIL_>
 struct Tc6GeoC {
   static constexpr int KS = KS_, DIL = DIL_, NS = (KS_ + 3) / 4, C = C_, NW = 4, RB = C_ / 32, NCT = NW / RB;
@@ -134,6 +174,8 @@
 template <int KS, int DIL> __global__ void respair16_f23_kernel(const PairArgs a);
 template <int KS, int DIL> __global__ void respair64_f23_kernel(const PairArgs a);
 template <int KS, int DIL> __global__ void respair64_tc6_kernel(const PairArgs a);
+template <bool DBG> __global__ void reschain32_f23_kernel(const PairArgs a);
+template <bool DBG> __global__ void reschain16_f23_kernel(const PairArgs a);
 #if DISSC_EXPERIMENTAL
 #define DISSC_PAIR_F23_SHAPES(X) X(11, 1) X(11, 3) X(11, 5) X(3, 1) X(3, 3) X(3, 5)
 #else
diff --git a/dissc_amd/csrc/respair_f23.hip b/dissc_amd/csrc/respair_f23.hip
--- a/dissc_amd/csrc/respair_f23.hip
+++ b/dissc_amd/csrc/respair_f23.hip
@@ -497,6 +497,154 @@
   }
 }
 
+template <bool DBG>
+__global__ void __launch_bounds__(256, 2) reschain32_f23_kernel(const PairArgs a) {
+  using G = F23ChainGeo32;
+  constexpr int C = G::C, NW = G::NW, NT = 64 * NW, XW = G::XW, PADL = G::PADL, HALO = G::HALO, WOUT = G::WOUT, PW = G::PW;
+  extern __shared__ __attribute__((aligned(16))) float xs[];
+
+  int b, len, o0;
+  if (!pair_tile<WOUT>(a, gridDim.y, b, len, o0)) return;
+  const int tid = threadIdx.x, lane = tid & 63, wave = tid >> 6;
+  const int l31 = lane & 31, h = lane >> 5;
+  const int t00 = o0 - HALO;
+  const float slope = a.slope;
+  const int dbg = DBG ? a.dbg : 0;
+  const size_t ob = (size_t)b * a.bstride;
+  const float* xb = a.x + ob;
+  typedef float f32x16f __attribute__((ext_vector_type(16)));
+  typedef float f32x2f __attribute__((ext_vector_type(2)));
+
+  const __amdgpu_buffer_rsrc_t wr = wave_rsrc(a.w1, 0x7ffffff0u);
+  const unsigned lane16 = lane * 16u;
+  f32x4 wv[4][4];
+  auto load_w = [&](int ci) __attribute__((always_inline)) {
+#pragma unroll
+    for (int st = 0; st < 4; ++st)
+#pragma unroll
+      for (int p = 0; p < 4; ++p) wv[st][p] = rsrc_load16(wr, lane16, (unsigned)(((ci * 4 + st) * 4 + p) * 1024));
+  };
+  load_w(0);
+
+  pair_stage_window<C, XW, NT>(a, xb, xs, t00 - PADL, len, tid);
+
+  const int col = wave * 32 + l31, pc = 2 * col, tc0 = t00 + pc;
+  const bool in_e = tc0 >= 0 && tc0 < len, in_o = tc0 + 1 >= 0 && tc0 + 1 < len;
+  f32x2f res[16];
+  {
+    const int tcl = tc0 < 0 ? 0 : (tc0 > a.ld - 2 ? a.ld - 2 : tc0);
+#pragma unroll
+    for (int r = 0; r < 16; ++r)
+      res[r] = *reinterpret_cast<const f32x2f*>(xb + (size_t)((r & 3) + 8 * (r >> 2) + 4 * h) * a.ld + tcl);
+  }
+  f32x16f acc[4];
+  auto clear = [&]() __attribute__((always_inline)) {
+#pragma unroll
+    for (int p = 0; p < 4; ++p)
+#pragma unroll
+      for (int e = 0; e < 16; ++e) acc[p][e] = 0.f;
+  };
+  auto taps = [&](const float* src, int dunit) __attribute__((always_inline)) {
+#pragma unroll
+    for (int st = 0; st < 4; ++st)
+#pragma unroll
+      for (int e = 0; e < 4; ++e) {
+        const float* q = src + (8 * st + 2 * e + h) * XW;
+        float x0, x1, x2, x3;
+        if (dunit == 1) {
+          const f32x2f lo = *reinterpret_cast<const f32x2f*>(q), hi = *reinterpret_cast<const f32x2f*>(q + 2);
+          x0 = lo[0]; x1 = lo[1]; x2 = hi[0]; x3 = hi[1];
+        } else {
+          x0 = q[0]; x1 = q[dunit]; x2 = q[2 * dunit]; x3 = q[3 * dunit];
+        }
+        float bq[4];
+        bq[0] = x0 - x2;
+        bq[1] = x1 + x2;
+        bq[2] = x2 - x1;
+        bq[3] = x1 - x3;
+#pragma unroll
+        for (int p = 0; p < 4; ++p) acc[p] = __builtin_amdgcn_mfma_f32_32x32x2f32(wv[st][p][e], bq[p], acc[p], 0, 0, 0);
+      }
+  };
+
+#pragma unroll
+  for (int m = 0; m < 3; ++m) {
+    const int d = G::dil(m), T0 = G::t0(m), NC1 = G::nc1(m);
+    const int c1 = col < NC1 ? col : NC1 - 1;
+    const int pe = T0 + 2 * d * (c1 / d) + (c1 % d);
+    __syncthreads();
+    clear();
+    if (!(dbg & 1)) taps(xs + PADL + pe - d, d);
+    load_w(2 * m + 1);
+
+    __syncthreads();
+    if (col < NC1 && !(dbg & 2)) {
+      const int te = t00 + pe, to = te + d;
+      const bool ine = te >= 0 && te < len, ino = to >= 0 && to < len;
+#pragma unroll
+      for (int r = 0; r < 16; ++r) {
+        const int row = (r & 3) + 8 * (r >> 2) + 4 * h;
+        const float bz = a.b1[(2 * m) * C + row];
+        const float y0 = acc[0][r], y1 = acc[1][r], y2 = acc[2][r], y3 = acc[3][r];
+        float ve = (y0 + y1) + y2 + bz, vo = (y1 - y2) - y3 + bz;
+        ve = ve > 0.f ? ve : ve * slope;
+        vo = vo > 0.f ? vo : vo * slope;
+        xs[row * XW + PADL + 1 + pe] = ine ? ve : 0.f;
+        xs[row * XW + PADL + 1 + pe + d] = ino ? vo : 0.f;
+      }
+    }
+    __syncthreads();
+    clear();
+    if (!(dbg & 1)) taps(xs + PADL + pc, 1);
+    if (m < 2) load_w(2 * m + 2);
+
+#pragma unroll
+    for (int r = 0; r < 16; ++r) {
+      const float bz = a.b1[(2 * m + 1) * C + (r & 3) + 8 * (r >> 2) + 4 * h];
+      const float y0 = acc[0][r], y1 = acc[1][r], y2 = acc[2][r], y3 = acc[3][r];
+      res[r][0] = (((y0 + y1) + y2) + bz) + res[r][0];
+      res[r][1] = (((y1 - y2) - y3) + bz) + res[r][1];
+    }
+    __syncthreads();
+    if (m < 2 && !(dbg & 2)) {
+#pragma unroll
+      for (int r = 0; r < 16; ++r) {
+        f32x2f v;
+        v[0] = in_e ? (res[r][0] > 0.f ? res[r][0] : res[r][0] * slope) : 0.f;
+        v[1] = in_o ? (res[r][1] > 0.f ? res[r][1] : res[r][1] * slope) : 0.f;
+        *reinterpret_cast<f32x2f*>(xs + ((r & 3) + 8 * (r >> 2) + 4 * h) * XW + PADL + pc) = v;
+      }
+    }
+  }
+
+  if (dbg & 4) {
+    if (res[0][0] == 123.f && a.acc) a.acc[0] = 1.f;
+    return;
+  }
+  float* ep = xs + wave * (8 * PW);
+  const int prow = lane >> 4, pc4 = lane & 15;
+  const int pq = wave * 64 + 4 * pc4;
+  const int tq = t00 + pq;
+  const bool live = pq >= HALO && pq < HALO + WOUT && tq < len;
+  const int epi = a.epi;
+#pragma unroll
+  for (int mq = 0; mq < 4; ++mq) {
+    __builtin_amdgcn_wave_barrier();
+#pragma unroll
+    for (int r = 0; r < 4; ++r) *reinterpret_cast<f32x2f*>(ep + (r + 4 * h) * PW + 2 * l31) = res[4 * mq + r];
+    __builtin_amdgcn_wave_barrier();
+#pragma unroll
+    for (int p = 0; p < 2; ++p) {
+      const int prw = 4 * p + prow;
+      const f32x4 v = *reinterpret_cast<const f32x4*>(ep + prw * PW + 4 * pc4);
+      if (!live) continue;
+      chain_store_tail(a, epi, ob + (size_t)(8 * mq + prw) * a.ld + tq, v, len - tq);
+    }
+  }
+}
+
+template __global__ void reschain32_f23_kernel<false>(const PairArgs);
+template __global__ void reschain32_f23_kernel<true>(const PairArgs);
 #define DISSC_INSTANCE(K_, D_) template __global__ void respair32_f23_kernel<K_, D_>(const PairArgs);
 DISSC_PAIR_F23_SHAPES(DISSC_INSTANCE)
 #undef DISSC_INSTANCE
diff --git a/include/dissc_hip.h b/include/dissc_hip.h
--- a/include/dissc_hip.h
+++ b/include/dissc_hip.h
@@ -115,6 +115,14 @@
 int dissc_resblock1d_bf3(const float* x, const float* const* w6_host, const float* const* b6_host, float* acc,
                          const int32_t* lengths, int B, int C, int k, const int32_t* dil3, int ld, int Lmax, float slope,
                          int epi, float mrf_div, int m0, int m1, void* stream);
+int dissc_reschain1d(const float* x, const float* const* w6_host, const float* const* b6_host, float* y, float* acc,
+                     const int32_t* lengths, int B, int C, int k, const int32_t* dil3, int ld, int Lmax, float slope, int epi,
+                     float mrf_div, int mode, void* stream);
+typedef struct {
+  int wout, span, halo, lds_bytes, tiles_per_wave;
+} DisscChainInfo;
+int dissc_chain_info(int C, int k, const int32_t* dil3, DisscChainInfo* out);
+int dissc_chain_bench(int B, int C, int L, int epi, int iters, int mode, float* ms_out);
 typedef struct {
   int32_t bm, bn, small_grid, tile;
   int32_t cols, h4, pad;
```
